# deweylab/RSEM

Hardware: AMD Instinct MI355X
Metric: EM read-alignments/s (nnz x EM iterations per second), rsem-run-em theta-only rounds (higher is better)
Workload: dtype f64; 1 GPU; BASELINE configs[2] (PairedEndQModel-shaped, the north-star target config): EM matrix of 50000000 reads x 200000 transcripts, 570042118 alignments (11.40/read) per GPU, frozen conprb (rounds >= 12); synthetic_config=C3, kernel=0, parallelism=1 GPU

## Files before the change

rsem_amd/csrc/em.hip:

```cpp
#include <climits>
#include <cstdlib>
#include <cmath>
#include <type_traits>

#include "comm_internal.hpp"
#include "em_internal.hpp"
#include "upload.hpp"
#include "sell_layout.hpp"

namespace {

using rsem::kEpsilon;

constexpr int kReduceBlocks = 64;
constexpr int kMaxTimedRounds = 4096;
constexpr int kWindow = 2048;
static_assert(kWindow == kLayoutWindow, "the layout sorts reads apart and sizes windows for the E step's LDS window (sell_layout.hpp)");

constexpr int kTotSlots = 64;

struct Ctrl {
    int done;
    int final_round;
    int totNum;
// ... 288 lines not shown
            const double change = fabs(th - old) / old;
            if (change >= 0.001) ++tot;
            bmax = fmax(bmax, change);
        }
    };
    if (pre) {
#pragma unroll
        for (int k = 0; k < kPre; k++) {
            const int i = lo + (int)threadIdx.x + kBlock * k;
            if (i < hi) one(i, pc[k], pp[k]);
        }
    } else {
        for (int i = lo + threadIdx.x; i < hi; i += kBlock) one(i, cur[i], A.prev[i]);
    }
    for (int d = 32; d >= 1; d >>= 1) {
        tot += __shfl_xor(tot, d);
        bmax = fmax(bmax, __shfl_xor(bmax, d));
    }
    csum = wave_sum(csum);
    __shared__ int s_tot[kBlock / 64];
    __shared__ double s_b[kBlock / 64], s_c[kBlock / 64];
    if (lane == 0) { s_tot[threadIdx.x >> 6] = tot; s_b[threadIdx.x >> 6] = bmax; s_c[threadIdx.x >> 6] = csum; }
    __syncthreads();
    if (threadIdx.x == 0) {
        for (int i = 1; i < kBlock / 64; i++) { tot += s_tot[i]; bmax = fmax(bmax, s_b[i]); csum += s_c[i]; }
        Ctrl* ctrl = A.ctrl;
        unsigned int zero = 0;
        if (bmax > 0.0) {
            const unsigned long long was = __hip_atomic_fetch_max(&ctrl->bbits, (unsigned long long)__double_as_longlong(bmax),
                                                                  __ATOMIC_RELAXED, __HIP_MEMORY_SCOPE_AGENT);
            asm volatile("v_and_b32 %0, 0, %1" : "=v"(zero) : "v"((unsigned int)was));
        }
        zero += sum_slot_put(ctrl, me, csum);
        const unsigned long long old = __hip_atomic_fetch_add(&ctrl->tick2, (((unsigned long long)(unsigned)tot << 32) | 1ull) + zero,
                                                              __ATOMIC_RELAXED, __HIP_MEMORY_SCOPE_AGENT);
        if ((int)(old & 0xffffffffull) == n_close - 1) {
            const int round = A.stat_round;
            const int totNum = (int)(old >> 32) + tot;
            const unsigned long long bb = __hip_atomic_load(&ctrl->bbits, __ATOMIC_RELAXED, __HIP_MEMORY_SCOPE_AGENT);
            const double fsum = sum_slots_take(ctrl, n_close);
            ctrl->last_sum = fsum;
            ctrl->last_bchange = __longlong_as_double((long long)bb);
            ctrl->last_totNum = totNum;
            ctrl->last_round = round;
            const bool stop = !(round < A.min_round || (totNum > 0 && round < A.max_round));
            if (stop) {
                ctrl->done = 1;
                ctrl->final_round = round;
            }
            if (A.mirror) {
                RoundStat* h = &A.mirror->hist[(round - 1) % kHistCap];
                h->sum = fsum;
                h->bchange = __longlong_as_double((long long)bb);
                h->totNum = totNum;
                h->round = round;
                if (stop) A.mirror->final_round = round;
                __hip_atomic_store(&A.mirror->last_round, round, __ATOMIC_RELEASE, __HIP_MEMORY_SCOPE_SYSTEM);
                if (stop) __hip_atomic_store(&A.mirror->done, 1, __ATOMIC_RELEASE, __HIP_MEMORY_SCOPE_SYSTEM);
            }
            __hip_atomic_store(&ctrl->bbits, 0ull, __ATOMIC_RELAXED, __HIP_MEMORY_SCOPE_AGENT);
            __hip_atomic_store(&ctrl->tick2, 0ull, __ATOMIC_RELAXED, __HIP_MEMORY_SCOPE_AGENT);
            for (int k = 0; k < 2 * kTotSlots; k++) A.prev[n + k] = 0.0;
        }
    }
}

__global__ __launch_bounds__(kBlock) void k_solo_finish(int32_t M, double N0, const double* __restrict__ buf, double* theta, double* counts_last) {
    const int n = M + 1;
    const int lane = threadIdx.x & 63;
    const double extra0 = wave_sum(buf[n + lane]) + N0, sum = wave_sum(buf[n + kTotSlots + lane]) + N0;
    const int i = blockIdx.x * blockDim.x + threadIdx.x;
    if (i < n) {
        const double c = buf[i] + (i == 0 ? extra0 : 0.0);
        counts_last[i] = c;
        theta[i] = c / sum;
    }
}

#ifndef RSEM_FQ_DEPTH
#define RSEM_FQ_DEPTH 3
#endif
constexpr int kFarQDepth = RSEM_FQ_DEPTH;
template <bool kFC, bool kSolo = false, bool kFQ = false>
__global__ __launch_bounds__(kBlock) void k_estep_lane(
    const Shape* __restrict__ shapes, const Unit* __restrict__ units, uint32_t T, int M,
    const double* __restrict__ theta, const double* __restrict__ tsrc, double N0, const unsigned char* __restrict__ sval,
    const int16_t* __restrict__ sexp, const int32_t* __restrict__ ssid, const double* __restrict__ sncp,
    const unsigned long long* __restrict__ masks, double* counts, double* noise_partial, double* totals, const Ctrl* ctrl,
    unsigned long long* trace, SoloArgs solo = SoloArgs(), XArgs xa = XArgs()) {
    if (ctrl->done) return;
    if (trace && threadIdx.x == 0) trace[2 * blockIdx.x] = wall_clock64();
    __shared__ double th_win[kWindow];
    __shared__ double cnt_win[kWindow];
    __shared__ int fq_sid[kFQ ? (kBlock / 64) * kFarQCap : 1];
    __shared__ double fq_val[kFQ ? (kBlock / 64) * kFarQCap : 1];
    __shared__ int fq_n[kBlock / 64];
    const Unit U = units[blockIdx.x];
    const int lane = threadIdx.x & 63;
    const int w = __builtin_amdgcn_readfirstlane((int)(threadIdx.x >> 6));
    FarQueue fq;
    if (kFQ) {
        fq.sid = fq_sid + w * kFarQCap;
        fq.val = fq_val + w * kFarQCap;
        fq.n = fq_n + w;
        if (lane == 0) fq_n[w] = 0;
    }
    if (kSolo && solo.stat_round > 0) solo_close_round(solo, M, N0, theta);
    double noise = 0.0, neff = 0.0;
    {
        const Shape& G = U.S;
        Shape S;
        S.plane_base = G.plane_base;
        S.slice_base = G.slice_base;
        S.n_slices = G.n_slices;
        S.row_base = 0;
        S.n_rows = 0;
        S.slot_base = G.slot_base;
        S.K = G.K;
        S.lg = G.lg;
        S.fmt = G.fmt;
        S.val_base = G.val_base;
        S.cut = G.cut;
        S.reserved = 0;
        const uint32_t u_end = S.slice_base + U.slice_begin + U.n_slices;
        const uint32_t s_begin = S.slice_base + U.slice_begin + (uint32_t)w * U.per_wave;
        const uint32_t s_end = min(u_end, s_begin + U.per_wave);
#define RSEM_ESTEP_BLOCK(KK, QQ, FF, XX) \
    estep_block<KK, kFC, QQ, (QQ ? kQ32Depth[KK - 1] : kF64Depth[KK - 1]), FF, XX>(S, s_begin, s_end, lane, U.base, U.span, theta, tsrc, N0, th_win, cnt_win, sval, sexp, ssid, sncp, masks, counts, noise, neff, M, xa)
#define RSEM_ESTEP_BLOCK_FQ(KK, QQ, XX) \
    estep_block<KK, kFC, QQ, kFarQDepth, true, XX, true>(S, s_begin, s_end, lane, U.base, U.span, theta, tsrc, N0, th_win, cnt_win, sval, sexp, ssid, sncp, masks, counts, noise, neff, M, xa, fq)
        const int code = (S.K - 1) | ((S.fmt == kFmtQ32 ? 1 : 0) << 2) | ((U.pad[0] != 0 ? 1 : 0) << 3) | (((!kFC && S.fmt == kFmtF64X) ? 1 : 0) << 4);
        if constexpr (kFQ) {
            if (s_begin < u_end) switch ((code & 7) | ((code >> 4) << 3)) {
                case 0: RSEM_ESTEP_BLOCK_FQ(1, false, false); break;
                case 1: RSEM_ESTEP_BLOCK_FQ(2, false, false); break;
                case 2: RSEM_ESTEP_BLOCK_FQ(3, false, false); break;
                case 3: RSEM_ESTEP_BLOCK_FQ(4, false, false); break;
                case 4: RSEM_ESTEP_BLOCK_FQ(1, true, false); break;
                case 5: RSEM_ESTEP_BLOCK_FQ(2, true, false); break;
                case 6: RSEM_ESTEP_BLOCK_FQ(3, true, false); break;
                case 7: RSEM_ESTEP_BLOCK_FQ(4, true, false); break;
                default:
                    if constexpr (!kFC) switch (code & 3) {
                        case 0: RSEM_ESTEP_BLOCK_FQ(1, false, true); break;
                        case 1: RSEM_ESTEP_BLOCK_FQ(2, false, true); break;
                        case 2: RSEM_ESTEP_BLOCK_FQ(3, false, true); break;
                        default: RSEM_ESTEP_BLOCK_FQ(4, false, true); break;
                    }
                    break;
            } else {
                const ThetaSrc th = theta_src<kFC>(theta, tsrc, N0, lane);
                stage_windows<kFC>(U.base, U.span, M, th, th_win, cnt_win);
            }
        } else
        if (s_begin < u_end) switch (code) {
            case 0: RSEM_ESTEP_BLOCK(1, false, false, false); break;
            case 1: RSEM_ESTEP_BLOCK(2, false, false, false); break;
            case 2: RSEM_ESTEP_BLOCK(3, false, false, false); break;
            case 3: RSEM_ESTEP_BLOCK(4, false, false, false); break;
            case 4: RSEM_ESTEP_BLOCK(1, true, false, false); break;
            case 5: RSEM_ESTEP_BLOCK(2, true, false, false); break;
            case 6: RSEM_ESTEP_BLOCK(3, true, false, false); break;
            case 7: RSEM_ESTEP_BLOCK(4, true, false, false); break;
            case 8: RSEM_ESTEP_BLOCK(1, false, true, false); break;
            case 9: RSEM_ESTEP_BLOCK(2, false, true, false); break;
            case 10: RSEM_ESTEP_BLOCK(3, false, true, false); break;
            case 11: RSEM_ESTEP_BLOCK(4, false, true, false); break;
            case 12: RSEM_ESTEP_BLOCK(1, true, true, false); break;
            case 13: RSEM_ESTEP_BLOCK(2, true, true, false); break;
            case 14: RSEM_ESTEP_BLOCK(3, true, true, false); break;
            case 15: RSEM_ESTEP_BLOCK(4, true, true, false); break;
            default:
                if constexpr (!kFC) switch (code & 11) {
                    case 0: RSEM_ESTEP_BLOCK(1, false, false, true); break;
                    case 1: RSEM_ESTEP_BLOCK(2, false, false, true); break;
                    case 2: RSEM_ESTEP_BLOCK(3, false, false, true); break;
                    case 3: RSEM_ESTEP_BLOCK(4, false, false, true); break;
                    case 8: RSEM_ESTEP_BLOCK(1, false, true, true); break;
                    case 9: RSEM_ESTEP_BLOCK(2, false, true, true); break;
                    case 10: RSEM_ESTEP_BLOCK(3, false, true, true); break;
                    default: RSEM_ESTEP_BLOCK(4, false, true, true); break;
                }
                break;
#undef RSEM_ESTEP_BLOCK
#undef RSEM_ESTEP_BLOCK_FQ
        } else {
            const ThetaSrc th = theta_src<kFC>(theta, tsrc, N0, lane);
            stage_windows<kFC>(U.base, U.span, M, th, th_win, cnt_win);
        }
    }
    __syncthreads();
    for (int i = threadIdx.x; i < U.span; i += blockDim.x) {
        const double v = cnt_win[i];
        if (v != 0.0) unsafeAtomicAdd(&counts[U.base + i], v);
    }
    block_add_totals(noise, neff, noise_partial, totals);
    if (trace && threadIdx.x == 0) trace[2 * blockIdx.x + 1] = wall_clock64();
}


__device__ inline double block_sum_det(double v) {
    __shared__ double red[kBlock / 64];
    __syncthreads();
    v = wave_sum(v);
    if ((threadIdx.x & 63) == 0) red[threadIdx.x >> 6] = v;
    __syncthreads();
    double t = 0.0;
    for (int i = 0; i < kBlock / 64; i++) t += red[i];
    return t;
}

__global__ __launch_bounds__(kBlock) void k_mstep_reduce(int32_t M, double N0, double* counts,
                                                          const double* __restrict__ noise_a, int n_a,
                                                          const double* __restrict__ noise_b, int n_b,
                                                          double* partials, const Ctrl* ctrl) {
    if (ctrl && ctrl->done) return;
    const int n = M + 1;
    const int per = (n + gridDim.x - 1) / gridDim.x;
    const int lo = blockIdx.x * per, hi = min(n, lo + per);
    if (blockIdx.x == 0) {
        double v = 0.0;
        for (int i = threadIdx.x; i < n_a; i += blockDim.x) v += noise_a[i];
        for (int i = threadIdx.x; i < n_b; i += blockDim.x) v += noise_b[i];
        double t = block_sum_det(v);
        if (threadIdx.x == 0) counts[0] = counts[0] + t + N0;
        __syncthreads();
    }
    double v = 0.0;
    for (int i = lo + threadIdx.x; i < hi; i += blockDim.x) v += counts[i];
    double t = block_sum_det(v);
    if (threadIdx.x == 0) partials[blockIdx.x] = t;
}

__global__ __launch_bounds__(kBlock) void k_mstep_apply(int32_t M, const double* __restrict__ partials,
                                                         int n_partials, double* counts,
                                                         const double* __restrict__ theta_old,
                                                         double* theta_new, double* counts_last, Ctrl* ctrl,
                                                         int round, int min_round, int max_round) {
// ... 192 lines not shown
#pragma unroll
        for (int k = 0; k < kPre; k++) {
            const int i = lo + (int)threadIdx.x + k * (int)blockDim.x;
            if (i < hi) one(i, pc[k], po[k]);
        }
    } else {
        for (int i = lo + threadIdx.x; i < hi; i += blockDim.x) one(i, counts[i], theta_old[i]);
    }
    __shared__ int s_tot[kBlock / 64];
    __shared__ double s_b[kBlock / 64], s_c[kBlock / 64];
    for (int d = 32; d >= 1; d >>= 1) {
        tot += __shfl_xor(tot, d);
        bmax = fmax(bmax, __shfl_xor(bmax, d));
    }
    csum = wave_sum(csum);
    __shared__ int s_last;
    if ((threadIdx.x & 63) == 0) { s_tot[threadIdx.x >> 6] = tot; s_b[threadIdx.x >> 6] = bmax; s_c[threadIdx.x >> 6] = csum; }
    if (threadIdx.x == 0) s_last = 0;
    __syncthreads();
    if (threadIdx.x == 0) {
        for (int i = 1; i < kBlock / 64; i++) { tot += s_tot[i]; bmax = fmax(bmax, s_b[i]); csum += s_c[i]; }
        unsigned int zero = 0;
        if (bmax > 0.0) {
            const unsigned long long was = __hip_atomic_fetch_max(&ctrl->bbits, (unsigned long long)__double_as_longlong(bmax),
                                                                  __ATOMIC_RELAXED, __HIP_MEMORY_SCOPE_AGENT);
            asm volatile("v_and_b32 %0, 0, %1" : "=v"(zero) : "v"((unsigned int)was));
        }
        zero += sum_slot_put(ctrl, (int)blockIdx.x, csum);
        const unsigned long long old = __hip_atomic_fetch_add(&ctrl->tick2, (((unsigned long long)(unsigned)tot << 32) | 1ull) + zero,
                                                              __ATOMIC_RELAXED, __HIP_MEMORY_SCOPE_AGENT);
        if ((unsigned)(old & 0xffffffffull) == gridDim.x - 1) {
            const int totNum = (int)(old >> 32) + tot;
            const unsigned long long bb = __hip_atomic_load(&ctrl->bbits, __ATOMIC_RELAXED, __HIP_MEMORY_SCOPE_AGENT);
            const double fsum = sum_slots_take(ctrl, (int)gridDim.x);
            ctrl->last_sum = fsum;
            ctrl->last_bchange = __longlong_as_double((long long)bb);
            ctrl->last_totNum = totNum;
            ctrl->last_round = round;
            const bool stop = !(round < min_round || (totNum > 0 && round < max_round));
            if (stop) {
                ctrl->done = 1;
                ctrl->final_round = round;
            }
            if (mirror) {
                RoundStat* h = &mirror->hist[(round - 1) % kHistCap];
                h->sum = fsum;
                h->bchange = __longlong_as_double((long long)bb);
                h->totNum = totNum;
                h->round = round;
                if (stop) mirror->final_round = round;
                __hip_atomic_store(&mirror->last_round, round, __ATOMIC_RELEASE, __HIP_MEMORY_SCOPE_SYSTEM);
                if (stop) __hip_atomic_store(&mirror->done, 1, __ATOMIC_RELEASE, __HIP_MEMORY_SCOPE_SYSTEM);
            }
            __hip_atomic_store(&ctrl->bbits, 0ull, __ATOMIC_RELAXED, __HIP_MEMORY_SCOPE_AGENT);
            __hip_atomic_store(&ctrl->tick2, 0ull, __ATOMIC_RELAXED, __HIP_MEMORY_SCOPE_AGENT);
            s_last = 1;
        }
    }
    __syncthreads();
    if (!kFused && s_last && threadIdx.x < 2 * kTotSlots) __hip_atomic_store(&totals[threadIdx.x], 0.0, __ATOMIC_RELAXED, __HIP_MEMORY_SCOPE_AGENT);
}

}


struct rsem_em_ctx {
    int device = 0;
    int32_t M = 0;
    uint64_t N1 = 0, nnz = 0;
    hipStream_t stream = nullptr;
    bool own_stream = true;
    uint64_t* d_row_ptr = nullptr;
    int32_t* d_sid = nullptr;
    double* d_cp = nullptr;
    double* d_ncp = nullptr;
    bool have_values = false;
    SellLayout L;
    unsigned char* d_sval = nullptr;
    double* d_sncp = nullptr;
    int16_t* d_sexp = nullptr;
    int* d_fill_err = nullptr;
    int value_bits = 64;
    int value_range_bits = 8;
    int short_last_plane = 1;
    int short_min_units = kShortClassMinUnits;
    bool layout_has_q32 = false;
    bool layout_ok = false;
    Unit* d_units = nullptr;
    unsigned long long* d_trace = nullptr;
    std::vector<Unit> h_units;
    uint64_t long_nnz = 0;
    uint32_t* d_rank = nullptr;
    double *d_xextra = nullptr, *d_xinv = nullptr;
    int split_rows = 1;
    int split_policy = 1;
    uint32_t n_far_units = 0;
    unsigned long long n_stray_reads = 0;
    int tune_passes_left = 1;
    uint32_t n_units = 0;
    uint32_t n_units_main = 0;
    uint32_t n_units_compact = 0;
    uint32_t n_units_queued = 0;
    int far_queue = 1;
    hipStream_t stream_x = nullptr;
    hipEvent_t ev_x_fork = nullptr, ev_x_join = nullptr;
    int x_overlap = 0;
    int noise_n = 0;
    size_t noise_cap = 0;
    double* d_theta[2] = {nullptr, nullptr};
    double* d_red3 = nullptr;
    double* d_red = nullptr;
    double* d_counts = nullptr;
    double* d_counts_last = nullptr;
    double* d_noise_a = nullptr;
    double* d_noise_b = nullptr;
    double* d_totals = nullptr;
    bool use_totals = false;
    double* d_partials = nullptr;
    double* d_w = nullptr;
    double* d_wn = nullptr;
    Ctrl* d_ctrl = nullptr;
    int grid_main = 0, grid_long = 0, grid_apply = 0;
    int kernel = RSEM_EM_KERNEL_AUTO;
    uint32_t forced_T = 0;
    int check_every = 64;
    int n_cus = 256;
    std::vector<hipEvent_t> events;
    HostMirror* mirror = nullptr;
    hipEvent_t lag_ev[2] = {nullptr, nullptr};
    hipStream_t stream2 = nullptr;
    hipEvent_t ev_e[4] = {nullptr, nullptr, nullptr, nullptr}, ev_s[4] = {nullptr, nullptr, nullptr, nullptr};
    rsem_comm* comm = nullptr;
    bool csr_released = false;
    int views_out = 0;
    rsem_em_progress_fn progress = nullptr;
    void* progress_user = nullptr;
};

namespace {

int resolved_kernel(const rsem_em_ctx* c) {
    return c->kernel == RSEM_EM_KERNEL_AUTO ? RSEM_EM_KERNEL_LANE : c->kernel;
}

bool same_unit(const Unit& a, const Unit& b) {
    return a.shape == b.shape && a.slice_begin == b.slice_begin && a.n_slices == b.n_slices && a.per_wave == b.per_wave && a.base == b.base &&
           a.span == b.span && a.pad[0] == b.pad[0] && a.pad[1] == b.pad[1] && !memcmp(&a.S, &b.S, sizeof(Shape));
}

int partition_units(rsem_em_ctx* c) {
    auto is_main = [](const Unit& u) { return u.S.fmt != kFmtF64X; };
    const auto mid = std::stable_partition(c->h_units.begin(), c->h_units.end(), is_main);
    c->n_units_main = (uint32_t)(mid - c->h_units.begin());
    auto queued = [](const Unit& u) { return u.pad[0] != 0 && (uint64_t)u.pad[1] <= 48ull * u.n_slices; };
    c->n_units_queued = (uint32_t)std::count_if(c->h_units.begin(), mid, queued);
    c->n_units_compact = c->n_units_main;
    if (c->far_queue && c->n_units_queued * 25ull >= c->n_units_main && c->n_units_queued)
        c->n_units_compact = (uint32_t)(std::stable_partition(c->h_units.begin(), mid, [&](const Unit& u) { return !queued(u); }) - c->h_units.begin());
    if (c->n_units)
        RSEM_HIP_TRY(hipMemcpyAsync(c->d_units, c->h_units.data(), sizeof(Unit) * c->n_units, hipMemcpyHostToDevice, c->stream));
    RSEM_HIP_TRY(hipStreamSynchronize(c->stream));
    return RSEM_OK;
}

int launch_estep(rsem_em_ctx* c, const double* d_theta, double* d_counts, hipStream_t st, bool use_ctrl) {
    const Ctrl* ctrl = c->d_ctrl;
// ... 23 lines not shown
                hipLaunchKernelGGL((k_estep_lane<false, false, true>), dim3(u1 - u0), dim3(kBlock), 0, s, c->L.d_shapes, c->d_units + u0, c->L.T, c->M,
                                   d_theta, (const double*)nullptr, 0.0, (const unsigned char*)c->d_sval, (const int16_t*)c->d_sexp, c->L.d_ssid,
                                   c->d_sncp, c->L.d_masks, d_counts, c->d_noise_a + u0, c->use_totals ? c->d_totals : nullptr, ctrl,
                                   c->d_trace ? c->d_trace + 2 * (size_t)u0 : nullptr, SoloArgs(), xa);
        };
        if (c->L.n_x_rows) {
            xa.extra = c->d_xextra; xa.inv = c->d_xinv; xa.slot_base = c->L.x_slot_base;
            static const bool batched = !(getenv("RSEM_HIP_ROWSUM_BATCHED") && atoi(getenv("RSEM_HIP_ROWSUM_BATCHED")) == 0);
            hipLaunchKernelGGL(batched ? k_far_rowsum<true> : k_far_rowsum<false>, dim3(rsem::ceil_div(c->L.n_x_slots, kBlock)), dim3(kBlock), 0, sx, c->L.n_x_slots,
                               (const uint64_t*)c->L.d_far_ptr, (const int32_t*)c->L.d_far_sid, (const double*)c->L.d_far_cp, d_theta, c->d_xextra, ctrl);
        }
        if (far_launch) lane_fq(nc, n_main, sf);
        if (!far_launch && sx == st) lane(0, n_all, st);
        else {
            lane(0, far_launch ? nc : n_main, st);
            lane(n_main, n_all, sx);
        }
        if (c->L.n_far) {
            const int grid = std::max(1, rsem::ceil_div(c->L.n_far, kBlock * 4));
            static const bool xcd = !(getenv("RSEM_HIP_COLSUM_XCD") && atoi(getenv("RSEM_HIP_COLSUM_XCD")) == 0);
            hipLaunchKernelGGL(xcd ? k_far_colsum<true> : k_far_colsum<false>, dim3(grid), dim3(kBlock), 0, sx, c->L.n_far, (const int32_t*)c->L.d_csc_sid,
                               (const double*)c->L.d_csc_cp, (const uint32_t*)c->L.d_csc_slot, c->L.x_slot_base, d_theta, (const double*)c->d_xinv, d_counts, ctrl);
        }
        if (second) {
            RSEM_HIP_TRY(hipGetLastError());
            RSEM_HIP_TRY(hipEventRecord(c->ev_x_join, s2));
            RSEM_HIP_TRY(hipStreamWaitEvent(st, c->ev_x_join, 0));
        }
    }
    RSEM_HIP_TRY(hipGetLastError());
    if (c->L.n_long_rows) {
        hipLaunchKernelGGL(k_estep_long, dim3(c->grid_long), dim3(kBlock), 0, st, (uint64_t)c->L.n_long_rows,
                           (const uint32_t*)(c->L.d_order + c->L.n_sell_rows), (const uint64_t*)c->d_row_ptr, (const int32_t*)c->d_sid, (const double*)c->d_cp,
                           (const double*)c->d_ncp, d_theta, d_counts, c->d_noise_b, ctrl, c->use_totals ? c->d_totals : nullptr);
        RSEM_HIP_TRY(hipGetLastError());
    }
    return RSEM_OK;
}

int n_noise_b(const rsem_em_ctx* c) {
    return c->L.n_long_rows ? c->grid_long : 0;
}

int launch_weights(rsem_em_ctx* c, const double* d_theta, hipStream_t st) {
    const int grid = std::max(1, std::min<int>(c->n_cus * 16, rsem::ceil_div(c->N1, kBlock)));
    hipLaunchKernelGGL(k_weights_csr, dim3(grid), dim3(kBlock), 0, st, c->N1, c->d_row_ptr, c->d_sid, c->d_cp, c->d_ncp, d_theta,
                       c->d_w, c->d_wn);
    RSEM_HIP_TRY(hipGetLastError());
    return RSEM_OK;
}

int launch_mstep(rsem_em_ctx* c, double N0, double* d_counts, const double* d_theta_old, double* d_theta_new,
                 int round, int min_round, int max_round, hipStream_t st, HostMirror* mirror = nullptr) {
    const int grid = std::max(1, std::min(kMstepBlocks, rsem::ceil_div((uint64_t)c->M + 1, kBlock * 4)));
    if (c->use_totals) {
        const int gridf = std::max(1, std::min(2 * kMstepBlocks, rsem::ceil_div((uint64_t)c->M + 1, kBlock * 2)));
        hipLaunchKernelGGL(k_mstep_fast<false>, dim3(gridf), dim3(kBlock), 0, st, c->M, N0, d_counts, c->d_totals, d_theta_old, d_theta_new,
                           c->d_counts_last, c->d_ctrl, round, min_round, max_round, mirror, (double*)nullptr);
        RSEM_HIP_TRY(hipGetLastError());
        return RSEM_OK;
    }
    hipLaunchKernelGGL(k_mstep_fused, dim3(grid), dim3(kBlock), 0, st, c->M, N0, d_counts, c->d_noise_a, c->noise_n,
                       c->d_noise_b, n_noise_b(c), c->d_partials, d_theta_old, d_theta_new, c->d_counts_last, c->d_ctrl,
                       round, min_round, max_round);
    RSEM_HIP_TRY(hipGetLastError());
    return RSEM_OK;
}

int build_layout(rsem_em_ctx* c);
void free_layout(rsem_em_ctx* c);

__global__ void k_sum_row_lengths(uint32_t n, const uint32_t* __restrict__ rows, const uint64_t* __restrict__ row_ptr, unsigned long long* out) {
    unsigned long long v = 0;
    for (uint32_t i = blockIdx.x * blockDim.x + threadIdx.x; i < n; i += gridDim.x * blockDim.x) v += row_ptr[rows[i] + 1] - row_ptr[rows[i]];
    for (int d = 32; d >= 1; d >>= 1) v += __shfl_xor(v, d);
    if ((threadIdx.x & 63) == 0 && v) atomicAdd(out, v);
}

int release_csr(rsem_em_ctx* c) {
    if (c->csr_released) return RSEM_OK;
    const char* why = nullptr;
    if (!c->layout_ok || !c->have_values) why = "there is no layout with values yet";
    else if (c->layout_has_q32 || c->value_bits == 32) why = "Q32 planes hold rounded values";
    else if (c->L.n_x_rows) why = "split rows keep part of their alignments outside the planes";
    else if (c->L.n_long_rows) why = "reads with more than 256 alignments live in the CSR alone";
    else if (c->views_out > 0) why = "a model context still holds the arrays";
    if (why) { rsem::set_last_error("release_csr: %s", why); return RSEM_ERR_STATE; }
    RSEM_HIP_TRY(hipSetDevice(c->device));
    RSEM_HIP_TRY(hipStreamSynchronize(c->stream));
    (void)hipFree(c->d_sid); c->d_sid = nullptr;
    (void)hipFree(c->d_cp); c->d_cp = nullptr;
    c->csr_released = true;
    return RSEM_OK;
}

int ensure_csr(rsem_em_ctx* c) {
    if (!c->csr_released) return RSEM_OK;
    RSEM_HIP_TRY(hipSetDevice(c->device));
    RSEM_HIP_TRY(dmalloc(&c->d_sid, c->nnz));
    if (hipError_t e = dmalloc(&c->d_cp, c->nnz); e != hipSuccess) {
        (void)hipFree(c->d_sid);
        c->d_sid = nullptr;
        RSEM_HIP_TRY(e);
    }
    if (c->L.n_sell_rows)
        hipLaunchKernelGGL(k_unfill_sell, dim3(rsem::ceil_div(c->L.n_sell_rows, kBlock)), dim3(kBlock), 0, c->stream, c->L.d_shapes, c->L.n_shapes, c->L.T,
                           c->L.n_sell_rows, (const uint32_t*)c->L.d_order, (const uint64_t*)c->d_row_ptr, (const int32_t*)c->L.d_ssid,
                           (const unsigned char*)c->d_sval, c->d_sid, c->d_cp);
    RSEM_HIP_TRY(hipGetLastError());
    RSEM_HIP_TRY(hipStreamSynchronize(c->stream));
    c->csr_released = false;
    return RSEM_OK;
}

int write_values(rsem_em_ctx* c) {
    if (c->d_fill_err) RSEM_HIP_TRY(hipMemsetAsync(c->d_fill_err, 0, sizeof(int), c->stream));
    int rc = sell_fill_values(c->L, c->stream, c->d_row_ptr, c->d_cp, c->d_ncp, c->d_sval, c->d_sncp, c->d_sexp, c->d_fill_err, c->d_sid);
    if (rc != RSEM_OK) return rc;
    if (c->layout_has_q32) {
        int h = 0;
        RSEM_HIP_TRY(hipMemcpyAsync(&h, c->d_fill_err, sizeof(int), hipMemcpyDeviceToHost, c->stream));
        RSEM_HIP_TRY(hipStreamSynchronize(c->stream));
        if (h) { rsem::set_last_error("Q32 planes: a read's values left the range its format was chosen for"); return RSEM_ERR_STATE; }
    }
    return RSEM_OK;
}

int fill_values(rsem_em_ctx* c) {
    if (c->value_bits == 32 || c->layout_has_q32) {
        free_layout(c);
        return build_layout(c);
    }
    return write_values(c);
}

void free_layout(rsem_em_ctx* c) {
    sell_free(c->L);
    hipFree(c->d_rank); hipFree(c->d_xextra); hipFree(c->d_xinv);
    c->d_rank = nullptr; c->d_xextra = nullptr; c->d_xinv = nullptr;
    hipFree(c->d_sval); hipFree(c->d_sncp); hipFree(c->d_sexp); hipFree(c->d_fill_err); hipFree(c->d_units); hipFree(c->d_noise_a);
    c->d_sval = nullptr; c->d_sncp = nullptr; c->d_sexp = nullptr; c->d_fill_err = nullptr; c->d_units = nullptr; c->d_noise_a = nullptr;
    c->h_units.clear();
    c->n_units = 0;
    c->layout_has_q32 = false;
    c->layout_ok = false;
}

int build_layout(rsem_em_ctx* c) {
    const uint32_t target_waves = (uint32_t)c->n_cus * 4 * 6 * 5 / 2;
    const bool q32 = c->value_bits == 32 && c->have_values;
    std::vector<Unit> units;
    int split = c->split_rows && resolved_kernel(c) == RSEM_EM_KERNEL_LANE && !q32;
    int short_on = c->short_last_plane, short_min_units = c->short_min_units;
    if (const char* e = getenv("RSEM_HIP_SHORT_LAST_PLANE")) short_on = atoi(e) != 0;
    if (const char* e = getenv("RSEM_HIP_SHORT_MIN_UNITS")) short_min_units = std::max(1, atoi(e));
    if (const char* e = getenv("RSEM_HIP_SPLIT")) split = split && atoi(e) != 0;
    if (split) split = c->split_policy;
    if (const char* e = getenv("RSEM_HIP_SPLIT_POLICY")) { if (split) split = !strcmp(e, "all") ? 2 : 1; }
    int rc = sell_build_refined(c->L, c->stream, c->N1, c->M, c->d_row_ptr, c->d_sid, target_waves, c->forced_T,
                                q32 ? c->d_cp : nullptr, c->value_range_bits, kWindow, units, &c->d_units, &c->n_stray_reads, split,
                                short_on ? short_min_units : 0);
    if (rc != RSEM_OK) return rc;
    if (c->L.n_x_rows) {
        const size_t nxs = (size_t)c->L.n_x_slots;
        RSEM_HIP_TRY(dmalloc(&c->d_xextra, nxs));
        RSEM_HIP_TRY(dmalloc(&c->d_xinv, nxs));
        RSEM_HIP_TRY(hipMemsetAsync(c->d_xextra, 0, sizeof(double) * std::max<size_t>(nxs, 1), c->stream));
        RSEM_HIP_TRY(hipMemsetAsync(c->d_xinv, 0, sizeof(double) * std::max<size_t>(nxs, 1), c->stream));
    }
    c->layout_has_q32 = q32;
    RSEM_HIP_TRY(hipMalloc((void**)&c->d_sval, std::max<uint64_t>(c->L.val_bytes, 1)));
    RSEM_HIP_TRY(dmalloc(&c->d_sncp, (size_t)c->L.n_slots));
    if (q32) {
        RSEM_HIP_TRY(dmalloc(&c->d_sexp, (size_t)c->L.n_slots));
        RSEM_HIP_TRY(dmalloc(&c->d_fill_err, 1));
    }
    RSEM_HIP_TRY(hipMemsetAsync(c->d_sval, 0, c->L.val_bytes, c->stream));
    RSEM_HIP_TRY(hipMemsetAsync(c->d_sncp, 0, sizeof(double) * c->L.n_slots, c->stream));
    if (c->have_values) {
        rc = write_values(c);
        if (rc != RSEM_OK) return rc;
    }
    RSEM_HIP_TRY(hipStreamSynchronize(c->stream));
    c->n_units = (uint32_t)units.size();
    c->h_units = units;
    if (const char* e = getenv("RSEM_HIP_X_OVERLAP")) c->x_overlap = atoi(e);
    if (const char* e = getenv("RSEM_HIP_FAR_QUEUE")) c->far_queue = atoi(e);
    rc = partition_units(c);
    if (rc != RSEM_OK) return rc;
    if ((c->L.n_x_rows || c->n_units_compact < c->n_units_main) && !c->stream_x) {
        RSEM_HIP_TRY(hipStreamCreateWithFlags(&c->stream_x, hipStreamNonBlocking));
        RSEM_HIP_TRY(hipEventCreateWithFlags(&c->ev_x_fork, hipEventDisableTiming));
        RSEM_HIP_TRY(hipEventCreateWithFlags(&c->ev_x_join, hipEventDisableTiming));
    }
    c->tune_passes_left = 1;
    if (const char* e = getenv("RSEM_HIP_TUNE")) c->tune_passes_left = atoi(e);
    c->n_far_units = 0;
    for (const Unit& u : c->h_units) c->n_far_units += u.pad[0] != 0;
    c->noise_cap = std::max<size_t>((size_t)c->n_cus * 8, c->n_units);
    RSEM_HIP_TRY(dmalloc(&c->d_noise_a, c->noise_cap));
    RSEM_HIP_TRY(hipMemsetAsync(c->d_noise_a, 0, sizeof(double) * c->noise_cap, c->stream));

    c->grid_long = std::max(1, std::min<int>(c->n_cus * 8, rsem::ceil_div(c->L.n_long_rows, kBlock / 64)));
    c->long_nnz = 0;
    if (c->L.n_long_rows) {
        unsigned long long* d_n = (unsigned long long*)c->d_noise_a;
        hipLaunchKernelGGL(k_sum_row_lengths, dim3(c->grid_long), dim3(kBlock), 0, c->stream, c->L.n_long_rows, c->L.d_order + c->L.n_sell_rows,
                           c->d_row_ptr, d_n);
        RSEM_HIP_TRY(hipGetLastError());
        unsigned long long h = 0;
        RSEM_HIP_TRY(hipMemcpyAsync(&h, d_n, sizeof(h), hipMemcpyDeviceToHost, c->stream));
        RSEM_HIP_TRY(hipMemsetAsync(c->d_noise_a, 0, sizeof(double), c->stream));
        RSEM_HIP_TRY(hipStreamSynchronize(c->stream));
        c->long_nnz = h;
    }
    c->layout_ok = true;
    return RSEM_OK;
}

void set_grid_for_kernel(rsem_em_ctx* c) {
    c->grid_main = std::max(1, std::min<int>(c->n_cus * 8, rsem::ceil_div(c->L.n_slices, kBlock / 64)));
}

}

extern "C" {

int rsem_em_create(rsem_em_ctx** out, int device, int32_t M, uint64_t N1, uint64_t nnz, const uint64_t* row_ptr,
                   const int32_t* sid, const double* conprb, const double* ncp) {
    RSEM_REQUIRE(out != nullptr, "out is NULL");
    *out = nullptr;
    RSEM_REQUIRE(M >= 1, "M must be >= 1");
    RSEM_REQUIRE(row_ptr != nullptr && (sid != nullptr || nnz == 0), "row_ptr / sid is NULL");
    RSEM_REQUIRE(N1 < 0xfffffff0ull, "N1 too large for one shard (max 2^32-16 reads)");
    RSEM_REQUIRE(row_ptr[0] == 0 && row_ptr[N1] == nnz, "row_ptr[0] != 0 or row_ptr[N1] != nnz");
    RSEM_REQUIRE((conprb == nullptr) == (ncp == nullptr), "conprb and ncp must be given together");
    int ndev = 0;
    if (hipGetDeviceCount(&ndev) != hipSuccess || device < 0 || device >= ndev) {
        (void)hipGetLastError();
        rsem::set_last_error("no HIP device %d (have %d)", device, ndev);
        return RSEM_ERR_NODEVICE;
    }
    RSEM_HIP_TRY(hipSetDevice(device));
    hipDeviceProp_t prop;
    RSEM_HIP_TRY(hipGetDeviceProperties(&prop, device));
    rsem_em_ctx* c = new (std::nothrow) rsem_em_ctx();
    if (!c) return RSEM_ERR_NOMEM;
    c->device = device;
    c->M = M;
    c->N1 = N1;
    c->nnz = nnz;
    c->n_cus = prop.multiProcessorCount > 0 ? prop.multiProcessorCount : 256;
    int rc = RSEM_OK;
    auto fail = [&](int code) { rsem_em_destroy(c); return code; };
#define TRY_OR_FAIL(expr)                                                                               \
    do {                                                                                                \
// ... 94 lines not shown
    }
    return RSEM_OK;
}

int rsem_em_set_comm(rsem_em_ctx* c, rsem_comm* comm) {
    RSEM_REQUIRE(c != nullptr, "NULL argument");
    c->comm = comm;
    return RSEM_OK;
}

int rsem_em_set_progress(rsem_em_ctx* c, rsem_em_progress_fn fn, void* user) {
    RSEM_REQUIRE(c != nullptr, "NULL argument");
    c->progress = fn;
    c->progress_user = user;
    return RSEM_OK;
}

int rsem_em_set_option(rsem_em_ctx* c, const char* key, int64_t value) {
    RSEM_REQUIRE(c && key, "NULL argument");
    if (!strcmp(key, "release_csr")) {
        RSEM_REQUIRE(value == 0 || value == 1, "release_csr must be 0 or 1");
        return value ? release_csr(c) : ensure_csr(c);
    }
    if (!strcmp(key, "kernel") || !strcmp(key, "split_rows") || !strcmp(key, "split_policy") || !strcmp(key, "value_bits") || !strcmp(key, "value_range_bits")) {
        int rc0 = ensure_csr(c);
        if (rc0 != RSEM_OK) return rc0;
    }
    if (!strcmp(key, "kernel")) {
        RSEM_REQUIRE(value >= RSEM_EM_KERNEL_AUTO && value <= RSEM_EM_KERNEL_LANE, "unknown kernel variant");
        RSEM_REQUIRE(value == RSEM_EM_KERNEL_AUTO || value == RSEM_EM_KERNEL_LANE, "kernel variants CSR (1) and SELL (2) were retired: AUTO (0) or LANE (3)");
        c->kernel = (int)value;
        if (c->layout_ok && c->L.n_x_rows && resolved_kernel(c) != RSEM_EM_KERNEL_LANE) {
            RSEM_HIP_TRY(hipSetDevice(c->device));
            free_layout(c);
            int rc = build_layout(c);
            if (rc != RSEM_OK) return rc;
        }
        set_grid_for_kernel(c);
        return RSEM_OK;
    }
    if (!strcmp(key, "split_overlap")) {
        RSEM_REQUIRE(value == 0 || value == 1, "split_overlap must be 0 or 1");
        c->x_overlap = (int)value;
        return RSEM_OK;
    }
    if (!strcmp(key, "split_policy")) {
        RSEM_REQUIRE(value == 1 || value == 2, "split_policy must be 1 (reads mostly outside their window) or 2 (every read with an id outside)");
        if (c->split_policy == (int)value) return RSEM_OK;
        c->split_policy = (int)value;
        c->x_overlap = value == 2 ? 1 : 0;
        RSEM_HIP_TRY(hipSetDevice(c->device));
        free_layout(c);
        int rc = build_layout(c);
        if (rc != RSEM_OK) return rc;
        set_grid_for_kernel(c);
        return RSEM_OK;
    }
    if (!strcmp(key, "split_rows")) {
        RSEM_REQUIRE(value == 0 || value == 1, "split_rows must be 0 or 1");
        if (c->split_rows == (int)value) return RSEM_OK;
        c->split_rows = (int)value;
        RSEM_HIP_TRY(hipSetDevice(c->device));
        free_layout(c);
        int rc = build_layout(c);
        if (rc != RSEM_OK) return rc;
        set_grid_for_kernel(c);
        return RSEM_OK;
    }
    if (!strcmp(key, "value_bits") || !strcmp(key, "value_range_bits")) {
        const bool bits = !strcmp(key, "value_bits");
        if (bits) RSEM_REQUIRE(value == 64 || value == 32, "value_bits must be 64 or 32");
        else RSEM_REQUIRE(value >= 0 && value <= 24, "value_range_bits must be in 0..24");
        int& field = bits ? c->value_bits : c->value_range_bits;
        if (field == (int)value) return RSEM_OK;
        field = (int)value;
        if (c->value_bits == 64 && !c->layout_has_q32) return RSEM_OK;
        RSEM_HIP_TRY(hipSetDevice(c->device));
        free_layout(c);
        int rc = build_layout(c);
        if (rc != RSEM_OK) return rc;
        set_grid_for_kernel(c);
        return RSEM_OK;
    }
    if (!strcmp(key, "short_last_plane") || !strcmp(key, "short_class_min_units")) {
        const bool sw = !strcmp(key, "short_last_plane");
        if (sw) RSEM_REQUIRE(value == 0 || value == 1, "short_last_plane must be 0 or 1");
        else RSEM_REQUIRE(value >= 1 && value <= 1000000, "short_class_min_units must be in 1..1000000");
        int& field = sw ? c->short_last_plane : c->short_min_units;
        if (field == (int)value) return RSEM_OK;
        field = (int)value;
        if (!sw && !c->short_last_plane) return RSEM_OK;
        RSEM_HIP_TRY(hipSetDevice(c->device));
        { int rc0 = ensure_csr(c); if (rc0 != RSEM_OK) return rc0; }
        free_layout(c);
        int rc = build_layout(c);
        if (rc != RSEM_OK) return rc;
        set_grid_for_kernel(c);
        return RSEM_OK;
    }
    if (!strcmp(key, "check_every")) {
        RSEM_REQUIRE(value >= 1 && value <= kHistCap / 4, "check_every out of range");
        c->check_every = (int)value;
        return RSEM_OK;
    }
    rsem::set_last_error("unknown option '%s'", key);
    return RSEM_ERR_INVALID;
}

int rsem_em_get_info(const rsem_em_ctx* c, const char* key, int64_t* value) {
    RSEM_REQUIRE(c && key && value, "NULL argument");
    if (!strcmp(key, "value_bits")) *value = c->value_bits;
    else if (!strcmp(key, "csr_released")) *value = c->csr_released ? 1 : 0;
    else if (!strcmp(key, "csr_bytes")) *value = (int64_t)(12 * c->nnz);
    else if (!strcmp(key, "value_range_bits")) *value = c->value_range_bits;
    else if (!strcmp(key, "far_units")) *value = c->n_far_units;
    else if (!strcmp(key, "units")) *value = c->n_units;
    else if (!strcmp(key, "units_compact")) *value = c->n_units_compact;
    else if (!strcmp(key, "units_main")) *value = c->n_units_main;
    else if (!strcmp(key, "units_queued")) *value = c->n_units_queued;
    else if (!strcmp(key, "unit_tables_agree")) {
        std::vector<Unit> d(c->n_units);
        if (c->n_units) {
            RSEM_HIP_TRY(hipSetDevice(c->device));
            RSEM_HIP_TRY(hipMemcpyAsync(d.data(), c->d_units, sizeof(Unit) * c->n_units, hipMemcpyDeviceToHost, c->stream));
            RSEM_HIP_TRY(hipStreamSynchronize(c->stream));
        }
        bool same = d.size() == c->h_units.size();
        for (size_t i = 0; same && i < d.size(); i++) same = same_unit(d[i], c->h_units[i]);
        *value = same ? 1 : 0;
    }
    else if (!strcmp(key, "stray_reads")) *value = (int64_t)c->n_stray_reads;
    else if (!strcmp(key, "reads_q32")) *value = c->L.n_q32_rows;
    else if (!strcmp(key, "reads_sliced")) *value = c->L.n_sell_rows;
    else if (!strcmp(key, "reads_long")) *value = c->L.n_long_rows;
    else if (!strcmp(key, "value_plane_bytes")) *value = (int64_t)c->L.val_bytes;
    else if (!strcmp(key, "value_plane_entries")) *value = (int64_t)c->L.n_val_entries;
    else if (!strcmp(key, "short_last_plane")) *value = c->short_last_plane;
    else if (!strcmp(key, "short_class_min_units")) *value = c->short_min_units;
    else if (!strcmp(key, "short_classes")) *value = (int64_t)__builtin_popcountll(c->L.short_classes);
    else if (!strcmp(key, "shapes")) *value = c->L.n_shapes;
    else if (!strcmp(key, "unit_bytes")) *value = (int64_t)sizeof(Unit);
    else if (!strcmp(key, "sid_plane_bytes")) *value = (int64_t)(c->L.n_planes * 256);
    else if (!strcmp(key, "slots")) *value = c->L.n_slots;
    else if (!strcmp(key, "sid_plane_bytes_loaded")) *value = (int64_t)(c->L.n_sid_planes_loaded * 256);
    else if (!strcmp(key, "slices")) *value = c->L.n_slices;
    else if (!strcmp(key, "split_rows")) *value = c->L.n_x_rows;
    else if (!strcmp(key, "far_entries")) *value = (int64_t)c->L.n_far;
    else if (!strcmp(key, "window_entries")) {
        int64_t w = 0;
        for (const Unit& u : c->h_units) w += u.span;
        *value = w;
    } else if (!strcmp(key, "physical_bytes_per_launch")) {
        int64_t w = 0;
        for (const Unit& u : c->h_units) w += u.span;
        const uint64_t long_nnz = c->long_nnz + (c->L.n_long_rows * 4ull) / 3;
        const uint64_t far_bytes = 28 * c->L.n_far + 40 * (uint64_t)c->L.n_x_slots;
        *value = (int64_t)(c->L.val_bytes + c->L.n_sid_planes_loaded * 256 + (uint64_t)c->L.n_slots * (8 + (c->layout_has_q32 ? 2 : 0)) +
                           (uint64_t)c->L.n_slices * 8 + (uint64_t)c->n_units * sizeof(Unit) + (uint64_t)w * 16 + 16 * ((uint64_t)c->M + 1)) +
                 (int64_t)(12 * long_nnz + far_bytes);
    }
    else if (!strcmp(key, "units")) *value = c->n_units;
    else { rsem::set_last_error("unknown info key '%s'", key); return RSEM_ERR_INVALID; }
    return RSEM_OK;
}

int rsem_em_debug_trace(rsem_em_ctx* c, const double* theta, unsigned long long* out, uint32_t* n_units_io) {
    RSEM_REQUIRE(c && theta && out && n_units_io, "NULL argument");
    RSEM_REQUIRE(resolved_kernel(c) == RSEM_EM_KERNEL_LANE && c->have_values && c->layout_ok, "needs the LANE kernel with values set");
    RSEM_REQUIRE(*n_units_io >= c->n_units, "trace buffer too small");
    RSEM_HIP_TRY(hipSetDevice(c->device));
    unsigned long long* d = nullptr;
    RSEM_HIP_TRY(hipMalloc((void**)&d, sizeof(unsigned long long) * 2 * std::max<uint32_t>(c->n_units, 1)));
    RSEM_HIP_TRY(hipMemcpyAsync(c->d_theta[0], theta, sizeof(double) * ((size_t)c->M + 1), hipMemcpyHostToDevice, c->stream));
    RSEM_HIP_TRY(hipMemsetAsync(c->d_ctrl, 0, sizeof(Ctrl), c->stream));
    int rc = RSEM_OK;
    for (int rep = 0; rep < 3 && rc == RSEM_OK; rep++) {
        c->d_trace = d;
        rc = launch_estep(c, c->d_theta[0], c->d_counts, c->stream, true);
        c->d_trace = nullptr;
    }
    hipError_t e = hipMemcpyAsync(out, d, sizeof(unsigned long long) * 2 * c->n_units, hipMemcpyDeviceToHost, c->stream);
    if (e == hipSuccess) e = hipStreamSynchronize(c->stream);
    (void)hipMemsetAsync(c->d_counts, 0, sizeof(double) * ((size_t)c->M + 1), c->stream);
    (void)hipStreamSynchronize(c->stream);
    (void)hipFree(d);
    if (e != hipSuccess) { rsem::set_last_error("trace download failed"); return RSEM_ERR_HIP; }
    *n_units_io = c->n_units;
    return rc;
}

int rsem_em_destroy(rsem_em_ctx* c) {
    if (!c) return RSEM_OK;
    (void)hipSetDevice(c->device);
    for (hipEvent_t e : c->events) (void)hipEventDestroy(e);
    hipFree(c->d_row_ptr); hipFree(c->d_sid); hipFree(c->d_cp); hipFree(c->d_ncp);
    sell_free(c->L); hipFree(c->d_sval); hipFree(c->d_sncp); hipFree(c->d_sexp); hipFree(c->d_fill_err);
    hipFree(c->d_theta[0]); hipFree(c->d_theta[1]); hipFree(c->d_red3);
    for (int i = 0; i < 4; i++) { if (c->ev_e[i]) (void)hipEventDestroy(c->ev_e[i]); if (c->ev_s[i]) (void)hipEventDestroy(c->ev_s[i]); }
    if (c->stream2) (void)hipStreamDestroy(c->stream2);
    if (c->stream_x) (void)hipStreamDestroy(c->stream_x);
    if (c->ev_x_fork) (void)hipEventDestroy(c->ev_x_fork);
    if (c->ev_x_join) (void)hipEventDestroy(c->ev_x_join);
    hipFree(c->d_counts_last); hipFree(c->d_noise_a); hipFree(c->d_noise_b); hipFree(c->d_partials);
    if (c->mirror) (void)hipHostFree(c->mirror);
    for (int i = 0; i < 2; i++) if (c->lag_ev[i]) (void)hipEventDestroy(c->lag_ev[i]);
    hipFree(c->d_w); hipFree(c->d_wn); hipFree(c->d_ctrl); hipFree(c->d_units);
    if (c->stream && c->own_stream) (void)hipStreamDestroy(c->stream);
    delete c;
    return RSEM_OK;
}

static int tune_unit_order(rsem_em_ctx* c, const double* d_theta) {
    while (c->tune_passes_left > 0) {
        --c->tune_passes_left;
        if (resolved_kernel(c) != RSEM_EM_KERNEL_LANE || c->n_units < 2048) return RSEM_OK;
        const uint32_t n = c->n_units;
        unsigned long long* d = nullptr;
        RSEM_HIP_TRY(hipMalloc((void**)&d, sizeof(unsigned long long) * 2 * n));
        std::vector<unsigned long long> t(2 * (size_t)n);
        int rc = RSEM_OK;
        for (int rep = 0; rep < 2 && rc == RSEM_OK; rep++) {
            c->d_trace = d;
            rc = launch_estep(c, d_theta, c->d_counts, c->stream, true);
            c->d_trace = nullptr;
        }
        hipError_t e = hipMemcpyAsync(t.data(), d, sizeof(unsigned long long) * 2 * n, hipMemcpyDeviceToHost, c->stream);
        if (e == hipSuccess) e = hipStreamSynchronize(c->stream);
        (void)hipFree(d);
        if (rc != RSEM_OK) return rc;
        if (e != hipSuccess) { rsem::set_last_error("unit tuning: trace download failed"); return RSEM_ERR_HIP; }
        std::vector<uint32_t> order(n);
        for (uint32_t i = 0; i < n; i++) order[i] = i;
        std::stable_sort(order.begin(), order.end(), [&](uint32_t a, uint32_t b) { return t[2 * a + 1] - t[2 * a] > t[2 * b + 1] - t[2 * b]; });
        std::vector<Unit> sorted(n);
        for (uint32_t i = 0; i < n; i++) sorted[i] = c->h_units[order[i]];
        c->h_units.swap(sorted);
        rc = partition_units(c);
        if (rc != RSEM_OK) return rc;
    }
    return RSEM_OK;
// ... 243 lines not shown
    RSEM_HIP_TRY(hipMemsetAsync(c->d_ctrl, 0, sizeof(Ctrl), st));
    RSEM_HIP_TRY(hipMemsetAsync(c->d_counts, 0, nb, st));
    int rc = launch_estep(c, c->d_theta[0], c->d_counts, st, true);
    if (rc != RSEM_OK) return rc;
    rc = launch_mstep(c, N0, c->d_counts, c->d_theta[0], c->d_theta[1], 1, 1, 1, st);
    if (rc != RSEM_OK) return rc;
    Ctrl h;
    RSEM_HIP_TRY(hipMemcpyAsync(&h, c->d_ctrl, sizeof(Ctrl), hipMemcpyDeviceToHost, st));
    if (counts) RSEM_HIP_TRY(hipMemcpyAsync(counts, c->d_counts_last, nb, hipMemcpyDeviceToHost, st));
    if (theta_new) RSEM_HIP_TRY(hipMemcpyAsync(theta_new, c->d_theta[1], nb, hipMemcpyDeviceToHost, st));
    RSEM_HIP_TRY(hipStreamSynchronize(st));
    if (sum) *sum = h.last_sum;
    if (bChange) *bChange = h.last_bchange;
    if (totNum) *totNum = h.last_totNum;
    return RSEM_OK;
}

int rsem_em_expected_weights(rsem_em_ctx* c, const double* theta, double N0, double* counts, double* w, double* w_noise) {
    RSEM_REQUIRE(c && theta, "NULL argument");
    if (!c->have_values) { rsem::set_last_error("CSR values were never set"); return RSEM_ERR_STATE; }
    if (!c->layout_ok) { rsem::set_last_error("the device layout could not be rebuilt after the last change of values / options"); return RSEM_ERR_STATE; }
    RSEM_HIP_TRY(hipSetDevice(c->device));
    hipStream_t st = c->stream;
    const size_t nb = sizeof(double) * ((size_t)c->M + 1);
    if (w || w_noise) { int rc0 = ensure_csr(c); if (rc0 != RSEM_OK) return rc0; }
    if ((w || w_noise) && !c->d_w) RSEM_HIP_TRY(dmalloc(&c->d_w, c->nnz));
    if ((w || w_noise) && !c->d_wn) RSEM_HIP_TRY(dmalloc(&c->d_wn, c->N1));
    RSEM_HIP_TRY(hipMemcpyAsync(c->d_theta[0], theta, nb, hipMemcpyHostToDevice, st));
    RSEM_HIP_TRY(hipMemsetAsync(c->d_ctrl, 0, sizeof(Ctrl), st));
    RSEM_HIP_TRY(hipMemsetAsync(c->d_counts, 0, nb, st));
    int rc = launch_estep(c, c->d_theta[0], c->d_counts, st, true);
    if (rc != RSEM_OK) return rc;
    hipLaunchKernelGGL(k_mstep_reduce, dim3(kReduceBlocks), dim3(kBlock), 0, st, c->M, N0, c->d_counts, c->d_noise_a, c->noise_n,
                       c->d_noise_b, n_noise_b(c), c->d_partials, (const Ctrl*)c->d_ctrl);
    RSEM_HIP_TRY(hipGetLastError());
    if ((w || w_noise) && c->N1) {
        rc = launch_weights(c, c->d_theta[0], st);
        if (rc != RSEM_OK) return rc;
    }
    if (counts) RSEM_HIP_TRY(hipMemcpyAsync(counts, c->d_counts, nb, hipMemcpyDeviceToHost, st));
    if (w && c->nnz) RSEM_HIP_TRY(hipMemcpyAsync(w, c->d_w, sizeof(double) * c->nnz, hipMemcpyDeviceToHost, st));
    if (w_noise && c->N1) RSEM_HIP_TRY(hipMemcpyAsync(w_noise, c->d_wn, sizeof(double) * c->N1, hipMemcpyDeviceToHost, st));
    RSEM_HIP_TRY(hipMemsetAsync(c->d_counts, 0, nb, st));
    RSEM_HIP_TRY(hipStreamSynchronize(st));
    return RSEM_OK;
}

}


namespace rsem {

int em_device_view(rsem_em_ctx* c, EmDeviceView* v) {
    RSEM_REQUIRE(c && v, "NULL argument");
    RSEM_HIP_TRY(hipSetDevice(c->device));
    { int rc0 = ensure_csr(c); if (rc0 != RSEM_OK) return rc0; }
    v->device = c->device;
    v->stream = c->stream;
    v->M = c->M;
    v->N1 = c->N1;
    v->nnz = c->nnz;
    v->d_row_ptr = c->d_row_ptr;
    v->d_sid = c->d_sid;
    v->d_cp = c->d_cp;
    v->d_ncp = c->d_ncp;
    v->d_w = c->d_w;
    v->d_wn = c->d_wn;
    return RSEM_OK;
}

__global__ void k_invert_order(uint64_t n, const uint32_t* __restrict__ order, uint32_t* rank) {
    const uint64_t p = (uint64_t)blockIdx.x * blockDim.x + threadIdx.x;
    if (p < n) rank[order[p]] = (uint32_t)p;
}

void em_view_hold(rsem_em_ctx* c) {
    if (c) c->views_out += 1;
}
void em_view_release(rsem_em_ctx* c) {
    if (c && c->views_out > 0) c->views_out -= 1;
}

bool em_planes_writable(const rsem_em_ctx* c) {
    return c && c->layout_ok && !c->layout_has_q32 && c->value_bits != 32 && !c->L.n_x_rows;
}

int em_planes_view(rsem_em_ctx* c, EmPlanesView* v) {
    RSEM_REQUIRE(c && v, "NULL argument");
    if (!em_planes_writable(c)) {
        set_last_error("the layout holds Q32 planes or split rows");
        return RSEM_ERR_STATE;
    }
    RSEM_HIP_TRY(hipSetDevice(c->device));
    if (!c->d_rank && c->N1) {
        RSEM_HIP_TRY(dmalloc(&c->d_rank, (size_t)c->N1));
        hipLaunchKernelGGL(k_invert_order, dim3(ceil_div(c->N1, kBlock)), dim3(kBlock), 0, c->stream, c->N1, (const uint32_t*)c->L.d_order, c->d_rank);
        RSEM_HIP_TRY(hipGetLastError());
    }
    v->d_rank = c->d_rank;
    v->d_shapes = c->L.d_shapes;
    v->n_shapes = c->L.n_shapes;
    v->T = c->L.T;
    v->n_sell_rows = c->L.n_sell_rows;
    v->d_sval = c->d_sval;
    v->d_sncp = c->d_sncp;
    return RSEM_OK;
}

int em_values_written_in_place(rsem_em_ctx* c) {
    RSEM_REQUIRE(c, "NULL argument");
    if (!c->layout_ok || c->layout_has_q32) { set_last_error("the layout cannot have been written in place"); return RSEM_ERR_STATE; }
    c->have_values = true;
    return RSEM_OK;
}

int em_values_changed(rsem_em_ctx* c) {
    RSEM_REQUIRE(c, "NULL argument");
    RSEM_HIP_TRY(hipSetDevice(c->device));
    c->have_values = true;
    return fill_values(c);
}


}

namespace { __global__ void k_preload_em() {} }
namespace rsem { void preload_em() { hipLaunchKernelGGL(k_preload_em, dim3(1), dim3(1), 0, nullptr); (void)hipGetLastError(); } }
```

rsem_amd/csrc/estep_block.hpp:

```cpp
#pragma once
#include <type_traits>

#include "simt_macros.hpp"

RSEM_DEVFN double wave_sum(double v) {
#pragma unroll
    for (int d = 32; d >= 1; d >>= 1) v += RSEM_SHFL_XOR(v, d);
    return v;
}


struct ThetaSrc {
    const double* v;
    double extra0, sum;
};
template <bool kFC>
RSEM_DEVFN double theta_at(const ThetaSrc& t, int i) {
    if (!kFC) return t.v[i];
    return (t.v[i] + (i == 0 ? t.extra0 : 0.0)) / t.sum;
}
template <bool kFC>
RSEM_DEVFN ThetaSrc theta_src(const double* __restrict__ v, const double* __restrict__ tsrc, double N0, int lane);

template <bool kFC>
RSEM_DEVFN void stage_windows(int base, int span, int M, const ThetaSrc& th, double* th_win, double* cnt_win) {
    for (int i = RSEM_TIDX; i < span; i += RSEM_BDIM) {
        const int sidv = base + i;
        th_win[i] = (sidv >= 0 && sidv <= M) ? theta_at<kFC>(th, sidv) : 0.0;
        cnt_win[i] = 0.0;
    }
    RSEM_SYNC();
}

struct XArgs {
    const double* extra = nullptr;
    double* inv = nullptr;
    uint32_t slot_base = 0;
};

#ifndef RSEM_FARQ_CAP
#define RSEM_FARQ_CAP 384
#endif
constexpr int kFarQCap = RSEM_FARQ_CAP;
static_assert(kFarQCap > 256, "a slice of K = 4 planes can append 256 entries");
struct FarQueue {
    int* sid = nullptr;
    double* val = nullptr;
    int* n = nullptr;
};

template <int K, bool kQ>
struct SliceRegs {
    int id[K];
    typename std::conditional<kQ, uint32_t, double>::type c[K];
    double nc;
    int e;
    double x;
    uint32_t slot0;
    double traw[K];
};

RSEM_DEVFN double pow2_of(int e) { return RSEM_LL_AS_DOUBLE((long long)(1023 + e) << 52); }

#ifndef RSEM_F64_DEPTHS
#define RSEM_F64_DEPTHS 2, 2, 2, 2
#endif
#ifndef RSEM_Q32_DEPTHS
#define RSEM_Q32_DEPTHS 2, 2, 2, 2
#endif
template <typename T>
RSEM_DEVFN T stream_load(const T* p) { return RSEM_NT_LOAD(p); }
template <int kCtrl>
RSEM_DEVFN double dpp_take(double v) {
    const long long b = RSEM_DOUBLE_AS_LL(v);
    const int lo = RSEM_DPP_MOV((int)(unsigned)b, kCtrl);
    const int hi = RSEM_DPP_MOV((int)(unsigned)(b >> 32), kCtrl);
    return RSEM_LL_AS_DOUBLE(((long long)hi << 32) | (unsigned)lo);
}
RSEM_DEVFN double read_sum_dpp(double part, int lg) {
    if (lg >= 1) part += dpp_take<0xB1>(part);
    if (lg >= 2) part += dpp_take<0x4E>(part);
    if (lg >= 3) part += dpp_take<0x141>(part);
    if (lg >= 4) part += dpp_take<0x140>(part);
    for (int d = 16; d < (1 << lg); d <<= 1) part += RSEM_SHFL_XOR(part, d);
    return part;
}
constexpr int kF64Depth[4] = {RSEM_F64_DEPTHS};
constexpr int kQ32Depth[4] = {RSEM_Q32_DEPTHS};

template <int K, bool kFC, bool kQ, int NBUF, bool kFar, bool kX = false, bool kFQ = false>
RSEM_DEVFN void estep_block(const Shape& S, uint32_t s_begin, uint32_t s_end, int lane, int base, int span,
                                   const double* __restrict__ theta, const double* __restrict__ tsrc, double N0, double* th_win, double* cnt_win,
                                   const unsigned char* __restrict__ sval, const int16_t* __restrict__ sexp, const int32_t* __restrict__ ssid,
                                   const double* __restrict__ sncp, const unsigned long long* __restrict__ masks,
                                   double* counts, double& noise, double& neff, int M, const XArgs& X = XArgs(), const FarQueue& FQ = FarQueue()) {
    static_assert(!kFQ || kFar, "the far queue belongs to the loop of the units with ids outside their window");
    static_assert(!kFQ || NBUF >= 3, "the far-queue loop requests theta a slice ahead: three register sets at least (the ring loop)");
    using ValT = typename std::conditional<kQ, uint32_t, double>::type;
    const ValT* __restrict__ scp = (const ValT*)(sval + S.val_base);
    const int lg = S.lg;
    const int g = lane & ((1 << lg) - 1);
    const bool g0 = (g == 0);
    const uint32_t R = 64u >> lg;
    uint32_t m_base = s_begin;
    unsigned long long mv = (s_begin + lane < s_end) ? masks[s_begin + lane] : ~0ull;
    auto mask_of = [&](uint32_t t) -> unsigned long long {
        if (t - m_base >= 64u) {
            m_base = t;
            mv = (t + lane < s_end) ? masks[t + lane] : ~0ull;
            RSEM_PIN(mv);
        }
        const int src = (int)(t - m_base);
        const uint32_t lo = RSEM_READLANE((int)(uint32_t)mv, src);
        const uint32_t hi = RSEM_READLANE((int)(uint32_t)(mv >> 32), src);
        return ((unsigned long long)hi << 32) | lo;
    };
    const unsigned ulane = (unsigned)lane, uslot = ulane >> lg;
    const unsigned Gk = (unsigned)shape_Gk(S);
    const unsigned last_lane = uslot * Gk + ((unsigned)g < Gk ? (unsigned)g : Gk - 1u);
    const bool last_ok = (unsigned)g < Gk;
    const uint32_t vstride = (uint32_t)RSEM_READFIRSTLANE((int)shape_val_stride(S));
    auto issue = [&](uint32_t t, unsigned long long m, SliceRegs<K, kQ>& b) {
        const uint32_t sl = t - S.slice_base;
        const uint64_t v0 = (uint64_t)sl * (K * 64);
        const ValT* __restrict__ vp = scp + (uint64_t)sl * vstride;
        if (kFQ || m != 0ull) {
            const int32_t* __restrict__ ip = ssid + (S.plane_base * 64 + v0);
#pragma unroll
            for (int k = 0; k < K; k++) b.id[k] = ip[k * 64 + ulane];
        }
#pragma unroll
        for (int k = 0; k < K - 1; k++) b.c[k] = stream_load(&vp[k * 64 + ulane]);
        b.c[K - 1] = stream_load(&vp[(K - 1) * 64 + last_lane]);
        const uint32_t slot0 = S.slot_base + sl * R;
        b.nc = (sncp + slot0)[uslot];
        b.e = kQ ? (int)(sexp + slot0)[uslot] : 0;
        b.x = kX ? (X.extra + (slot0 - X.slot_base))[uslot] : 0.0;
        b.slot0 = slot0;
    };
    auto spill = [&](const int* rsid, double* acc) {
#pragma unroll
        for (int k = 0; k < K; k++) {
            if (acc[k] != 0.0) {
                const unsigned off = (unsigned)(rsid[k] - base);
                if (!kFar) RSEM_LDS_ADD(&cnt_win[off < (unsigned)span ? off : 0u], acc[k]);
                else if (off < (unsigned)span) RSEM_LDS_ADD(&cnt_win[off], acc[k]);
                else if (kFQ) {
                    const int at = RSEM_LDS_FETCH_ADD_I32(FQ.n, 1);
                    FQ.sid[at] = rsid[k];
                    FQ.val[at] = acc[k];
                } else RSEM_ATOMIC_ADD(&counts[rsid[k]], acc[k]);
            }
            acc[k] = 0.0;
        }
    };
    auto far_queue_room = [&](bool all) {
        if (!kFQ) return;
        RSEM_WAVE_SYNC();
        const int n = RSEM_READFIRSTLANE(*FQ.n);
        if (n > (all ? 0 : kFarQCap - 64 * K)) {
            for (int i = lane; i < n; i += 64) RSEM_ATOMIC_ADD(&counts[FQ.sid[i]], FQ.val[i]);
            RSEM_WAIT_VM0();
            RSEM_WAVE_SYNC();
            if (lane == 0) *FQ.n = 0;
            RSEM_WAVE_SYNC();
        }
    };

    int rsid[K];
    double rth[K], acc[K];
#pragma unroll
    for (int k = 0; k < K; k++) { rsid[k] = 0; rth[k] = 0.0; acc[k] = 0.0; }
    ThetaSrc th{theta, 0.0, 1.0};
    double th0 = 0.0;
    auto pregather = [&](SliceRegs<K, kQ>& b, unsigned long long m) {
        if (!kFQ) return;
        const bool starts = ((m >> lane) & 1ull) != 0ull;
#pragma unroll
        for (int k = 0; k < K; k++) {
            const int sidv = b.id[k];
            const bool want = starts && !((unsigned)(sidv - base) < (unsigned)span);
            b.traw[k] = th.v[want ? sidv : 0];
        }
    };
    auto reduce = [&](const SliceRegs<K, kQ>& cur, unsigned long long cur_m) {
        if (cur_m != 0ull) {
            far_queue_room(false);
            if ((cur_m >> lane) & 1ull) {
                spill(rsid, acc);
                bool far = false;
#pragma unroll
                for (int k = 0; k < K; k++) {
                    const int sidv = cur.id[k];
                    rsid[k] = sidv;
                    const unsigned off = (unsigned)(sidv - base);
                    const bool in = off < (unsigned)span;
                    rth[k] = th_win[in ? off : 0u];
                    far = far || !in;
                }
                if (kFQ) {
#pragma unroll
                    for (int k = 0; k < K; k++)
                        if (!((unsigned)(rsid[k] - base) < (unsigned)span))
                            rth[k] = kFC ? (cur.traw[k] + (rsid[k] == 0 ? th.extra0 : 0.0)) / th.sum : cur.traw[k];
                } else if (kFar && far) {
                    double t[K];
#pragma unroll
                    for (int k = 0; k < K; k++) {
                        const bool in = (unsigned)(rsid[k] - base) < (unsigned)span;
                        t[k] = theta_at<kFC>(th, in ? 0 : rsid[k]);
                    }
#pragma unroll
                    for (int k = 0; k < K; k++) {
                        RSEM_PIN(t[k]);
                        if (!((unsigned)(rsid[k] - base) < (unsigned)span)) rth[k] = t[k];
                    }
                }
            }
        }
        double f0 = g0 ? th0 * cur.nc : 0.0;
        if (f0 < kEpsilon) f0 = 0.0;
        double f[K];
        double part = f0 + ((kX && g0) ? cur.x : 0.0);
        const double scale = kQ ? pow2_of(cur.e) : 1.0;
#pragma unroll
        for (int k = 0; k < K; k++) {
            const ValT cr = (k == K - 1 && !last_ok) ? ValT(0) : cur.c[k];
            const double cv = kQ ? (double)cr * scale : (double)cr;
            double v = rth[k] * cv;
            if (v < kEpsilon) v = 0.0;
            f[k] = v;
            part += v;
        }
        part = read_sum_dpp(part, lg);
        const double inv = (part >= kEpsilon) ? 1.0 / part : 0.0;
        if (kX) RSEM_STORE_SAME(&(X.inv + (cur.slot0 - X.slot_base))[uslot], inv);
        noise += f0 * inv;
        neff += (g0 && part >= kEpsilon) ? 1.0 : 0.0;
#pragma unroll
        for (int k = 0; k < K; k++) acc[k] = acc[k] + f[k] * inv;
    };
    if constexpr (NBUF == 2) {
        SliceRegs<K, kQ> A, B;
        unsigned long long mA = ~0ull, mB = 0;
        issue(s_begin, mA, A);
        th = theta_src<kFC>(theta, tsrc, N0, lane);
        th0 = theta_at<kFC>(th, 0);
        stage_windows<kFC>(base, span, M, th, th_win, cnt_win);
        uint32_t s = s_begin;
        for (; s + 2 < s_end; s += 2) {
            mB = mask_of(s + 1);
            issue(s + 1, mB, B);
            reduce(A, mA);
            mA = mask_of(s + 2);
            issue(s + 2, mA, A);
            reduce(B, mB);
        }
        if (s + 1 < s_end) {
            mB = mask_of(s + 1);
            issue(s + 1, mB, B);
            reduce(A, mA);
            reduce(B, mB);
        } else {
            reduce(A, mA);
        }
    } else {
        SliceRegs<K, kQ> buf[NBUF];
        unsigned long long mk[NBUF];
        mk[0] = ~0ull;
        issue(s_begin, mk[0], buf[0]);
        th = theta_src<kFC>(theta, tsrc, N0, lane);
        th0 = theta_at<kFC>(th, 0);
        stage_windows<kFC>(base, span, M, th, th_win, cnt_win);
        auto within = [&](uint32_t t) -> uint32_t { return t < s_end ? t : s_end - 1u; };
#pragma unroll
        for (int j = 1; j < NBUF - 1; j++) {
            const uint32_t tt = within(s_begin + j);
            mk[j] = mask_of(tt);
            issue(tt, mk[j], buf[j]);
        }
        pregather(buf[0], mk[0]);
        uint32_t s = s_begin;
        for (; s + NBUF <= s_end; s += NBUF) {
#pragma unroll
            for (int j = 0; j < NBUF; j++) {
                constexpr int ahead = NBUF - 1;
                const int nj = (j + ahead) % NBUF;
                const uint32_t tt = within(s + j + ahead);
                mk[nj] = mask_of(tt);
                issue(tt, mk[nj], buf[nj]);
                pregather(buf[(j + 1) % NBUF], mk[(j + 1) % NBUF]);
                reduce(buf[j], mk[j]);
            }
        }
#pragma unroll
        for (int j = 0; j < NBUF - 1; j++)
            if (s + j < s_end) {
                if (j > 0) pregather(buf[j], mk[j]);
                reduce(buf[j], mk[j]);
            }
    }
    far_queue_room(false);
    spill(rsid, acc);
    far_queue_room(true);
}

template <bool kFC>
RSEM_DEVFN ThetaSrc theta_src(const double* __restrict__ v, const double* __restrict__ tsrc, double N0, int lane) {
    ThetaSrc t{v, 0.0, 1.0};
    if (kFC) {
        const double a = wave_sum(tsrc[lane]);
        const double b = wave_sum(tsrc[kTotSlots + lane]);
        t.extra0 = a + N0;
        t.sum = b + N0;
    }
    return t;
}
```

rsem_amd/csrc/host/run_em.cpp:

```cpp
#include <charconv>
#include <chrono>
#include <cstdint>
#include <cstdio>
#include <cstdlib>
#include <cstring>
#include <ctime>
#include <fcntl.h>
#include <functional>
#include <memory>
#include <string>
#include <unistd.h>
#include <thread>
#include <vector>

#include "../../../include/rsem_hip.h"
#include "bam_io.hpp"
#include "files.hpp"
#include "model_host.hpp"
#include "reads.hpp"
#include "results.hpp"
#include "ofb.hpp"
#include "rsb.hpp"

using namespace rsemh;
// ... 538 lines not shown
    do {
        ++ROUND;
        const bool updateModel = ROUND <= 10;
        const bool calc = model.needCalcConPrb;
        rsem_model_tables t = tables_of(model);
        each_shard([&](Shard& X, int k) {
            X.rc = RSEM_OK;
            if (calc) X.rc = rsem_model_set_tables(X.mc, &t);
            if (X.rc != RSEM_OK) { X.err = rsem_hip_last_error(); return; }
            double* cts = S == 1 ? counts.data() : s_counts[k].data();
            double s1 = 0.0, b1 = 0.0;
            int32_t t1 = 0;
            rsem_model_accum a;
            if (updateModel) {
                Model::Accum& A = S == 1 ? acc : s_acc[k];
                a.prof = A.prof.data(); a.noise = A.noise.data(); a.rspd = A.rspd.data(); a.gld = A.gld.data();
                a.gld0_lb = P.minL - 1; a.gld0_ub = P.maxL;
            }
            const double n0 = S == 1 ? (double)N0 : 0.0;
            double* thn = S == 1 ? theta_new.data() : nullptr;
            if (calc)
                X.rc = rsem_model_round(X.mc, theta.data(), n0, cts, thn, &s1, &b1, &t1, updateModel ? &a : nullptr);
            else if (updateModel) X.rc = rsem_model_estep_update(X.mc, theta.data(), n0, cts, thn, &s1, &b1, &t1, &a);
            else X.rc = rsem_em_step(X.em, theta.data(), n0, cts, thn, &s1, &b1, &t1);
            if (X.rc != RSEM_OK) { X.err = rsem_hip_last_error(); return; }
            if (S == 1) { sum = s1; bChange = b1; totNum = t1; }
        });
        check_shards(calc ? "rsem_model_round" : (updateModel ? "rsem_model_estep_update" : "rsem_em_step"));
        model.needCalcConPrb = false;
        if (S > 1) {
            for (int j = 0; j <= M; j++) {
                double c = s_counts[0][j];
                for (int k = 1; k < S; k++) c += s_counts[k][j];
                counts[j] = c;
            }
            counts[0] += N0;
            sum = 0.0;
            for (int j = 0; j <= M; j++) sum += counts[j];
            if (!(sum >= kEpsilon)) die("rsem-run-em: the fractional counts sum to %g", sum);
            bChange = 0.0; totNum = 0;
            for (int j = 0; j <= M; j++) {
                theta_new[j] = counts[j] / sum;
                if (theta[j] >= 1e-7) {
                    const double change = fabs(theta_new[j] - theta[j]) / theta[j];
                    if (change >= 0.001) ++totNum;
                    if (bChange < change) bChange = change;
                }
            }
            if (updateModel) {
                for (size_t i = 0; i < acc.prof.size(); i++) { double v = s_acc[0].prof[i]; for (int k = 1; k < S; k++) v += s_acc[k].prof[i]; acc.prof[i] = v; }
                for (size_t i = 0; i < acc.noise.size(); i++) { double v = s_acc[0].noise[i]; for (int k = 1; k < S; k++) v += s_acc[k].noise[i]; acc.noise[i] = v; }
                for (size_t i = 0; i < acc.rspd.size(); i++) { double v = s_acc[0].rspd[i]; for (int k = 1; k < S; k++) v += s_acc[k].rspd[i]; acc.rspd[i] = v; }
                for (size_t i = 0; i < acc.gld.size(); i++) { double v = s_acc[0].gld[i]; for (int k = 1; k < S; k++) v += s_acc[k].gld[i]; acc.gld[i] = v; }
            }
        }
        if (updateModel) model.finish_round(acc, refs);
        theta.swap(theta_new);
        if (verbose) printf("ROUND = %d, SUM = %.15g, bChange = %g, totNum = %d\n", ROUND, sum, bChange, totNum);
        if (round_times) {
            const auto now = std::chrono::steady_clock::now();
            printf("[timing]   model round %-2d            %8.3f s\n", ROUND, std::chrono::duration<double>(now - t_round).count());
            t_round = now;
        }
        if (ROUND >= 11 && !model.needCalcConPrb) break;
    } while (ROUND < MIN_ROUND || (totNum > 0 && ROUND < MAX_ROUND));
    lap("rounds 1-11 (model rounds)");
    std::thread releaser([&]() {
        if (getenv("RSEM_HIP_NO_RELEASE")) return;
        {
            std::vector<std::pair<char*, size_t>> big;
            for (int tag = 0; tag < 3; tag++)
                for (int m = 0; m < 2; m++) { big.push_back(rs.mate[tag][m].off.owned_bytes()); big.push_back(rs.mate[tag][m].seq.owned_bytes()); big.push_back(rs.mate[tag][m].qual.owned_bytes()); }
            big.push_back(dat.pos.owned_bytes()); big.push_back(dat.insertL.owned_bytes()); big.push_back(dat.sid_signed.owned_bytes());
            give_back_pages(big, getenv("RSEM_HIP_RELEASE_THREADS") ? atoi(getenv("RSEM_HIP_RELEASE_THREADS")) : 8);
        }
        for (int tag = 0; tag < 3; tag++)
            for (int m = 0; m < 2; m++) rs.mate[tag][m] = ReadFile();
        dat.pos.release(); dat.insertL.release(); dat.sid_signed.release();
        std::vector<uint8_t>().swap(ref_seq);
        std::vector<uint32_t>().swap(mask_words);
        std::vector<uint8_t>().swap(lq);
    });
    Joiner release_joiner{releaser};
    if (leanDevice) {
        each_shard([&](Shard& X, int) {
            rsem_model_destroy(X.mc);
            X.mc = nullptr;
            if (rsem_em_set_option(X.em, "release_csr", 1) != RSEM_OK && verbose)
                printf("--lean-device: the caller-order arrays stay on the device (%s)\n", rsem_hip_last_error());
        });
        lap("lean device");
    }
    if (ROUND < MIN_ROUND || (totNum > 0 && ROUND < MAX_ROUND)) {
        const int round0 = ROUND;
        std::vector<std::vector<double>> s_theta(S, theta);
        std::vector<int> s_rounds(S, ROUND);
        std::vector<int32_t> s_tn(S, 0);
        std::vector<double> s_bc(S, 0.0);
        if (verbose)
            hip_check(rsem_em_set_progress(sh[0].em, [](int r, double sm, double bc, int tn, void*) {
                printf("ROUND = %d, SUM = %.15g, bChange = %g, totNum = %d\n", r, sm, bc, tn);
            }, nullptr), "rsem_em_set_progress");
        if (value_bits == 32) {
            each_shard([&](Shard& X, int) {
                X.rc = value_range_bits >= 0 ? rsem_em_set_option(X.em, "value_range_bits", value_range_bits) : RSEM_OK;
                if (X.rc == RSEM_OK) X.rc = rsem_em_set_option(X.em, "value_bits", 32);
                if (X.rc != RSEM_OK) X.err = rsem_hip_last_error();
            });
            check_shards("rsem_em_set_option(value_bits)");
            lap("Q32 value planes");
        }
        each_shard([&](Shard& X, int k) {
            X.rc = rsem_em_run(X.em, s_theta[k].data(), (double)N0, round0, MIN_ROUND, MAX_ROUND, &s_rounds[k], k == 0 ? counts.data() : nullptr,
                               &s_bc[k], &s_tn[k], nullptr);
            if (X.rc != RSEM_OK) X.err = rsem_hip_last_error();
        });
        check_shards("rsem_em_run");
        for (int k = 1; k < S; k++)
            if (s_rounds[k] != s_rounds[0]) die("rsem-run-em: shard %d stopped at round %d, shard 0 at round %d", k, s_rounds[k], s_rounds[0]);
        theta = s_theta[0];
        ROUND = s_rounds[0];
        totNum = s_tn[0];
        bChange = s_bc[0];
    }
    lap("rounds >= 12 (device loop)");
    if (totNum > 0) fprintf(stderr, "Warning: RSEM reaches %d iterations before meeting the convergence criteria.\n", MAX_ROUND);

    if (genGibbsOut) {
        std::unique_ptr<double[]> cp(new double[nnz ? nnz : 1]), ncp(new double[N1 ? N1 : 1]);
        OfbHeader ofb_hdr;
        each_shard([&](Shard& X, int) {
            X.rc = X.mc ? rsem_model_get_values(X.mc, cp.get() + X.a, ncp.get() + X.lo) : rsem_em_get_values(X.em, cp.get() + X.a, ncp.get() + X.lo);
            if (X.rc != RSEM_OK) X.err = rsem_hip_last_error();
        });
        check_shards("rsem_model_get_values");
        if (ofbMode >= 1) {
            const int ntb = N1 > 100000 ? hardware_threads() : 1;
            std::vector<OfbPart> parts(ntb);
            parallel_for(ntb, [&](int t) {
                const uint64_t lo = N1 * t / ntb, hi = N1 * (t + 1) / ntb;
                OfbPart& P = parts[t];
                P.lens.reserve((size_t)(hi - lo));
                P.sid.reserve((size_t)(dat.row_ptr[hi] - dat.row_ptr[lo] + (hi - lo)));
                P.val.reserve((size_t)(dat.row_ptr[hi] - dat.row_ptr[lo] + (hi - lo)));
                for (uint64_t i = lo; i < hi; i++) {
                    uint32_t n = 0;
                    if (ncp[i] >= kEpsilon) { ++n; P.sid.push_back(0); P.val.push_back(through_15_digits(ncp[i])); }
                    for (uint64_t k = dat.row_ptr[i]; k < dat.row_ptr[i + 1]; k++)
                        if (cp[k] >= kEpsilon) { ++n; P.sid.push_back(sid_abs[k]); P.val.push_back(through_15_digits(cp[k])); }
                    if (n > 0) P.lens.push_back(n);
                }
            });
            ofb_hdr = write_ofb_arrays(imdName, M, N0, parts);
            if (ofbMode == 1) write_ofb_header(imdName, ofb_hdr);
        } else {
            remove_ofb(imdName);
        }
        const std::string ofg_path = imdName + ".ofg";
        if (ofbMode == 1) ::unlink(ofg_path.c_str());
        char head[64];
        const int head_n = snprintf(head, sizeof(head), "%d %llu\n", M, (unsigned long long)N0);
        const int nt = ofbMode == 1 ? 0 : (N1 > 100000 ? hardware_threads() : 1);
        std::vector<std::string> bufs(nt);
        parallel_for(nt, [&](int t) {
            const uint64_t lo = N1 * t / nt, hi = N1 * (t + 1) / nt;
            std::string& b = bufs[t];
// ... 131 lines not shown
```

rsem_amd/csrc/sell_layout.hpp:

```cpp
#pragma once
#include <hipcub/hipcub.hpp>

#include <algorithm>
#include <vector>

#include "common.hpp"

namespace {

#include "sell_shape.hpp"

constexpr int kShapesPerFmt = 28;
constexpr int kShapeBits = 8;
constexpr int kFullShapes = 3 * kShapesPerFmt;
constexpr int kShortPerFmt = 32;
constexpr int kMaxShapes = kFullShapes + 2 * kShortPerFmt;
static_assert(kMaxShapes <= kShapeTableMax, "the kernels that keep the shape table in LDS size it by kShapeTableMax (sell_shape.hpp)");
constexpr int kShapeIds = 1 << kShapeBits;
constexpr int kLongShape = kShapeIds - 1;
constexpr uint32_t kKeyMinSidCap = (1u << (31 - kShapeBits)) - 1;
constexpr int kKeyApartBit = 63 - kShapeBits;
constexpr int kMaxK = 4;
constexpr int kBlock = 256;

struct Q32Scale { int e; };
__host__ __device__ inline bool q32_scale_of(double mx, double mn_nonzero, int range_bits, Q32Scale& q) {
    if (!(mx > 0.0) || !(mx < 1e300)) return false;
    int ex;
    (void)frexp(mx, &ex);
    q.e = ex - 32;
    if (q.e < -1000 || q.e > 900) return false;
    return mn_nonzero >= ldexp(mx, -range_bits);
}
struct Q32Range {
    double vmx = 0.0, vmn = 1.79e308;
    __host__ __device__ void add(double v) {
        if (!(v >= 0.0)) vmx = 1e308;
        vmx = fmax(vmx, v);
        if (v > 0.0) vmn = fmin(vmn, v);
    }
    __host__ __device__ bool takes_q32(int range_bits, Q32Scale& q) const { return q32_scale_of(vmx, vmn, range_bits, q); }
};
__host__ __device__ inline bool row_takes_q32(const double* __restrict__ cp, uint64_t fr, uint64_t to, int range_bits) {
    Q32Range r;
    for (uint64_t j = fr; j < to; j++) r.add(cp[j]);
    Q32Scale q;
    return r.takes_q32(range_bits, q);
}
__host__ __device__ inline uint32_t q32_mantissa(double v, int e) {
    const double m = rint(ldexp(v, -e));
    return m >= 4294967295.0 ? 0xffffffffu : (uint32_t)m;
}

__host__ __device__ inline int short_class_index(int lg, int K, int q) {
    if (lg < 1 || lg > 6 || K < 3 || K > 4 || q < 1 || q > 3) return -1;
    if (lg == 1) return q == 2 ? (K - 3) : -1;
    return 2 + (lg - 2) * 6 + (K - 3) * 3 + (q - 1);
}
__host__ __device__ inline bool shape_of_id(int id, int& fmt, int& lg, int& K, int& cut) {
    if (id < 0 || id >= kMaxShapes) return false;
    if (id < kFullShapes) {
        fmt = id / kShapesPerFmt;
        lg = (id % kShapesPerFmt) / 4;
        K = id % 4 + 1;
        cut = 0;
        return true;
    }
    const int j = id - kFullShapes, i = j % kShortPerFmt;
    fmt = j / kShortPerFmt;
    if (i < 2) { lg = 1; K = 3 + i; cut = 2; return true; }
    lg = 2 + (i - 2) / 6;
    K = 3 + ((i - 2) % 6) / 3;
    cut = 3 - (i - 2) % 3;
    return true;
}
__host__ __device__ inline int shape_fmt_of_id(int id) { return id < kFullShapes ? id / kShapesPerFmt : (id - kFullShapes) / kShortPerFmt; }
__host__ __device__ inline int full_shape_of_id(int id) {
    int fmt, lg, K, cut;
    if (id < kFullShapes || !shape_of_id(id, fmt, lg, K, cut)) return id;
    return fmt * kShapesPerFmt + lg * 4 + K - 1;
}

__host__ __device__ inline int shape_id_of(uint64_t L, uint32_t short_classes = 0, bool even_quarters = false) {
    if (L <= 4) return (int)(L == 0 ? 0 : L - 1);
    int lg = 1;
    uint64_t cap = 8;
    while (L > cap) { cap <<= 1; ++lg; }
    if (lg > 6) return kLongShape;
    int K = (int)((L + (1u << lg) - 1) >> lg);
    if (short_classes) {
        const int G = 1 << lg, n_last = (int)L - (K - 1) * G;
        int q = (n_last * 4 + G - 1) >> lg;
        if (even_quarters) q = (q + 1) & ~1;
        const int i = short_class_index(lg, K, q);
        if (i >= 0 && ((short_classes >> i) & 1u)) return kFullShapes + i;
    }
    return lg * 4 + (K - 1);
}
__host__ __device__ inline int shape_id_in_fmt(int id, int fmt) {
    return id < kFullShapes ? id + fmt * kShapesPerFmt : id + fmt * kShortPerFmt;
}

__host__ __device__ inline bool slot_to_row(const Shape& S, uint32_t T, uint32_t slice_local, uint32_t r, uint32_t& q) {
    const uint32_t R = shape_R(S), rpb = R * T;
    const uint32_t b = slice_local / T, t = slice_local % T;
    if ((uint64_t)b * rpb >= S.n_rows) return false;
    const uint32_t left = S.n_rows - b * rpb;
    const uint32_t nb = left < rpb ? left : rpb;
    const uint32_t Tb = (nb + R - 1) / R;
    if (t >= Tb || r * Tb + t >= nb) return false;
    q = b * rpb + r * Tb + t;
    return true;
}

__host__ __device__ inline uint32_t mix32(uint32_t h, uint32_t v) {
    h ^= v + 0x9e3779b9u + (h << 6) + (h >> 2);
    return h;
}


constexpr int kLayoutWindow = 2048;
constexpr int kAnchorReach = kLayoutWindow / 2;
constexpr int kMedianExactMax = 64;
__host__ __device__ inline uint64_t row_key_of(uint64_t i, int32_t M, const uint64_t* __restrict__ row_ptr,
                                               const int32_t* __restrict__ sid, const double* __restrict__ cp, int range_bits,
                                               int apart, int* err, int split = 0, uint32_t* split_far = nullptr,
                                               uint64_t short_classes = 0 ) {
    uint64_t fr = row_ptr[i], to = row_ptr[i + 1];
    if (to < fr) { *err = 1; return 0; }
    uint32_t h = 0x811c9dc5u, mn = 0xffffffffu;
    Q32Range vr;
    for (uint64_t j = fr; j < to; j++) {
        int32_t s = sid[j];
        if (s < 1 || s > M) { *err = 2; s = 1; }
        h = mix32(h, (uint32_t)s);
        mn = (uint32_t)s < mn ? (uint32_t)s : mn;
        if (cp) vr.add(cp[j]);
    }
    const uint64_t L = to - fr;
    if (L > 1 && !*err) {
        uint32_t med = (uint32_t)sid[fr + L / 2];
        if (L <= (uint64_t)kMedianExactMax) {
            for (uint64_t j = fr; j < to; j++) {
                const uint32_t v = (uint32_t)sid[j];
                uint32_t less = 0, leq = 0;
                for (uint64_t k = fr; k < to; k++) {
                    const uint32_t u = (uint32_t)sid[k];
                    less += u < v ? 1u : 0u;
                    leq += u <= v ? 1u : 0u;
                }
                if (less <= L / 2 && L / 2 < leq) { med = v; break; }
            }
        }
        const uint32_t floor_sid = med > (uint32_t)kAnchorReach ? med - (uint32_t)kAnchorReach : 0u;
        uint32_t lo = med;
        for (uint64_t j = fr; j < to; j++) {
            const uint32_t v = (uint32_t)sid[j];
            if (v >= floor_sid && v < lo) lo = v;
        }
        mn = lo;
    }
    uint64_t far = 0, L_in = 0;
    uint32_t h_in = 0x811c9dc5u;
    if (apart && L > 1 && !*err)
        for (uint64_t j = fr; j < to; j++) {
            const uint32_t v = (uint32_t)sid[j];
            if (v < mn || v >= mn + (uint32_t)apart) far = 1;
            else { ++L_in; h_in = mix32(h_in, v); }
        }
    int shape = shape_id_of(to - fr);
    if (far && split && (split == 2 || 2 * L_in <= L) && shape != kLongShape && (uint64_t)mn <= kKeyMinSidCap) {
        shape = shape_id_in_fmt(shape_id_of(L_in), kFmtF64X);
        if (split_far) *split_far = (uint32_t)(L - L_in);
        return ((uint64_t)shape << (64 - kShapeBits)) | ((uint64_t)mn << 32) | h_in;
    }
    if (mn > kKeyMinSidCap) mn = kKeyMinSidCap;
    Q32Scale q;
    if (shape != kLongShape) {
        const bool q32 = cp && vr.takes_q32(range_bits, q);
        if (short_classes) shape = shape_id_of(to - fr, (uint32_t)(short_classes >> (q32 ? 32 : 0)), q32);
        if (q32) shape = shape_id_in_fmt(shape, kFmtQ32);
    }
    return ((uint64_t)shape << (64 - kShapeBits)) | (far << kKeyApartBit) | ((uint64_t)mn << 32) | h;
}

__global__ void k_row_keys(uint64_t N1, int32_t M, const uint64_t* __restrict__ row_ptr,
                           const int32_t* __restrict__ sid, const double* __restrict__ cp, int range_bits, int apart, int split,
                           const unsigned char* __restrict__ also_apart, uint64_t* keys, uint32_t* vals, int* err,
                           unsigned long long* n_split = nullptr , uint64_t short_classes = 0) {
    uint64_t i = (uint64_t)blockIdx.x * blockDim.x + threadIdx.x;
    if (i >= N1) return;
    int e = 0;
    uint32_t nf = 0;
    uint64_t key = row_key_of(i, M, row_ptr, sid, cp, range_bits, apart, &e, split, &nf, short_classes);
    if (n_split && nf) { atomicAdd(&n_split[0], 1ull); atomicAdd(&n_split[1], (unsigned long long)nf); }
    if (also_apart && also_apart[i] && shape_fmt_of_id((int)(key >> (64 - kShapeBits))) != kFmtF64X) key |= 1ull << kKeyApartBit;
    if (e) *err = e;
    if (e == 1) return;
    keys[i] = key;
    vals[i] = (uint32_t)i;
}

constexpr int kLenHist = 257;
__global__ void k_row_length_hist(uint64_t N1, const uint64_t* __restrict__ row_ptr, const double* __restrict__ cp, int range_bits,
                                  unsigned long long* hist ) {
    __shared__ unsigned int h[2 * kLenHist];
    for (int i = threadIdx.x; i < 2 * kLenHist; i += blockDim.x) h[i] = 0;
    __syncthreads();
    for (uint64_t i = (uint64_t)blockIdx.x * blockDim.x + threadIdx.x; i < N1; i += (uint64_t)gridDim.x * blockDim.x) {
        const uint64_t fr = row_ptr[i], to = row_ptr[i + 1];
        if (to < fr || to - fr > 256) continue;
        const int fmt = (cp && row_takes_q32(cp, fr, to, range_bits)) ? kFmtQ32 : kFmtF64;
        atomicAdd(&h[fmt * kLenHist + (int)(to - fr)], 1u);
    }
    __syncthreads();
    for (int i = threadIdx.x; i < 2 * kLenHist; i += blockDim.x)
        if (h[i]) atomicAdd(&hist[i], (unsigned long long)h[i]);
}
#ifndef RSEM_SHORT_CLASS_MIN_UNITS
#define RSEM_SHORT_CLASS_MIN_UNITS 8
#endif
constexpr int kShortClassMinUnits = RSEM_SHORT_CLASS_MIN_UNITS;
inline uint64_t short_classes_worth_it(const unsigned long long* hist, uint32_t target_waves, uint32_t forced_T, int min_units) {
    uint64_t rows[2][kShortPerFmt] = {}, n_slices = 0;
    for (int f = 0; f < 2; f++)
        for (int L = 1; L < kLenHist; L++) {
            const unsigned long long n = hist[f * kLenHist + L];
            if (!n) continue;
            int fmt, lg, K, cut;
            const int id = shape_id_of((uint64_t)L, 0xffffffffu, f == kFmtQ32);
            shape_of_id(id, fmt, lg, K, cut);
            n_slices += (n + (64u >> lg) - 1) >> (6 - lg);
            if (id >= kFullShapes) rows[f][id - kFullShapes] += n;
        }
    const uint32_t T = forced_T ? forced_T : std::min<uint64_t>(256, std::max<uint64_t>(8, n_slices / std::max(1u, target_waves)));
    uint64_t mask = 0;
    for (int f = 0; f < 2; f++)
        for (int i = 0; i < kShortPerFmt; i++) {
            int fmt, lg, K, cut;
            shape_of_id(kFullShapes + i, fmt, lg, K, cut);
            const uint64_t slices = rows[f][i] >> (6 - lg);
            if (slices >= (uint64_t)min_units * 4 * T && slices > 0) mask |= 1ull << (f * 32 + i);
        }
    return mask;
}

__global__ void k_shape_bounds(uint64_t N1, const uint64_t* __restrict__ keys, uint32_t* first) {
    uint64_t p = (uint64_t)blockIdx.x * blockDim.x + threadIdx.x;
    if (p >= N1) return;
    int sh = (int)(keys[p] >> (64 - kShapeBits));
    if (p == 0 || sh != (int)(keys[p - 1] >> (64 - kShapeBits))) first[sh] = (uint32_t)p;
}

__device__ inline int find_shape_by_row(const Shape* shapes, int n, uint32_t p) {
    int sh = 0;
    while (sh + 1 < n && p >= shapes[sh + 1].row_base) ++sh;
    return sh;
}

__host__ __device__ inline bool in_split_window(int32_t id, uint32_t anchor, int reach) { return (uint32_t)id - anchor < (uint32_t)reach; }

template <bool kIds>
__host__ __device__ inline void sell_fill_row(const Shape& S, uint32_t T, uint32_t p, const uint32_t* __restrict__ order,
                                              const uint64_t* __restrict__ row_ptr, const int32_t* __restrict__ sid,
                                              const double* __restrict__ cp, const double* __restrict__ ncp, int32_t* ssid,
                                              unsigned char* sval, double* sncp, int16_t* sexp, int* err, uint32_t anchor = 0,
                                              int reach = kLayoutWindow) {
    const int G = shape_G(S);
    uint32_t slice_local, r;
    row_to_slot(S, T, p - S.row_base, slice_local, r);
    uint32_t orig = order[p];
    uint64_t fr = row_ptr[orig];
    int L = (int)(row_ptr[orig + 1] - fr);
    const uint64_t pl_local = (uint64_t)slice_local * S.K * 64;
    const uint64_t vl_local = (uint64_t)slice_local * shape_val_stride(S);
    const uint64_t pl0 = S.plane_base * 64 + pl_local;
    const uint32_t slot = S.slot_base + slice_local * shape_R(S) + r;
    Q32Scale q{0};
    if (cp && S.fmt == kFmtQ32) {
        double vmx = 0.0;
        for (int c = 0; c < L; c++) vmx = fmax(vmx, cp[fr + c]);
        if (!q32_scale_of(vmx, vmx, 0, q)) { if (err) *err = 3; q.e = 0; }
        if (sexp) sexp[slot] = (int16_t)q.e;
    }
    int ci = 0;
    for (int c = 0; c < L; c++) {
        if (S.fmt == kFmtF64X && !in_split_window(sid[fr + c], anchor, reach)) continue;
        const uint64_t off = (uint64_t)(ci >> S.lg) * 64 + r * G + (ci & (G - 1));
        bool ok;
        const uint64_t voff = vl_local + shape_val_off(S, r, ci, &ok);
        ++ci;
        if (!ok) { if (err) *err = 4; continue; }
        if (kIds) ssid[pl0 + off] = sid[fr + c];
        if (cp) {
            if (S.fmt == kFmtQ32) ((uint32_t*)(sval + S.val_base))[voff] = q32_mantissa(cp[fr + c], q.e);
            else ((double*)(sval + S.val_base))[voff] = cp[fr + c];
        }
    }
    if (ncp) sncp[slot] = ncp[orig];
}

__host__ __device__ inline void sell_unfill_row(const Shape& S, uint32_t T, uint32_t p, const uint32_t* __restrict__ order,
                                                const uint64_t* __restrict__ row_ptr, const int32_t* __restrict__ ssid,
                                                const unsigned char* __restrict__ sval, int32_t* sid, double* cp) {
    const int G = shape_G(S);
    uint32_t slice_local, r;
    row_to_slot(S, T, p - S.row_base, slice_local, r);
    const uint32_t orig = order[p];
    const uint64_t fr = row_ptr[orig];
    const int L = (int)(row_ptr[orig + 1] - fr);
    const uint64_t pl_local = (uint64_t)slice_local * S.K * 64;
    const uint64_t vl_local = (uint64_t)slice_local * shape_val_stride(S);
    const uint64_t pl0 = S.plane_base * 64 + pl_local;
    for (int c = 0; c < L; c++) {
        const uint64_t off = (uint64_t)(c >> S.lg) * 64 + r * G + (c & (G - 1));
        sid[fr + c] = ssid[pl0 + off];
        cp[fr + c] = ((const double*)(sval + S.val_base))[vl_local + shape_val_off(S, r, c)];
    }
}
__global__ void k_unfill_sell(const Shape* __restrict__ shapes, int n_shapes, uint32_t T, uint32_t n_sell_rows,
                              const uint32_t* __restrict__ order, const uint64_t* __restrict__ row_ptr, const int32_t* __restrict__ ssid,
                              const unsigned char* __restrict__ sval, int32_t* sid, double* cp) {
    const uint32_t p = blockIdx.x * blockDim.x + threadIdx.x;
    if (p >= n_sell_rows) return;
    sell_unfill_row(shapes[find_shape_by_row(shapes, n_shapes, p)], T, p, order, row_ptr, ssid, sval, sid, cp);
}

template <bool kIds>
__global__ void k_fill_sell(const Shape* __restrict__ shapes, int n_shapes, uint32_t T, uint32_t n_sell_rows,
                            const uint32_t* __restrict__ order, const uint64_t* __restrict__ row_ptr,
                            const int32_t* __restrict__ sid, const double* __restrict__ cp,
                            const double* __restrict__ ncp, int32_t* ssid, unsigned char* sval, double* sncp,
                            int16_t* sexp, int* err, const uint32_t* __restrict__ xanchor, uint32_t x_row_base, int reach,
                            const uint32_t* __restrict__ xreach = nullptr ) {
    uint32_t p = blockIdx.x * blockDim.x + threadIdx.x;
    if (p >= n_sell_rows) return;
    const Shape S = shapes[find_shape_by_row(shapes, n_shapes, p)];
    const bool x = S.fmt == kFmtF64X;
    sell_fill_row<kIds>(S, T, p, order, row_ptr, sid, cp, ncp, ssid, sval, sncp, sexp, err, x ? xanchor[p - x_row_base] : 0u,
                        (x && xreach) ? (int)xreach[p - x_row_base] : reach);
}

__host__ __device__ inline bool slice_lane_changed(const Shape& S, uint32_t T, uint32_t sl, int lane, const int32_t* __restrict__ ssid) {
    if (sl % T == 0) return true;
    const uint64_t pl0 = (S.plane_base + (uint64_t)sl * S.K) * 64;
    bool changed = false;
    for (int k = 0; k < S.K; k++) {
        int v = ssid[pl0 + (uint64_t)k * 64 + lane];
        int pv = ssid[pl0 - (uint64_t)S.K * 64 + (uint64_t)k * 64 + lane];
        changed = changed || (pv != v);
    }
    return changed;
}
__host__ __device__ inline unsigned long long read_lanes_of(const Shape& S, int lane) {
    const int G = shape_G(S);
    const int gb = lane & ~(G - 1);
    return (G == 64) ? ~0ull : (((1ull << G) - 1) << gb);
}

__global__ void k_slice_masks(const Shape* __restrict__ shapes, int n_shapes, uint32_t T, uint32_t n_slices,
                              const int32_t* __restrict__ ssid, unsigned long long* masks) {
    __shared__ Shape sh_shapes[kMaxShapes];
    for (int i = threadIdx.x; i < n_shapes; i += blockDim.x) sh_shapes[i] = shapes[i];
    __syncthreads();
    int lane = threadIdx.x & 63;
    uint32_t s = blockIdx.x * (blockDim.x / 64) + (threadIdx.x >> 6);
    if (s >= n_slices) return;
    int sh = 0;
    while (sh + 1 < n_shapes && s >= sh_shapes[sh + 1].slice_base) ++sh;
    const Shape S = sh_shapes[sh];
    const bool changed = slice_lane_changed(S, T, s - S.slice_base, lane, ssid);
    unsigned long long m = __ballot(changed);
    m = __ballot((m & read_lanes_of(S, lane)) != 0);
    if (lane == 0) masks[s] = m;
}

__global__ void k_count_sid_planes(const Shape* __restrict__ shapes, int n_shapes, uint32_t n_slices,
                                   const unsigned long long* __restrict__ masks, unsigned long long* out) {
    const uint32_t s = blockIdx.x * blockDim.x + threadIdx.x;
    unsigned long long k = 0;
    if (s < n_slices && masks[s] != 0ull) {
        int sh = 0;
        while (sh + 1 < n_shapes && s >= shapes[sh + 1].slice_base) ++sh;
        k = (unsigned long long)shapes[sh].K;
    }
    for (int d = 32; d >= 1; d >>= 1) k += __shfl_xor(k, d);
    if ((threadIdx.x & 63) == 0 && k) atomicAdd(out, k);
}

__global__ void k_slice_minsid(const Shape* __restrict__ shapes, int n_shapes, uint32_t T, uint32_t n_slices,
                               const uint64_t* __restrict__ keys_sorted, uint32_t* slice_minsid) {
    uint32_t s = blockIdx.x * blockDim.x + threadIdx.x;
    if (s >= n_slices) return;
    int sh = 0;
    while (sh + 1 < n_shapes && s >= shapes[sh + 1].slice_base) ++sh;
    const Shape S = shapes[sh];
    const uint32_t sl = s - S.slice_base, R = shape_R(S);
    uint32_t q = (sl / T) * R * T + sl % T;
    slice_minsid[s] = (uint32_t)((keys_sorted[S.row_base + q] >> 32) & kKeyMinSidCap);
}

__global__ void k_slice_maxanchor(const Shape* __restrict__ shapes, int n_shapes, uint32_t T, uint32_t n_slices,
                                  const uint64_t* __restrict__ keys_sorted, uint32_t* slice_maxanchor) {
    uint32_t s = blockIdx.x * blockDim.x + threadIdx.x;
    if (s >= n_slices) return;
    int sh = 0;
    while (sh + 1 < n_shapes && s >= shapes[sh + 1].slice_base) ++sh;
    const Shape S = shapes[sh];
// ... 18 lines not shown
    while (sh + 1 < n_shapes && s >= sh_shapes[sh + 1].slice_base) ++sh;
    const Shape S = sh_shapes[sh];
    uint64_t pl0 = (S.plane_base + (uint64_t)(s - S.slice_base) * S.K) * 64;
    int mx = 0;
    const long long lim = (long long)slice_minsid[s] + window_cap;
    for (int k = 0; k < S.K; k++) {
        const int v = ssid[pl0 + (uint64_t)k * 64 + lane];
        if ((long long)v < lim) mx = max(mx, v);
    }
    for (int d = 32; d >= 1; d >>= 1) mx = max(mx, __shfl_xor(mx, d));
    if (lane == 0) slice_maxsid[s] = (uint32_t)mx;
}

template <typename T>
hipError_t dmalloc(T** p, size_t n) { return hipMalloc((void**)p, std::max<size_t>(n, 1) * sizeof(T)); }

__global__ void k_x_anchors(uint32_t n_x, uint32_t x_row_base, const uint64_t* __restrict__ keys_sorted, uint32_t* xanchor) {
    const uint32_t x = blockIdx.x * blockDim.x + threadIdx.x;
    if (x < n_x) xanchor[x] = (uint32_t)((keys_sorted[x_row_base + x] >> 32) & kKeyMinSidCap);
}
__global__ void k_x_far(const Shape* __restrict__ shapes, int n_shapes, uint32_t T, uint32_t n_x, uint32_t x_row_base, uint32_t x_slot_base,
                        const uint32_t* __restrict__ order, const uint64_t* __restrict__ row_ptr, const int32_t* __restrict__ sid,
                        const uint32_t* __restrict__ xanchor, uint64_t* nfar, const uint64_t* __restrict__ far_ptr, int32_t* far_sid, uint64_t* far_src,
                        uint32_t* far_eslot, int reach, const uint32_t* __restrict__ xreach = nullptr) {
    const uint32_t x = blockIdx.x * blockDim.x + threadIdx.x;
    if (x >= n_x) return;
    if (xreach) reach = (int)xreach[x];
    const uint32_t p = x_row_base + x, orig = order[p], anchor = xanchor[x];
    const uint64_t fr = row_ptr[orig], to = row_ptr[orig + 1];
    const Shape S = shapes[find_shape_by_row(shapes, n_shapes, p)];
    uint32_t slice_local, r;
    row_to_slot(S, T, p - S.row_base, slice_local, r);
    const uint32_t slot = S.slot_base + slice_local * shape_R(S) + r, xs = slot - x_slot_base;
    if (!far_ptr) {
        uint64_t n = 0;
        for (uint64_t j = fr; j < to; j++) n += in_split_window(sid[j], anchor, reach) ? 0 : 1;
        nfar[xs] = n;
        return;
    }
    uint64_t e = far_ptr[xs];
    for (uint64_t j = fr; j < to; j++)
        if (!in_split_window(sid[j], anchor, reach)) { far_sid[e] = sid[j]; far_src[e] = j; far_eslot[e] = slot; ++e; }
}
constexpr int kCscSlotBlockLg = 16;
__global__ void k_x_csc_keys(uint64_t n_far, uint32_t x_slot_base, const int32_t* __restrict__ far_sid, const uint32_t* __restrict__ far_eslot,
                             uint64_t* keys, uint64_t* vals, int block_lg) {
    const uint64_t e = (uint64_t)blockIdx.x * blockDim.x + threadIdx.x;
    if (e >= n_far) return;
    keys[e] = ((uint64_t)((far_eslot[e] - x_slot_base) >> block_lg) << 32) | (uint32_t)far_sid[e];
    vals[e] = e;
}
__global__ void k_x_csc(uint64_t n_far, const uint64_t* __restrict__ perm, const int32_t* __restrict__ far_sid, const uint64_t* __restrict__ far_src,
                        const uint32_t* __restrict__ far_eslot, int32_t* csc_sid, uint64_t* csc_src, uint32_t* csc_slot) {
    const uint64_t i = (uint64_t)blockIdx.x * blockDim.x + threadIdx.x;
    if (i >= n_far) return;
    const uint64_t e = perm[i];
    csc_sid[i] = far_sid[e];
    csc_src[i] = far_src[e];
    csc_slot[i] = far_eslot[e];
}
__global__ void k_x_values(uint64_t n_far, const double* __restrict__ cp, const uint64_t* __restrict__ far_src, const uint64_t* __restrict__ csc_src,
                           double* far_cp, double* csc_cp) {
    const uint64_t i = (uint64_t)blockIdx.x * blockDim.x + threadIdx.x;
    if (i >= n_far) return;
    far_cp[i] = cp[far_src[i]];
    csc_cp[i] = cp[csc_src[i]];
}

struct SellLayout {
    uint64_t N1 = 0;
    uint32_t T = 16;
    uint32_t* d_order = nullptr;
    uint32_t n_sell_rows = 0;
    uint32_t n_long_rows = 0;
    Shape h_shapes[kMaxShapes];
    int n_shapes = 0;
    Shape* d_shapes = nullptr;
    uint32_t n_slices = 0;
    uint32_t n_slots = 0;
    uint64_t n_planes = 0;
    uint64_t val_bytes = 0;
    uint64_t n_val_entries = 0;
    uint64_t short_classes = 0;
    uint32_t n_q32_rows = 0;
    uint64_t n_q32_planes = 0;
    uint64_t n_sid_planes_loaded = 0;
    uint32_t x_row_base = 0, n_x_rows = 0;
    uint32_t x_slot_base = 0;
    uint64_t n_far = 0;
    uint32_t* d_xanchor = nullptr;
    uint32_t* d_xreach = nullptr;
    uint32_t n_x_slots = 0;
    uint64_t* d_far_ptr = nullptr;
    int32_t* d_far_sid = nullptr;
    uint64_t* d_far_src = nullptr;
    double* d_far_cp = nullptr;
    int32_t* d_csc_sid = nullptr;
    uint64_t* d_csc_src = nullptr;
    uint32_t* d_csc_slot = nullptr;
    double* d_csc_cp = nullptr;
    int32_t* d_ssid = nullptr;
    unsigned long long* d_masks = nullptr;
    uint32_t* d_slice_minsid = nullptr;
    uint32_t* d_slice_maxsid = nullptr;
    uint32_t* d_slice_maxanchor = nullptr;
};

inline void sell_free(SellLayout& L) {
    hipFree(L.d_order); hipFree(L.d_shapes); hipFree(L.d_ssid); hipFree(L.d_masks); hipFree(L.d_slice_minsid); hipFree(L.d_slice_maxsid); hipFree(L.d_slice_maxanchor);
    hipFree(L.d_xanchor); hipFree(L.d_xreach); hipFree(L.d_far_ptr); hipFree(L.d_far_sid); hipFree(L.d_far_src); hipFree(L.d_far_cp);
    hipFree(L.d_csc_sid); hipFree(L.d_csc_src); hipFree(L.d_csc_slot); hipFree(L.d_csc_cp);
    L = SellLayout();
}

inline int sell_fill_values(const SellLayout& L, hipStream_t st, const uint64_t* d_row_ptr, const double* d_cp,
                            const double* d_ncp, void* d_sval, double* d_sncp, int16_t* d_sexp = nullptr,
                            int* d_err = nullptr, const int32_t* d_sid = nullptr) {
    RSEM_HIP_TRY(hipMemsetAsync(d_sval, 0, L.val_bytes, st));
    RSEM_HIP_TRY(hipMemsetAsync(d_sncp, 0, sizeof(double) * L.n_slots, st));
    if (d_sexp) RSEM_HIP_TRY(hipMemsetAsync(d_sexp, 0, sizeof(int16_t) * L.n_slots, st));
    if (L.n_x_rows && !d_sid) { rsem::set_last_error("a layout with split rows needs the transcript ids to place their values"); return RSEM_ERR_STATE; }
    if (L.n_sell_rows) {
        hipLaunchKernelGGL(k_fill_sell<false>, dim3(rsem::ceil_div(L.n_sell_rows, kBlock)), dim3(kBlock), 0, st,
                           L.d_shapes, L.n_shapes, L.T, L.n_sell_rows, L.d_order, d_row_ptr, d_sid,
                           d_cp, d_ncp, (int32_t*)nullptr, (unsigned char*)d_sval, d_sncp, d_sexp, d_err, (const uint32_t*)L.d_xanchor, L.x_row_base, kLayoutWindow,
                           (const uint32_t*)L.d_xreach);
        RSEM_HIP_TRY(hipGetLastError());
    }
    if (L.n_far) {
        hipLaunchKernelGGL(k_x_values, dim3(rsem::ceil_div(L.n_far, kBlock)), dim3(kBlock), 0, st, L.n_far, d_cp, (const uint64_t*)L.d_far_src,
                           (const uint64_t*)L.d_csc_src, L.d_far_cp, L.d_csc_cp);
        RSEM_HIP_TRY(hipGetLastError());
    }
    return RSEM_OK;
}

inline int sell_build_far(SellLayout& L, hipStream_t st, const uint64_t* d_row_ptr, const int32_t* d_sid, const uint64_t* d_keys_sorted) {
    const uint32_t nx = L.n_x_rows;
    if (!nx) return RSEM_OK;
    const uint32_t nxs = L.n_x_slots;
    if (d_keys_sorted) {
        RSEM_HIP_TRY(dmalloc(&L.d_xanchor, nx));
        hipLaunchKernelGGL(k_x_anchors, dim3(rsem::ceil_div(nx, kBlock)), dim3(kBlock), 0, st, nx, L.x_row_base, d_keys_sorted, L.d_xanchor);
    } else {
        hipFree(L.d_far_ptr); hipFree(L.d_far_sid); hipFree(L.d_far_src); hipFree(L.d_far_cp);
        hipFree(L.d_csc_sid); hipFree(L.d_csc_src); hipFree(L.d_csc_slot); hipFree(L.d_csc_cp);
        L.d_far_ptr = nullptr; L.d_far_sid = nullptr; L.d_far_src = nullptr; L.d_far_cp = nullptr;
        L.d_csc_sid = nullptr; L.d_csc_src = nullptr; L.d_csc_slot = nullptr; L.d_csc_cp = nullptr;
        L.n_far = 0;
    }
    RSEM_HIP_TRY(dmalloc(&L.d_far_ptr, (size_t)nxs + 1));
    uint64_t* d_n = nullptr;
    void* d_tmp = nullptr;
    uint64_t *d_perm_in = nullptr, *d_perm = nullptr, *d_k_in = nullptr, *d_k_out = nullptr;
    uint32_t* d_eslot = nullptr;
    auto cleanup = [&]() { hipFree(d_n); hipFree(d_tmp); hipFree(d_perm_in); hipFree(d_perm); hipFree(d_k_in); hipFree(d_k_out); hipFree(d_eslot); };
    hipError_t e = dmalloc(&d_n, (size_t)nxs + 1);
    if (e == hipSuccess) e = hipMemsetAsync(d_n, 0, sizeof(uint64_t) * ((size_t)nxs + 1), st);
    if (e != hipSuccess) { cleanup(); RSEM_HIP_TRY(e); }
    hipLaunchKernelGGL(k_x_far, dim3(rsem::ceil_div(nx, kBlock)), dim3(kBlock), 0, st, (const Shape*)L.d_shapes, L.n_shapes, L.T, nx, L.x_row_base, L.x_slot_base,
                       (const uint32_t*)L.d_order, d_row_ptr, d_sid, (const uint32_t*)L.d_xanchor, d_n, (const uint64_t*)nullptr, (int32_t*)nullptr,
                       (uint64_t*)nullptr, (uint32_t*)nullptr, kLayoutWindow, (const uint32_t*)L.d_xreach);
    size_t tb = 0;
    e = hipcub::DeviceScan::ExclusiveSum(nullptr, tb, d_n, L.d_far_ptr, (size_t)nxs + 1, st);
    if (e == hipSuccess) e = hipMalloc(&d_tmp, tb ? tb : 1);
    if (e == hipSuccess) e = hipcub::DeviceScan::ExclusiveSum(d_tmp, tb, d_n, L.d_far_ptr, (size_t)nxs + 1, st);
    uint64_t nf = 0;
    if (e == hipSuccess) e = hipMemcpyAsync(&nf, L.d_far_ptr + nxs, sizeof(uint64_t), hipMemcpyDeviceToHost, st);
    if (e == hipSuccess) e = hipStreamSynchronize(st);
    if (e != hipSuccess) { cleanup(); RSEM_HIP_TRY(e); }
    L.n_far = nf;
    e = dmalloc(&L.d_far_sid, nf);
    if (e == hipSuccess) e = dmalloc(&L.d_far_src, nf);
    if (e == hipSuccess) e = dmalloc(&L.d_far_cp, nf);
    if (e == hipSuccess) e = dmalloc(&L.d_csc_sid, nf);
    if (e == hipSuccess) e = dmalloc(&L.d_csc_src, nf);
    if (e == hipSuccess) e = dmalloc(&L.d_csc_slot, nf);
    if (e == hipSuccess) e = dmalloc(&L.d_csc_cp, nf);
    if (e == hipSuccess) e = dmalloc(&d_eslot, nf);
    if (e == hipSuccess) e = hipMemsetAsync(L.d_far_cp, 0, sizeof(double) * std::max<uint64_t>(nf, 1), st);
    if (e == hipSuccess) e = hipMemsetAsync(L.d_csc_cp, 0, sizeof(double) * std::max<uint64_t>(nf, 1), st);
    if (e != hipSuccess) { cleanup(); RSEM_HIP_TRY(e); }
    hipLaunchKernelGGL(k_x_far, dim3(rsem::ceil_div(nx, kBlock)), dim3(kBlock), 0, st, (const Shape*)L.d_shapes, L.n_shapes, L.T, nx, L.x_row_base, L.x_slot_base,
                       (const uint32_t*)L.d_order, d_row_ptr, d_sid, (const uint32_t*)L.d_xanchor, (uint64_t*)nullptr, (const uint64_t*)L.d_far_ptr,
                       L.d_far_sid, L.d_far_src, d_eslot, kLayoutWindow, (const uint32_t*)L.d_xreach);
    if (nf) {
        hipFree(d_tmp); d_tmp = nullptr;
        e = dmalloc(&d_perm_in, nf);
        if (e == hipSuccess) e = dmalloc(&d_perm, nf);
        if (e == hipSuccess) e = dmalloc(&d_k_in, nf);
        if (e == hipSuccess) e = dmalloc(&d_k_out, nf);
        if (e != hipSuccess) { cleanup(); RSEM_HIP_TRY(e); }
        int block_lg = kCscSlotBlockLg;
        if (const char* eb = getenv("RSEM_HIP_CSC_BLOCK_LG")) block_lg = std::min(31, std::max(8, atoi(eb)));
        hipLaunchKernelGGL(k_x_csc_keys, dim3(rsem::ceil_div(nf, kBlock)), dim3(kBlock), 0, st, nf, L.x_slot_base, (const int32_t*)L.d_far_sid,
                           (const uint32_t*)d_eslot, d_k_in, d_perm_in, block_lg);
        tb = 0;
        e = hipcub::DeviceRadixSort::SortPairs(nullptr, tb, (const uint64_t*)d_k_in, d_k_out, (const uint64_t*)d_perm_in, d_perm, nf, 0, 64, st);
        if (e == hipSuccess) e = hipMalloc(&d_tmp, tb ? tb : 1);
        if (e == hipSuccess) e = hipcub::DeviceRadixSort::SortPairs(d_tmp, tb, (const uint64_t*)d_k_in, d_k_out, (const uint64_t*)d_perm_in, d_perm, nf, 0, 64, st);
        if (e != hipSuccess) { cleanup(); RSEM_HIP_TRY(e); }
        hipLaunchKernelGGL(k_x_csc, dim3(rsem::ceil_div(nf, kBlock)), dim3(kBlock), 0, st, nf, (const uint64_t*)d_perm, (const int32_t*)L.d_far_sid,
                           (const uint64_t*)L.d_far_src, (const uint32_t*)d_eslot, L.d_csc_sid, L.d_csc_src, L.d_csc_slot);
    }
    e = hipGetLastError();
    if (e == hipSuccess) e = hipStreamSynchronize(st);
    cleanup();
    RSEM_HIP_TRY(e);
    return RSEM_OK;
}

inline int sell_build(SellLayout& L, hipStream_t st, uint64_t N1, int32_t M, const uint64_t* d_row_ptr,
                      const int32_t* d_sid, uint32_t target_waves, uint32_t forced_T = 0,
                      const double* d_cp_for_q32 = nullptr, int range_bits = 0, const unsigned char* d_also_apart = nullptr, int split = 0,
                      int short_min_units = 0 ) {
    L.N1 = N1;
    int apart = kLayoutWindow;
    if (const char* e = getenv("RSEM_HIP_APART")) apart = atoi(e) ? kLayoutWindow : 0;
    uint64_t *d_keys = nullptr, *d_keys2 = nullptr;
    uint32_t *d_vals = nullptr, *d_first = nullptr;
    int* d_err = nullptr;
    void* d_tmp = nullptr;
    unsigned long long* d_ns = nullptr;
    auto cleanup = [&]() {
        hipFree(d_keys); hipFree(d_keys2); hipFree(d_vals); hipFree(d_first); hipFree(d_err); hipFree(d_tmp); hipFree(d_ns);
    };
    RSEM_HIP_TRY(dmalloc(&d_keys, N1));
    RSEM_HIP_TRY(dmalloc(&d_keys2, N1));
    RSEM_HIP_TRY(dmalloc(&d_vals, N1));
    RSEM_HIP_TRY(dmalloc(&L.d_order, N1));
    RSEM_HIP_TRY(dmalloc(&d_first, kShapeIds));
    RSEM_HIP_TRY(dmalloc(&d_err, 1));
    RSEM_HIP_TRY(hipMemsetAsync(d_err, 0, sizeof(int), st));
    RSEM_HIP_TRY(hipMemsetAsync(d_first, 0xff, kShapeIds * sizeof(uint32_t), st));
    uint64_t short_classes = 0;
    if (N1 && short_min_units > 0) {
        unsigned long long* d_hist = nullptr;
        unsigned long long h_hist[2 * kLenHist];
        RSEM_HIP_TRY(dmalloc(&d_hist, 2 * kLenHist));
        hipError_t e = hipMemsetAsync(d_hist, 0, sizeof(h_hist), st);
        if (e == hipSuccess) {
            hipLaunchKernelGGL(k_row_length_hist, dim3((unsigned)std::min<uint64_t>(4096, rsem::ceil_div(N1, kBlock))), dim3(kBlock), 0, st, N1, d_row_ptr,
                               d_cp_for_q32, range_bits, d_hist);
            e = hipGetLastError();
        }
        if (e == hipSuccess) e = hipMemcpyAsync(h_hist, d_hist, sizeof(h_hist), hipMemcpyDeviceToHost, st);
        if (e == hipSuccess) e = hipStreamSynchronize(st);
        (void)hipFree(d_hist);
        if (e != hipSuccess) { cleanup(); RSEM_HIP_TRY(e); }
        short_classes = short_classes_worth_it(h_hist, target_waves, forced_T, short_min_units);
    }
    L.short_classes = short_classes;
    if (N1) {
        int do_split = apart ? split : 0;
        if (do_split) {
            unsigned long long h_ns[2] = {0, 0};
            RSEM_HIP_TRY(dmalloc(&d_ns, 2));
            RSEM_HIP_TRY(hipMemsetAsync(d_ns, 0, 2 * sizeof(unsigned long long), st));
            hipLaunchKernelGGL(k_row_keys, dim3(rsem::ceil_div(N1, kBlock)), dim3(kBlock), 0, st, N1, M, d_row_ptr, d_sid,
                               d_cp_for_q32, range_bits, apart, do_split, d_also_apart, d_keys, d_vals, d_err, d_ns, short_classes);
            RSEM_HIP_TRY(hipGetLastError());
            RSEM_HIP_TRY(hipMemcpyAsync(h_ns, d_ns, sizeof(h_ns), hipMemcpyDeviceToHost, st));
            RSEM_HIP_TRY(hipStreamSynchronize(st));
            if (h_ns[0] * 20ull < N1 && !getenv("RSEM_HIP_SPLIT_ALWAYS")) do_split = 0;
        }
        if (!do_split) {
            hipLaunchKernelGGL(k_row_keys, dim3(rsem::ceil_div(N1, kBlock)), dim3(kBlock), 0, st, N1, M, d_row_ptr, d_sid,
                               d_cp_for_q32, range_bits, apart, 0, d_also_apart, d_keys, d_vals, d_err, (unsigned long long*)nullptr, short_classes);
            RSEM_HIP_TRY(hipGetLastError());
        }
        size_t tb = 0;
        RSEM_HIP_TRY(hipcub::DeviceRadixSort::SortPairs(nullptr, tb, d_keys, d_keys2, d_vals, L.d_order, N1, 0, 64, st));
        RSEM_HIP_TRY(hipMalloc(&d_tmp, tb ? tb : 1));
        RSEM_HIP_TRY(hipcub::DeviceRadixSort::SortPairs(d_tmp, tb, d_keys, d_keys2, d_vals, L.d_order, N1, 0, 64, st));
        hipLaunchKernelGGL(k_shape_bounds, dim3(rsem::ceil_div(N1, kBlock)), dim3(kBlock), 0, st, N1, d_keys2, d_first);
        RSEM_HIP_TRY(hipGetLastError());
    }
    uint32_t h_first[kShapeIds];
    int h_err = 0;
    RSEM_HIP_TRY(hipMemcpyAsync(h_first, d_first, sizeof(h_first), hipMemcpyDeviceToHost, st));
    RSEM_HIP_TRY(hipMemcpyAsync(&h_err, d_err, sizeof(int), hipMemcpyDeviceToHost, st));
    RSEM_HIP_TRY(hipStreamSynchronize(st));
    if (h_err) {
        cleanup();
        rsem::set_last_error(h_err == 1 ? "row_ptr is not monotone" : "sid outside 1..M");
        return RSEM_ERR_INVALID;
    }
    L.n_shapes = 0;
    L.n_slices = 0;
    L.n_planes = 0;
    L.n_slots = 0;
    L.val_bytes = 0;
    L.n_q32_rows = 0;
    L.n_q32_planes = 0;
    L.n_x_rows = 0;
    L.x_row_base = 0;
    L.x_slot_base = 0;
    L.n_far = 0;
    L.n_x_slots = 0;
    L.n_val_entries = 0;
    uint32_t long_first = (h_first[kLongShape] == 0xffffffffu) ? (uint32_t)N1 : h_first[kLongShape];
    L.n_sell_rows = long_first;
    L.n_long_rows = (uint32_t)N1 - long_first;
    for (int id = 0; id < kMaxShapes; id++) {
        if (h_first[id] == 0xffffffffu) continue;
        uint32_t next = long_first;
        for (int j = id + 1; j < kMaxShapes; j++)
            if (h_first[j] != 0xffffffffu) { next = h_first[j]; break; }
        Shape& S = L.h_shapes[L.n_shapes++];
        {
            int fmt = 0, lg = 0, K = 1, cut = 0;
            shape_of_id(id, fmt, lg, K, cut);
            S.fmt = fmt; S.lg = lg; S.K = K; S.cut = cut; S.reserved = 0;
        }
        S.row_base = h_first[id];
        S.n_rows = next - h_first[id];
        uint32_t rps = shape_R(S);
        S.n_slices = (S.n_rows + rps - 1) / rps;
        S.slice_base = L.n_slices;
        S.plane_base = L.n_planes;
        S.slot_base = L.n_slots;
        S.val_base = L.val_bytes;
        L.n_slices += S.n_slices;
        L.n_planes += (uint64_t)S.n_slices * S.K;
        L.n_slots += S.n_slices * rps;
        L.val_bytes += shape_val_bytes(S);
        L.n_val_entries += (uint64_t)S.n_slices * shape_val_stride(S);
        if (S.fmt == kFmtQ32) { L.n_q32_rows += S.n_rows; L.n_q32_planes += (uint64_t)S.n_slices * S.K; }
        if (S.fmt == kFmtF64X) {
            if (!L.n_x_rows) { L.x_row_base = S.row_base; L.x_slot_base = S.slot_base; }
            L.n_x_rows += S.n_rows;
            L.n_x_slots += S.n_slices * rps;
        }
    }
    uint32_t T = forced_T ? forced_T : L.n_slices / std::max(1u, target_waves);
    L.T = std::min<uint32_t>(256, std::max<uint32_t>(forced_T ? 1 : 8, T));
    RSEM_HIP_TRY(dmalloc(&L.d_shapes, kMaxShapes));
    RSEM_HIP_TRY(hipMemcpyAsync(L.d_shapes, L.h_shapes, sizeof(Shape) * kMaxShapes, hipMemcpyHostToDevice, st));
    RSEM_HIP_TRY(dmalloc(&L.d_ssid, L.n_planes * 64));
    RSEM_HIP_TRY(dmalloc(&L.d_masks, (size_t)L.n_slices));
    RSEM_HIP_TRY(dmalloc(&L.d_slice_minsid, (size_t)L.n_slices));
    RSEM_HIP_TRY(dmalloc(&L.d_slice_maxsid, (size_t)L.n_slices));
    RSEM_HIP_TRY(dmalloc(&L.d_slice_maxanchor, (size_t)L.n_slices));
    RSEM_HIP_TRY(hipMemsetAsync(L.d_ssid, 0, sizeof(int32_t) * L.n_planes * 64, st));
    if (L.n_x_rows) {
        const int frc = sell_build_far(L, st, d_row_ptr, d_sid, d_keys2);
        if (frc != RSEM_OK) { cleanup(); return frc; }
    }
    if (L.n_sell_rows) {
        hipLaunchKernelGGL(k_fill_sell<true>, dim3(rsem::ceil_div(L.n_sell_rows, kBlock)), dim3(kBlock), 0, st,
                           L.d_shapes, L.n_shapes, L.T, L.n_sell_rows, L.d_order, d_row_ptr, d_sid, (const double*)nullptr,
                           (const double*)nullptr, L.d_ssid, (unsigned char*)nullptr, (double*)nullptr, (int16_t*)nullptr,
                           (int*)nullptr, (const uint32_t*)L.d_xanchor, L.x_row_base, kLayoutWindow);
        RSEM_HIP_TRY(hipGetLastError());
        hipLaunchKernelGGL(k_slice_minsid, dim3(rsem::ceil_div(L.n_slices, kBlock)), dim3(kBlock), 0, st, L.d_shapes,
                           L.n_shapes, L.T, L.n_slices, d_keys2, L.d_slice_minsid);
        RSEM_HIP_TRY(hipGetLastError());
        hipLaunchKernelGGL(k_slice_maxanchor, dim3(rsem::ceil_div(L.n_slices, kBlock)), dim3(kBlock), 0, st, L.d_shapes,
                           L.n_shapes, L.T, L.n_slices, d_keys2, L.d_slice_maxanchor);
        RSEM_HIP_TRY(hipGetLastError());
        hipLaunchKernelGGL(k_slice_maxsid, dim3(rsem::ceil_div(L.n_slices, kBlock / 64)), dim3(kBlock), 0, st, L.d_shapes,
                           L.n_shapes, L.n_slices, L.d_ssid, L.d_slice_minsid, kLayoutWindow, L.d_slice_maxsid);
        RSEM_HIP_TRY(hipGetLastError());
        hipLaunchKernelGGL(k_slice_masks, dim3(rsem::ceil_div(L.n_slices, kBlock / 64)), dim3(kBlock), 0, st,
                           L.d_shapes, L.n_shapes, L.T, L.n_slices, L.d_ssid, L.d_masks);
        RSEM_HIP_TRY(hipGetLastError());
        unsigned long long* d_cnt = (unsigned long long*)d_keys;
        RSEM_HIP_TRY(hipMemsetAsync(d_cnt, 0, sizeof(unsigned long long), st));
        hipLaunchKernelGGL(k_count_sid_planes, dim3(rsem::ceil_div(L.n_slices, kBlock)), dim3(kBlock), 0, st, L.d_shapes, L.n_shapes,
                           L.n_slices, (const unsigned long long*)L.d_masks, d_cnt);
        RSEM_HIP_TRY(hipGetLastError());
        unsigned long long h_cnt = 0;
        RSEM_HIP_TRY(hipMemcpyAsync(&h_cnt, d_cnt, sizeof(h_cnt), hipMemcpyDeviceToHost, st));
        RSEM_HIP_TRY(hipStreamSynchronize(st));
        L.n_sid_planes_loaded = h_cnt;
    }
    RSEM_HIP_TRY(hipStreamSynchronize(st));
    cleanup();
    return RSEM_OK;
}

struct Unit {
    int32_t shape;
    uint32_t slice_begin;
    uint32_t n_slices;
    uint32_t per_wave;
    int32_t base;
    int32_t span;
    int32_t pad[2];
    Shape S;
};

inline int sell_build_units(const SellLayout& L, std::vector<Unit>& units, int window_cap) {
    std::vector<uint32_t> ms(L.n_slices), mx(L.n_slices), ma(L.n_slices);
    if (L.n_slices) {
        RSEM_HIP_TRY(hipMemcpy(ms.data(), L.d_slice_minsid, sizeof(uint32_t) * L.n_slices, hipMemcpyDeviceToHost));
        RSEM_HIP_TRY(hipMemcpy(mx.data(), L.d_slice_maxsid, sizeof(uint32_t) * L.n_slices, hipMemcpyDeviceToHost));
        RSEM_HIP_TRY(hipMemcpy(ma.data(), L.d_slice_maxanchor, sizeof(uint32_t) * L.n_slices, hipMemcpyDeviceToHost));
    }
    double f_full = 1.0, f_half = 0.0;
    if (const char* e = getenv("RSEM_HIP_TAPER")) {
        double a = 0, b = 0;
        if (sscanf(e, "%lf,%lf", &a, &b) == 2 && a >= 0 && b >= 0 && a + b <= 1.0) { f_full = a; f_half = b; }
    }
    constexpr uint32_t W = 4;
    units.clear();
    auto add = [&](int sh, const Shape& S, uint32_t sl0, uint32_t n, uint32_t per_wave) {
        Unit U;
        U.shape = sh;
        U.slice_begin = sl0;
// ... 75 lines not shown
__global__ __launch_bounds__(256) void k_x_reach(const Unit* __restrict__ units, uint32_t T, const uint32_t* __restrict__ xanchor, uint32_t x_row_base, uint32_t* xreach) {
    const Unit U = units[blockIdx.x];
    const Shape& S = U.S;
    if (S.fmt != kFmtF64X) return;
    const uint32_t R = shape_R(S);
    for (uint32_t i = threadIdx.x; i < U.n_slices * R; i += blockDim.x) {
        uint32_t q;
        if (!slot_to_row(S, T, U.slice_begin + i / R, i % R, q)) continue;
        const uint32_t x = S.row_base + q - x_row_base;
        const long long top = (long long)U.base + U.span;
        const long long r = top - (long long)xanchor[x];
        xreach[x] = (uint32_t)(r < 1 ? kLayoutWindow : (r > kLayoutWindow ? kLayoutWindow : r));
    }
}

inline int sell_masks(SellLayout& L, hipStream_t st) {
    if (!L.n_slices) return RSEM_OK;
    hipLaunchKernelGGL(k_slice_masks, dim3(rsem::ceil_div(L.n_slices, kBlock / 64)), dim3(kBlock), 0, st, L.d_shapes, L.n_shapes, L.T, L.n_slices, L.d_ssid, L.d_masks);
    RSEM_HIP_TRY(hipGetLastError());
    unsigned long long* d_cnt = nullptr;
    RSEM_HIP_TRY(dmalloc(&d_cnt, 1));
    hipError_t e = hipMemsetAsync(d_cnt, 0, sizeof(unsigned long long), st);
    if (e == hipSuccess) {
        hipLaunchKernelGGL(k_count_sid_planes, dim3(rsem::ceil_div(L.n_slices, kBlock)), dim3(kBlock), 0, st, L.d_shapes, L.n_shapes, L.n_slices,
                           (const unsigned long long*)L.d_masks, d_cnt);
        e = hipGetLastError();
    }
    unsigned long long h_cnt = 0;
    if (e == hipSuccess) e = hipMemcpyAsync(&h_cnt, d_cnt, sizeof(h_cnt), hipMemcpyDeviceToHost, st);
    if (e == hipSuccess) e = hipStreamSynchronize(st);
    (void)hipFree(d_cnt);
    RSEM_HIP_TRY(e);
    L.n_sid_planes_loaded = h_cnt;
    return RSEM_OK;
}

inline int sell_refine_split_windows(SellLayout& L, hipStream_t st, const uint64_t* d_row_ptr, const int32_t* d_sid, std::vector<Unit>& units, Unit* d_units) {
    if (!L.n_x_rows || units.empty()) return RSEM_OK;
    size_t n_far_x = 0;
    for (const Unit& u : units) n_far_x += (u.S.fmt == kFmtF64X && u.pad[0] != 0) ? 1 : 0;
    if (!n_far_x) return RSEM_OK;
    RSEM_HIP_TRY(dmalloc(&L.d_xreach, L.n_x_rows));
    hipLaunchKernelGGL(k_x_reach, dim3((unsigned)units.size()), dim3(256), 0, st, (const Unit*)d_units, L.T, (const uint32_t*)L.d_xanchor, L.x_row_base, L.d_xreach);
    RSEM_HIP_TRY(hipGetLastError());
    RSEM_HIP_TRY(hipMemsetAsync(L.d_ssid, 0, sizeof(int32_t) * L.n_planes * 64, st));
    hipLaunchKernelGGL(k_fill_sell<true>, dim3(rsem::ceil_div(L.n_sell_rows, kBlock)), dim3(kBlock), 0, st, L.d_shapes, L.n_shapes, L.T, L.n_sell_rows, L.d_order,
                       d_row_ptr, d_sid, (const double*)nullptr, (const double*)nullptr, L.d_ssid, (unsigned char*)nullptr, (double*)nullptr, (int16_t*)nullptr,
                       (int*)nullptr, (const uint32_t*)L.d_xanchor, L.x_row_base, kLayoutWindow, (const uint32_t*)L.d_xreach);
    RSEM_HIP_TRY(hipGetLastError());
    int rc = sell_masks(L, st);
    if (rc == RSEM_OK) rc = sell_build_far(L, st, d_row_ptr, d_sid, nullptr);
    if (rc == RSEM_OK) rc = sell_flag_far_units(L, units, d_units, st);
    return rc;
}

__global__ __launch_bounds__(256) void k_mark_stray_reads(const Unit* __restrict__ units, const int32_t* __restrict__ ssid, const uint32_t* __restrict__ order,
                                                          uint32_t T, int32_t M, const uint64_t* __restrict__ row_ptr, const int32_t* __restrict__ sid,
                                                          unsigned char* also_apart, unsigned long long* n_marked) {
    const Unit U = units[blockIdx.x];
    if (U.pad[0] == 0) return;
    const Shape& S = U.S;
    const uint64_t p0 = (S.plane_base + (uint64_t)U.slice_begin * S.K) * 64, n = (uint64_t)U.n_slices * S.K * 64;
    unsigned long long mine = 0;
    for (uint64_t i = threadIdx.x; i < n; i += blockDim.x) {
        if (!unit_entry_is_far(U, ssid[p0 + i])) continue;
        const uint32_t sl = U.slice_begin + (uint32_t)(i / ((uint64_t)S.K * 64));
        const uint32_t r = (uint32_t)(i % 64) >> S.lg;
        uint32_t q;
        if (!slot_to_row(S, T, sl, r, q)) continue;
        const uint32_t orig = order[S.row_base + q];
        int e = 0;
        const uint64_t key = row_key_of(orig, M, row_ptr, sid, nullptr, 0, kLayoutWindow, &e);
        if (((key >> kKeyApartBit) & 1ull) == 0ull && also_apart[orig] == 0) {
            also_apart[orig] = 1;
            ++mine;
        }
    }
    if (mine) atomicAdd(n_marked, mine);
}

inline int sell_build_refined(SellLayout& L, hipStream_t st, uint64_t N1, int32_t M, const uint64_t* d_row_ptr, const int32_t* d_sid,
                              uint32_t target_waves, uint32_t forced_T, const double* d_cp_for_q32, int range_bits, int window_cap,
                              std::vector<Unit>& units, Unit** d_units, unsigned long long* n_strays = nullptr, int split = 0,
                              int short_min_units = 0) {
    unsigned char* d_also = nullptr;
    unsigned long long* d_n = nullptr;
    if (n_strays) *n_strays = 0;
    const char* knob = getenv("RSEM_HIP_APART");
    const bool refine = !(knob && atoi(knob) == 0);
    for (int pass = 0; pass < 2; pass++) {
        int rc = sell_build(L, st, N1, M, d_row_ptr, d_sid, target_waves, forced_T, d_cp_for_q32, range_bits, d_also, split, short_min_units);
        if (rc == RSEM_OK) rc = sell_build_units(L, units, window_cap);
        if (rc != RSEM_OK) { (void)hipFree(d_also); return rc; }
        (void)hipFree(*d_units);
        *d_units = nullptr;
        hipError_t e = dmalloc(d_units, units.size());
        if (e == hipSuccess && !units.empty()) e = hipMemcpyAsync(*d_units, units.data(), sizeof(Unit) * units.size(), hipMemcpyHostToDevice, st);
        if (e != hipSuccess) { (void)hipFree(d_also); RSEM_HIP_TRY(e); }
        rc = sell_flag_far_units(L, units, *d_units, st);
        if (rc != RSEM_OK) { (void)hipFree(d_also); return rc; }
        size_t n_far_units = 0;
        for (const Unit& u : units) n_far_units += u.pad[0] != 0;
        if (pass == 1 || !n_far_units || N1 == 0 || !refine) break;
        unsigned long long n = 0;
        e = hipMalloc((void**)&d_also, N1);
        if (e == hipSuccess) e = hipMalloc((void**)&d_n, sizeof(unsigned long long));
        if (e == hipSuccess) e = hipMemsetAsync(d_also, 0, N1, st);
        if (e == hipSuccess) e = hipMemsetAsync(d_n, 0, sizeof(unsigned long long), st);
        if (e == hipSuccess) {
            hipLaunchKernelGGL(k_mark_stray_reads, dim3((unsigned)units.size()), dim3(256), 0, st, (const Unit*)*d_units, (const int32_t*)L.d_ssid,
                               (const uint32_t*)L.d_order, L.T, M, d_row_ptr, d_sid, d_also, d_n);
            e = hipGetLastError();
        }
        if (e == hipSuccess) e = hipMemcpyAsync(&n, d_n, sizeof(n), hipMemcpyDeviceToHost, st);
        if (e == hipSuccess) e = hipStreamSynchronize(st);
        (void)hipFree(d_n);
        if (e != hipSuccess) { (void)hipFree(d_also); RSEM_HIP_TRY(e); }
        if (n == 0) break;
        if (n * 1000ull < N1 && n_far_units * 100 < units.size()) break;
        if (n_strays) *n_strays = n;
        sell_free(L);
    }
    (void)hipFree(d_also);
    if (L.n_x_rows && !(getenv("RSEM_HIP_X_REFINE") && atoi(getenv("RSEM_HIP_X_REFINE")) == 0))
        return sell_refine_split_windows(L, st, d_row_ptr, d_sid, units, *d_units);
    return RSEM_OK;
}

}
```

rsem_amd/csrc/sell_shape.hpp:

```cpp
#pragma once

constexpr int kFmtF64 = 0, kFmtQ32 = 1, kFmtF64X = 2;
constexpr int kShapeTableMax = 148;

struct Shape {
    uint64_t plane_base;
    uint32_t slice_base;
    uint32_t n_slices;
    uint32_t row_base;
    uint32_t n_rows;
    uint32_t slot_base;
    int32_t K;
    int32_t lg;
    int32_t fmt;
    uint64_t val_base;
    int32_t cut;
    int32_t reserved;
};

__host__ __device__ inline uint32_t plane_bytes(int fmt) { return fmt == kFmtQ32 ? 256u : 512u; }

__host__ __device__ inline int shape_G(const Shape& S) {
    return 1 << S.lg;
}
__host__ __device__ inline uint32_t shape_R(const Shape& S) {
    return 64u >> S.lg;
}

__host__ __device__ inline uint32_t shape_val_stride(int K, int cut) {
    return (uint32_t)(K * 64 - 16 * cut);
}
__host__ __device__ inline uint32_t shape_val_stride(const Shape& S) { return shape_val_stride(S.K, S.cut); }
__host__ __device__ inline int shape_Gk(int lg, int cut) {
    return ((1 << lg) * (4 - cut)) >> 2;
}
__host__ __device__ inline int shape_Gk(const Shape& S) { return shape_Gk(S.lg, S.cut); }
__host__ __device__ inline uint32_t shape_val_off(int lg, int K, int cut, uint32_t r, int c, bool* ok = nullptr) {
    const int k = c >> lg, g = c & ((1 << lg) - 1);
    if (k < K - 1 || cut == 0) {
        if (ok) *ok = k < K;
        return (uint32_t)k * 64u + (r << lg) + (uint32_t)g;
    }
    const int Gk = shape_Gk(lg, cut);
    if (ok) *ok = k == K - 1 && g < Gk;
    return (uint32_t)(K - 1) * 64u + r * (uint32_t)Gk + (uint32_t)g;
}
__host__ __device__ inline uint32_t shape_val_off(const Shape& S, uint32_t r, int c, bool* ok = nullptr) {
    return shape_val_off(S.lg, S.K, S.cut, r, c, ok);
}
__host__ __device__ inline uint64_t shape_val_bytes(const Shape& S) {
    return (uint64_t)S.n_slices * shape_val_stride(S) * (plane_bytes(S.fmt) / 64u);
}

__host__ __device__ inline void row_to_slot(const Shape& S, uint32_t T, uint32_t q, uint32_t& slice_local, uint32_t& r) {
    const uint32_t R = shape_R(S), rpb = R * T;
    const uint32_t b = q / rpb, qb = q % rpb;
    const uint32_t left = S.n_rows - b * rpb;
    const uint32_t nb = left < rpb ? left : rpb;
    const uint32_t Tb = (nb + R - 1) / R;
    r = qb / Tb;
    slice_local = b * T + qb % Tb;
}
```

Before: 633.9 billion read-alignments/s.

## Add 56-bit packed value planes with shared per-read exponent for E-step

After: 635.3 billion read-alignments/s, median of 4. No clear change (+0.2%).

```diff
diff --git a/rsem_amd/csrc/em.hip b/rsem_amd/csrc/em.hip
--- a/rsem_amd/csrc/em.hip
+++ b/rsem_amd/csrc/em.hip
@@ -394,7 +394,7 @@
 #endif
 constexpr int kFarQDepth = RSEM_FQ_DEPTH;
 template <bool kFC, bool kSolo = false, bool kFQ = false>
-__global__ __launch_bounds__(kBlock) void k_estep_lane(
+__global__ __launch_bounds__(kBlock, kFQ ? 1 : 4) void k_estep_lane(
     const Shape* __restrict__ shapes, const Unit* __restrict__ units, uint32_t T, int M,
     const double* __restrict__ theta, const double* __restrict__ tsrc, double N0, const unsigned char* __restrict__ sval,
     const int16_t* __restrict__ sexp, const int32_t* __restrict__ ssid, const double* __restrict__ sncp,
@@ -438,12 +438,17 @@
         const uint32_t s_begin = S.slice_base + U.slice_begin + (uint32_t)w * U.per_wave;
         const uint32_t s_end = min(u_end, s_begin + U.per_wave);
 #define RSEM_ESTEP_BLOCK(KK, QQ, FF, XX) \
-    estep_block<KK, kFC, QQ, (QQ ? kQ32Depth[KK - 1] : kF64Depth[KK - 1]), FF, XX>(S, s_begin, s_end, lane, U.base, U.span, theta, tsrc, N0, th_win, cnt_win, sval, sexp, ssid, sncp, masks, counts, noise, neff, M, xa)
+    estep_block<KK, kFC, QQ, (QQ == kFmtQ32 ? kQ32Depth[KK - 1] : kF64Depth[KK - 1]), FF, XX>(S, s_begin, s_end, lane, U.base, U.span, theta, tsrc, N0, th_win, cnt_win, sval, sexp, ssid, sncp, masks, counts, noise, neff, M, xa)
 #define RSEM_ESTEP_BLOCK_FQ(KK, QQ, XX) \
     estep_block<KK, kFC, QQ, kFarQDepth, true, XX, true>(S, s_begin, s_end, lane, U.base, U.span, theta, tsrc, N0, th_win, cnt_win, sval, sexp, ssid, sncp, masks, counts, noise, neff, M, xa, fq)
-        const int code = (S.K - 1) | ((S.fmt == kFmtQ32 ? 1 : 0) << 2) | ((U.pad[0] != 0 ? 1 : 0) << 3) | (((!kFC && S.fmt == kFmtF64X) ? 1 : 0) << 4);
+        const int code = (S.K - 1) | ((S.fmt == kFmtQ32 ? 1 : 0) << 2) | ((U.pad[0] != 0 ? 1 : 0) << 3) | (((!kFC && S.fmt == kFmtF64X) ? 1 : 0) << 4) |
+                         ((S.fmt == kFmtF56 ? 1 : 0) << 5);
         if constexpr (kFQ) {
             if (s_begin < u_end) switch ((code & 7) | ((code >> 4) << 3)) {
+                case 16: RSEM_ESTEP_BLOCK_FQ(1, kFmtF56, false); break;
+                case 17: RSEM_ESTEP_BLOCK_FQ(2, kFmtF56, false); break;
+                case 18: RSEM_ESTEP_BLOCK_FQ(3, kFmtF56, false); break;
+                case 19: RSEM_ESTEP_BLOCK_FQ(4, kFmtF56, false); break;
                 case 0: RSEM_ESTEP_BLOCK_FQ(1, false, false); break;
                 case 1: RSEM_ESTEP_BLOCK_FQ(2, false, false); break;
                 case 2: RSEM_ESTEP_BLOCK_FQ(3, false, false); break;
@@ -466,6 +471,14 @@
             }
         } else
         if (s_begin < u_end) switch (code) {
+            case 32: RSEM_ESTEP_BLOCK(1, kFmtF56, false, false); break;
+            case 33: RSEM_ESTEP_BLOCK(2, kFmtF56, false, false); break;
+            case 34: RSEM_ESTEP_BLOCK(3, kFmtF56, false, false); break;
+            case 35: RSEM_ESTEP_BLOCK(4, kFmtF56, false, false); break;
+            case 40: RSEM_ESTEP_BLOCK(1, kFmtF56, true, false); break;
+            case 41: RSEM_ESTEP_BLOCK(2, kFmtF56, true, false); break;
+            case 42: RSEM_ESTEP_BLOCK(3, kFmtF56, true, false); break;
+            case 43: RSEM_ESTEP_BLOCK(4, kFmtF56, true, false); break;
             case 0: RSEM_ESTEP_BLOCK(1, false, false, false); break;
             case 1: RSEM_ESTEP_BLOCK(2, false, false, false); break;
             case 2: RSEM_ESTEP_BLOCK(3, false, false, false); break;
@@ -824,6 +837,8 @@
     int* d_fill_err = nullptr;
     int value_bits = 64;
     int value_range_bits = 8;
+    int value_pack = 0;
+    bool layout_packed = false;
     int short_last_plane = 1;
     int short_min_units = kShortClassMinUnits;
     bool layout_has_q32 = false;
@@ -1013,6 +1028,7 @@
     const char* why = nullptr;
     if (!c->layout_ok || !c->have_values) why = "there is no layout with values yet";
     else if (c->layout_has_q32 || c->value_bits == 32) why = "Q32 planes hold rounded values";
+    else if (c->L.n_f56_rows && !c->d_sexp) why = "the packed reads' exponents are missing";
     else if (c->L.n_x_rows) why = "split rows keep part of their alignments outside the planes";
     else if (c->L.n_long_rows) why = "reads with more than 256 alignments live in the CSR alone";
     else if (c->views_out > 0) why = "a model context still holds the arrays";
@@ -1037,7 +1053,7 @@
     if (c->L.n_sell_rows)
         hipLaunchKernelGGL(k_unfill_sell, dim3(rsem::ceil_div(c->L.n_sell_rows, kBlock)), dim3(kBlock), 0, c->stream, c->L.d_shapes, c->L.n_shapes, c->L.T,
                            c->L.n_sell_rows, (const uint32_t*)c->L.d_order, (const uint64_t*)c->d_row_ptr, (const int32_t*)c->L.d_ssid,
-                           (const unsigned char*)c->d_sval, c->d_sid, c->d_cp);
+                           (const unsigned char*)c->d_sval, c->d_sid, c->d_cp, (const int16_t*)c->d_sexp);
     RSEM_HIP_TRY(hipGetLastError());
     RSEM_HIP_TRY(hipStreamSynchronize(c->stream));
     c->csr_released = false;
@@ -1048,17 +1064,18 @@
     if (c->d_fill_err) RSEM_HIP_TRY(hipMemsetAsync(c->d_fill_err, 0, sizeof(int), c->stream));
     int rc = sell_fill_values(c->L, c->stream, c->d_row_ptr, c->d_cp, c->d_ncp, c->d_sval, c->d_sncp, c->d_sexp, c->d_fill_err, c->d_sid);
     if (rc != RSEM_OK) return rc;
-    if (c->layout_has_q32) {
+    if (c->layout_has_q32 || c->L.n_f56_rows) {
         int h = 0;
         RSEM_HIP_TRY(hipMemcpyAsync(&h, c->d_fill_err, sizeof(int), hipMemcpyDeviceToHost, c->stream));
         RSEM_HIP_TRY(hipStreamSynchronize(c->stream));
-        if (h) { rsem::set_last_error("Q32 planes: a read's values left the range its format was chosen for"); return RSEM_ERR_STATE; }
-    }
-    return RSEM_OK;
-}
-
+        if (h) { rsem::set_last_error("Q32 / packed planes: a read's values left the range its format was chosen for"); return RSEM_ERR_STATE; }
+    }
+    return RSEM_OK;
+}
+
+bool pack_wanted(const rsem_em_ctx* c);
 int fill_values(rsem_em_ctx* c) {
-    if (c->value_bits == 32 || c->layout_has_q32) {
+    if (c->value_bits == 32 || c->layout_has_q32 || c->layout_packed || pack_wanted(c)) {
         free_layout(c);
         return build_layout(c);
     }
@@ -1074,12 +1091,20 @@
     c->h_units.clear();
     c->n_units = 0;
     c->layout_has_q32 = false;
+    c->layout_packed = false;
     c->layout_ok = false;
+}
+
+bool pack_wanted(const rsem_em_ctx* c) {
+    int on = c->value_pack;
+    if (const char* e = getenv("RSEM_HIP_VALUE_PACK")) on = atoi(e) != 0;
+    return on && c->have_values && c->value_bits != 32 && resolved_kernel(c) == RSEM_EM_KERNEL_LANE;
 }
 
 int build_layout(rsem_em_ctx* c) {
     const uint32_t target_waves = (uint32_t)c->n_cus * 4 * 6 * 5 / 2;
     const bool q32 = c->value_bits == 32 && c->have_values;
+    const bool pack = !q32 && pack_wanted(c);
     std::vector<Unit> units;
     int split = c->split_rows && resolved_kernel(c) == RSEM_EM_KERNEL_LANE && !q32;
     int short_on = c->short_last_plane, short_min_units = c->short_min_units;
@@ -1089,8 +1114,8 @@
     if (split) split = c->split_policy;
     if (const char* e = getenv("RSEM_HIP_SPLIT_POLICY")) { if (split) split = !strcmp(e, "all") ? 2 : 1; }
     int rc = sell_build_refined(c->L, c->stream, c->N1, c->M, c->d_row_ptr, c->d_sid, target_waves, c->forced_T,
-                                q32 ? c->d_cp : nullptr, c->value_range_bits, kWindow, units, &c->d_units, &c->n_stray_reads, split,
-                                short_on ? short_min_units : 0);
+                                (q32 || pack) ? c->d_cp : nullptr, c->value_range_bits, kWindow, units, &c->d_units, &c->n_stray_reads, split,
+                                short_on ? short_min_units : 0, pack ? 1 : 0);
     if (rc != RSEM_OK) return rc;
     if (c->L.n_x_rows) {
         const size_t nxs = (size_t)c->L.n_x_slots;
@@ -1100,9 +1125,10 @@
         RSEM_HIP_TRY(hipMemsetAsync(c->d_xinv, 0, sizeof(double) * std::max<size_t>(nxs, 1), c->stream));
     }
     c->layout_has_q32 = q32;
+    c->layout_packed = pack;
     RSEM_HIP_TRY(hipMalloc((void**)&c->d_sval, std::max<uint64_t>(c->L.val_bytes, 1)));
     RSEM_HIP_TRY(dmalloc(&c->d_sncp, (size_t)c->L.n_slots));
-    if (q32) {
+    if (q32 || c->L.n_f56_rows) {
         RSEM_HIP_TRY(dmalloc(&c->d_sexp, (size_t)c->L.n_slots));
         RSEM_HIP_TRY(dmalloc(&c->d_fill_err, 1));
     }
@@ -1363,6 +1389,18 @@
         set_grid_for_kernel(c);
         return RSEM_OK;
     }
+    if (!strcmp(key, "value_pack")) {
+        RSEM_REQUIRE(value == 0 || value == 1, "value_pack must be 0 or 1");
+        c->value_pack = (int)value;
+        if (!c->layout_ok || c->layout_has_q32 || pack_wanted(c) == c->layout_packed) return RSEM_OK;
+        RSEM_HIP_TRY(hipSetDevice(c->device));
+        { int rc0 = ensure_csr(c); if (rc0 != RSEM_OK) return rc0; }
+        free_layout(c);
+        int rc = build_layout(c);
+        if (rc != RSEM_OK) return rc;
+        set_grid_for_kernel(c);
+        return RSEM_OK;
+    }
     if (!strcmp(key, "short_last_plane") || !strcmp(key, "short_class_min_units")) {
         const bool sw = !strcmp(key, "short_last_plane");
         if (sw) RSEM_REQUIRE(value == 0 || value == 1, "short_last_plane must be 0 or 1");
@@ -1416,9 +1454,15 @@
     else if (!strcmp(key, "reads_long")) *value = c->L.n_long_rows;
     else if (!strcmp(key, "value_plane_bytes")) *value = (int64_t)c->L.val_bytes;
     else if (!strcmp(key, "value_plane_entries")) *value = (int64_t)c->L.n_val_entries;
+    else if (!strcmp(key, "value_pack")) *value = c->value_pack;
+    else if (!strcmp(key, "reads_f56")) *value = c->L.n_f56_rows;
+    else if (!strcmp(key, "reads_f56_fraction")) {
+        *value = c->L.n_sell_rows ? (int64_t)(((unsigned __int128)c->L.n_f56_rows * 1000000000ull) / c->L.n_sell_rows) : 0;
+    }
+    else if (!strcmp(key, "value_exponent_bytes")) *value = (c->layout_has_q32 || c->L.n_f56_rows) ? (int64_t)c->L.n_slots * 2 : 0;
     else if (!strcmp(key, "short_last_plane")) *value = c->short_last_plane;
     else if (!strcmp(key, "short_class_min_units")) *value = c->short_min_units;
-    else if (!strcmp(key, "short_classes")) *value = (int64_t)__builtin_popcountll(c->L.short_classes);
+    else if (!strcmp(key, "short_classes")) *value = (int64_t)(__builtin_popcountll(c->L.short_classes) + __builtin_popcount(c->L.short_classes_f56));
     else if (!strcmp(key, "shapes")) *value = c->L.n_shapes;
     else if (!strcmp(key, "unit_bytes")) *value = (int64_t)sizeof(Unit);
     else if (!strcmp(key, "sid_plane_bytes")) *value = (int64_t)(c->L.n_planes * 256);
@@ -1436,7 +1480,7 @@
         for (const Unit& u : c->h_units) w += u.span;
         const uint64_t long_nnz = c->long_nnz + (c->L.n_long_rows * 4ull) / 3;
         const uint64_t far_bytes = 28 * c->L.n_far + 40 * (uint64_t)c->L.n_x_slots;
-        *value = (int64_t)(c->L.val_bytes + c->L.n_sid_planes_loaded * 256 + (uint64_t)c->L.n_slots * (8 + (c->layout_has_q32 ? 2 : 0)) +
+        *value = (int64_t)(c->L.val_bytes + c->L.n_sid_planes_loaded * 256 + (uint64_t)c->L.n_slots * (8 + ((c->layout_has_q32 || c->L.n_f56_rows) ? 2 : 0)) +
                            (uint64_t)c->L.n_slices * 8 + (uint64_t)c->n_units * sizeof(Unit) + (uint64_t)w * 16 + 16 * ((uint64_t)c->M + 1)) +
                  (int64_t)(12 * long_nnz + far_bytes);
     }
@@ -1846,13 +1890,13 @@
 }
 
 bool em_planes_writable(const rsem_em_ctx* c) {
-    return c && c->layout_ok && !c->layout_has_q32 && c->value_bits != 32 && !c->L.n_x_rows;
+    return c && c->layout_ok && !c->layout_has_q32 && c->value_bits != 32 && !c->L.n_x_rows && !c->L.n_f56_rows;
 }
 
 int em_planes_view(rsem_em_ctx* c, EmPlanesView* v) {
     RSEM_REQUIRE(c && v, "NULL argument");
     if (!em_planes_writable(c)) {
-        set_last_error("the layout holds Q32 planes or split rows");
+        set_last_error("the layout holds Q32 planes, split rows or 56-bit entries (value_pack)");
         return RSEM_ERR_STATE;
     }
     RSEM_HIP_TRY(hipSetDevice(c->device));
@@ -1873,7 +1917,7 @@
 
 int em_values_written_in_place(rsem_em_ctx* c) {
     RSEM_REQUIRE(c, "NULL argument");
-    if (!c->layout_ok || c->layout_has_q32) { set_last_error("the layout cannot have been written in place"); return RSEM_ERR_STATE; }
+    if (!c->layout_ok || c->layout_has_q32 || c->L.n_f56_rows) { set_last_error("the layout cannot have been written in place"); return RSEM_ERR_STATE; }
     c->have_values = true;
     return RSEM_OK;
 }
diff --git a/rsem_amd/csrc/estep_block.hpp b/rsem_amd/csrc/estep_block.hpp
--- a/rsem_amd/csrc/estep_block.hpp
+++ b/rsem_amd/csrc/estep_block.hpp
@@ -49,10 +49,12 @@
     int* n = nullptr;
 };
 
-template <int K, bool kQ>
+template <int kFmt>
+struct SliceVal { using type = typename std::conditional<kFmt == kFmtQ32, uint32_t, typename std::conditional<kFmt == kFmtF56, uint64_t, double>::type>::type; };
+template <int K, int kFmt>
 struct SliceRegs {
     int id[K];
-    typename std::conditional<kQ, uint32_t, double>::type c[K];
+    typename SliceVal<kFmt>::type c[K];
     double nc;
     int e;
     double x;
@@ -88,7 +90,17 @@
 constexpr int kF64Depth[4] = {RSEM_F64_DEPTHS};
 constexpr int kQ32Depth[4] = {RSEM_Q32_DEPTHS};
 
-template <int K, bool kFC, bool kQ, int NBUF, bool kFar, bool kX = false, bool kFQ = false>
+RSEM_DEVFN void f56_or_group(uint32_t& lo, uint32_t& hi) {
+    lo |= (uint32_t)RSEM_DPP_MOV((int)lo, 0xB1);  hi |= (uint32_t)RSEM_DPP_MOV((int)hi, 0xB1);
+    lo |= (uint32_t)RSEM_DPP_MOV((int)lo, 0x4E);  hi |= (uint32_t)RSEM_DPP_MOV((int)hi, 0x4E);
+    lo |= (uint32_t)RSEM_DPP_MOV((int)lo, 0x141); hi |= (uint32_t)RSEM_DPP_MOV((int)hi, 0x141);
+}
+RSEM_DEVFN void f56_top_byte(uint64_t w, unsigned j, uint32_t& lo, uint32_t& hi) {
+    const uint32_t tb = j < 7u ? (uint32_t)(w >> 56) : 0u;
+    lo = j < 4u ? tb << (8u * j) : 0u;
+    hi = j >= 4u ? tb << (8u * (j & 3u)) : 0u;
+}
+template <int K, bool kFC, int kFmt, int NBUF, bool kFar, bool kX = false, bool kFQ = false>
 RSEM_DEVFN void estep_block(const Shape& S, uint32_t s_begin, uint32_t s_end, int lane, int base, int span,
                                    const double* __restrict__ theta, const double* __restrict__ tsrc, double N0, double* th_win, double* cnt_win,
                                    const unsigned char* __restrict__ sval, const int16_t* __restrict__ sexp, const int32_t* __restrict__ ssid,
@@ -96,7 +108,10 @@
                                    double* counts, double& noise, double& neff, int M, const XArgs& X = XArgs(), const FarQueue& FQ = FarQueue()) {
     static_assert(!kFQ || kFar, "the far queue belongs to the loop of the units with ids outside their window");
     static_assert(!kFQ || NBUF >= 3, "the far-queue loop requests theta a slice ahead: three register sets at least (the ring loop)");
-    using ValT = typename std::conditional<kQ, uint32_t, double>::type;
+    constexpr bool kQ = kFmt == kFmtQ32, kP = kFmt == kFmtF56;
+    static_assert(kFmt == kFmtF64 || kQ || kP, "split rows (F64X shapes) run the F64 loop with kX");
+    static_assert(!(kP && kX), "split rows hold doubles");
+    using ValT = typename SliceVal<kFmt>::type;
     const ValT* __restrict__ scp = (const ValT*)(sval + S.val_base);
     const int lg = S.lg;
     const int g = lane & ((1 << lg) - 1);
@@ -119,8 +134,13 @@
     const unsigned Gk = (unsigned)shape_Gk(S);
     const unsigned last_lane = uslot * Gk + ((unsigned)g < Gk ? (unsigned)g : Gk - 1u);
     const bool last_ok = (unsigned)g < Gk;
-    const uint32_t vstride = (uint32_t)RSEM_READFIRSTLANE((int)shape_val_stride(S));
-    auto issue = [&](uint32_t t, unsigned long long m, SliceRegs<K, kQ>& b) {
+    const uint32_t vstride = (uint32_t)RSEM_READFIRSTLANE((int)(kP ? shape_val_stride(S) / 8u * 7u : shape_val_stride(S)));
+    constexpr unsigned kPlane = kP ? 56u : 64u;
+    const unsigned vlane = kP ? (unsigned)f56_word_of(ulane) : ulane;
+    const unsigned vlast = kP ? (unsigned)f56_word_of(last_lane) : last_lane;
+    const bool p_regroup = kP && (Gk & 7u) != 0u && Gk != (1u << lg);
+    const unsigned entry_src = p_regroup ? ((ulane / Gk) << lg) + ulane % Gk : ulane;
+    auto issue = [&](uint32_t t, unsigned long long m, SliceRegs<K, kFmt>& b) {
         const uint32_t sl = t - S.slice_base;
         const uint64_t v0 = (uint64_t)sl * (K * 64);
         const ValT* __restrict__ vp = scp + (uint64_t)sl * vstride;
@@ -130,11 +150,11 @@
             for (int k = 0; k < K; k++) b.id[k] = ip[k * 64 + ulane];
         }
 #pragma unroll
-        for (int k = 0; k < K - 1; k++) b.c[k] = stream_load(&vp[k * 64 + ulane]);
-        b.c[K - 1] = stream_load(&vp[(K - 1) * 64 + last_lane]);
+        for (int k = 0; k < K - 1; k++) b.c[k] = stream_load(&vp[k * kPlane + vlane]);
+        b.c[K - 1] = stream_load(&vp[(K - 1) * kPlane + vlast]);
         const uint32_t slot0 = S.slot_base + sl * R;
         b.nc = (sncp + slot0)[uslot];
-        b.e = kQ ? (int)(sexp + slot0)[uslot] : 0;
+        b.e = (kQ || kP) ? (int)(sexp + slot0)[uslot] : 0;
         b.x = kX ? (X.extra + (slot0 - X.slot_base))[uslot] : 0.0;
         b.slot0 = slot0;
     };
@@ -173,7 +193,7 @@
     for (int k = 0; k < K; k++) { rsid[k] = 0; rth[k] = 0.0; acc[k] = 0.0; }
     ThetaSrc th{theta, 0.0, 1.0};
     double th0 = 0.0;
-    auto pregather = [&](SliceRegs<K, kQ>& b, unsigned long long m) {
+    auto pregather = [&](SliceRegs<K, kFmt>& b, unsigned long long m) {
         if (!kFQ) return;
         const bool starts = ((m >> lane) & 1ull) != 0ull;
 #pragma unroll
@@ -183,7 +203,22 @@
             b.traw[k] = th.v[want ? sidv : 0];
         }
     };
-    auto reduce = [&](const SliceRegs<K, kQ>& cur, unsigned long long cur_m) {
+    auto f56_value = [&](uint64_t w, bool last) -> double {
+        const bool regroup = last && p_regroup;
+        uint32_t lo, hi;
+        uint32_t wtop = (uint32_t)(w >> 32);
+        if (regroup) wtop = (uint32_t)RSEM_SHFL((int)wtop, (int)entry_src);
+        f56_top_byte((uint64_t)wtop << 32, ulane & 7u, lo, hi);
+        f56_or_group(lo, hi);
+        if (regroup) {
+            lo = (uint32_t)RSEM_SHFL((int)lo, (int)last_lane);
+            hi = (uint32_t)RSEM_SHFL((int)hi, (int)last_lane);
+        }
+        const unsigned j = (last ? last_lane : ulane) & 7u;
+        const uint64_t entry = j == 7u ? (((uint64_t)hi << 32) | lo) : (w & 0x00ffffffffffffffull);
+        return RSEM_LL_AS_DOUBLE((long long)entry);
+    };
+    auto reduce = [&](const SliceRegs<K, kFmt>& cur, unsigned long long cur_m) {
         if (cur_m != 0ull) {
             far_queue_room(false);
             if ((cur_m >> lane) & 1ull) {
@@ -223,10 +258,18 @@
         double f[K];
         double part = f0 + ((kX && g0) ? cur.x : 0.0);
         const double scale = kQ ? pow2_of(cur.e) : 1.0;
+        const uint64_t rebase = kP ? (uint64_t)(long long)(cur.e - 1) << 52 : 0ull;
 #pragma unroll
         for (int k = 0; k < K; k++) {
-            const ValT cr = (k == K - 1 && !last_ok) ? ValT(0) : cur.c[k];
-            const double cv = kQ ? (double)cr * scale : (double)cr;
+            double cv;
+            if constexpr (kP) {
+                const uint64_t entry = (uint64_t)RSEM_DOUBLE_AS_LL(f56_value(cur.c[k], k == K - 1));
+                const bool none = (k == K - 1 && !last_ok) || (entry >> 52) == 0ull;
+                cv = none ? 0.0 : RSEM_LL_AS_DOUBLE((long long)(entry + rebase));
+            } else {
+                const ValT cr = (k == K - 1 && !last_ok) ? ValT(0) : cur.c[k];
+                cv = kQ ? (double)cr * scale : (double)cr;
+            }
             double v = rth[k] * cv;
             if (v < kEpsilon) v = 0.0;
             f[k] = v;
@@ -241,7 +284,7 @@
         for (int k = 0; k < K; k++) acc[k] = acc[k] + f[k] * inv;
     };
     if constexpr (NBUF == 2) {
-        SliceRegs<K, kQ> A, B;
+        SliceRegs<K, kFmt> A, B;
         unsigned long long mA = ~0ull, mB = 0;
         issue(s_begin, mA, A);
         th = theta_src<kFC>(theta, tsrc, N0, lane);
@@ -265,7 +308,7 @@
             reduce(A, mA);
         }
     } else {
-        SliceRegs<K, kQ> buf[NBUF];
+        SliceRegs<K, kFmt> buf[NBUF];
         unsigned long long mk[NBUF];
         mk[0] = ~0ull;
         issue(s_begin, mk[0], buf[0]);
diff --git a/rsem_amd/csrc/host/run_em.cpp b/rsem_amd/csrc/host/run_em.cpp
--- a/rsem_amd/csrc/host/run_em.cpp
+++ b/rsem_amd/csrc/host/run_em.cpp
@@ -644,6 +644,16 @@
         std::vector<uint8_t>().swap(lq);
     });
     Joiner release_joiner{releaser};
+    if (value_bits != 32 && (ROUND < MIN_ROUND || (totNum > 0 && ROUND < MAX_ROUND))) {
+        each_shard([&](Shard& X, int) {
+            int64_t cur = 0;
+            X.rc = rsem_em_get_info(X.em, "value_pack", &cur);
+            if (X.rc == RSEM_OK) X.rc = rsem_em_set_option(X.em, "value_pack", cur);
+            if (X.rc != RSEM_OK) X.err = rsem_hip_last_error();
+        });
+        check_shards("rsem_em_set_option(value_pack)");
+        lap("packed value planes");
+    }
     if (leanDevice) {
         each_shard([&](Shard& X, int) {
             rsem_model_destroy(X.mc);
diff --git a/rsem_amd/csrc/sell_layout.hpp b/rsem_amd/csrc/sell_layout.hpp
--- a/rsem_amd/csrc/sell_layout.hpp
+++ b/rsem_amd/csrc/sell_layout.hpp
@@ -16,6 +16,9 @@
 constexpr int kShortPerFmt = 32;
 constexpr int kMaxShapes = kFullShapes + 2 * kShortPerFmt;
 static_assert(kMaxShapes <= kShapeTableMax, "the kernels that keep the shape table in LDS size it by kShapeTableMax (sell_shape.hpp)");
+constexpr int kF56FullBase = kMaxShapes;
+constexpr int kF56ShortBase = kF56FullBase + kShapesPerFmt;
+constexpr int kShapeIdEnd = kF56ShortBase + kShortPerFmt;
 constexpr int kShapeIds = 1 << kShapeBits;
 constexpr int kLongShape = kShapeIds - 1;
 constexpr uint32_t kKeyMinSidCap = (1u << (31 - kShapeBits)) - 1;
@@ -58,7 +61,12 @@
     return 2 + (lg - 2) * 6 + (K - 3) * 3 + (q - 1);
 }
 __host__ __device__ inline bool shape_of_id(int id, int& fmt, int& lg, int& K, int& cut) {
-    if (id < 0 || id >= kMaxShapes) return false;
+    if (id < 0 || id >= kShapeIdEnd) return false;
+    if (id >= kF56FullBase) {
+        const bool ok = id < kF56ShortBase ? shape_of_id(id - kF56FullBase, fmt, lg, K, cut) : shape_of_id(kFullShapes + (id - kF56ShortBase), fmt, lg, K, cut);
+        fmt = kFmtF56;
+        return ok;
+    }
     if (id < kFullShapes) {
         fmt = id / kShapesPerFmt;
         lg = (id % kShapesPerFmt) / 4;
@@ -74,11 +82,14 @@
     cut = 3 - (i - 2) % 3;
     return true;
 }
-__host__ __device__ inline int shape_fmt_of_id(int id) { return id < kFullShapes ? id / kShapesPerFmt : (id - kFullShapes) / kShortPerFmt; }
+__host__ __device__ inline int shape_fmt_of_id(int id) {
+    if (id >= kF56FullBase) return kFmtF56;
+    return id < kFullShapes ? id / kShapesPerFmt : (id - kFullShapes) / kShortPerFmt;
+}
 __host__ __device__ inline int full_shape_of_id(int id) {
     int fmt, lg, K, cut;
-    if (id < kFullShapes || !shape_of_id(id, fmt, lg, K, cut)) return id;
-    return fmt * kShapesPerFmt + lg * 4 + K - 1;
+    if (id < kFullShapes || (id >= kF56FullBase && id < kF56ShortBase) || !shape_of_id(id, fmt, lg, K, cut)) return id;
+    return (fmt == kFmtF56 ? kF56FullBase : fmt * kShapesPerFmt) + lg * 4 + K - 1;
 }
 
 __host__ __device__ inline int shape_id_of(uint64_t L, uint32_t short_classes = 0, bool even_quarters = false) {
@@ -98,6 +109,7 @@
     return lg * 4 + (K - 1);
 }
 __host__ __device__ inline int shape_id_in_fmt(int id, int fmt) {
+    if (fmt == kFmtF56) return id < kFullShapes ? kF56FullBase + id : kF56ShortBase + (id - kFullShapes);
     return id < kFullShapes ? id + fmt * kShapesPerFmt : id + fmt * kShortPerFmt;
 }
 
@@ -125,17 +137,19 @@
 __host__ __device__ inline uint64_t row_key_of(uint64_t i, int32_t M, const uint64_t* __restrict__ row_ptr,
                                                const int32_t* __restrict__ sid, const double* __restrict__ cp, int range_bits,
                                                int apart, int* err, int split = 0, uint32_t* split_far = nullptr,
-                                               uint64_t short_classes = 0 ) {
+                                               uint64_t short_classes = 0 ,
+                                               int pack = 0 , uint32_t short_f56 = 0 ) {
     uint64_t fr = row_ptr[i], to = row_ptr[i + 1];
     if (to < fr) { *err = 1; return 0; }
     uint32_t h = 0x811c9dc5u, mn = 0xffffffffu;
     Q32Range vr;
+    F56Range pr;
     for (uint64_t j = fr; j < to; j++) {
         int32_t s = sid[j];
         if (s < 1 || s > M) { *err = 2; s = 1; }
         h = mix32(h, (uint32_t)s);
         mn = (uint32_t)s < mn ? (uint32_t)s : mn;
-        if (cp) vr.add(cp[j]);
+        if (cp) { if (pack) pr.add(cp[j]); else vr.add(cp[j]); }
     }
     const uint64_t L = to - fr;
     if (L > 1 && !*err) {
@@ -177,8 +191,11 @@
     if (mn > kKeyMinSidCap) mn = kKeyMinSidCap;
     Q32Scale q;
     if (shape != kLongShape) {
-        const bool q32 = cp && vr.takes_q32(range_bits, q);
-        if (short_classes) shape = shape_id_of(to - fr, (uint32_t)(short_classes >> (q32 ? 32 : 0)), q32);
+        const bool q32 = cp && !pack && vr.takes_q32(range_bits, q);
+        int E56;
+        const bool f56 = cp && pack && pr.takes_f56(E56);
+        if (f56) shape = shape_id_in_fmt(shape_id_of(to - fr, short_f56), kFmtF56);
+        else if (short_classes) shape = shape_id_of(to - fr, (uint32_t)(short_classes >> (q32 ? 32 : 0)), q32);
         if (q32) shape = shape_id_in_fmt(shape, kFmtQ32);
     }
     return ((uint64_t)shape << (64 - kShapeBits)) | (far << kKeyApartBit) | ((uint64_t)mn << 32) | h;
@@ -187,12 +204,13 @@
 __global__ void k_row_keys(uint64_t N1, int32_t M, const uint64_t* __restrict__ row_ptr,
                            const int32_t* __restrict__ sid, const double* __restrict__ cp, int range_bits, int apart, int split,
                            const unsigned char* __restrict__ also_apart, uint64_t* keys, uint32_t* vals, int* err,
-                           unsigned long long* n_split = nullptr , uint64_t short_classes = 0) {
+                           unsigned long long* n_split = nullptr , uint64_t short_classes = 0,
+                           int pack = 0, uint32_t short_f56 = 0) {
     uint64_t i = (uint64_t)blockIdx.x * blockDim.x + threadIdx.x;
     if (i >= N1) return;
     int e = 0;
     uint32_t nf = 0;
-    uint64_t key = row_key_of(i, M, row_ptr, sid, cp, range_bits, apart, &e, split, &nf, short_classes);
+    uint64_t key = row_key_of(i, M, row_ptr, sid, cp, range_bits, apart, &e, split, &nf, short_classes, pack, short_f56);
     if (n_split && nf) { atomicAdd(&n_split[0], 1ull); atomicAdd(&n_split[1], (unsigned long long)nf); }
     if (also_apart && also_apart[i] && shape_fmt_of_id((int)(key >> (64 - kShapeBits))) != kFmtF64X) key |= 1ull << kKeyApartBit;
     if (e) *err = e;
@@ -203,27 +221,30 @@
 
 constexpr int kLenHist = 257;
 __global__ void k_row_length_hist(uint64_t N1, const uint64_t* __restrict__ row_ptr, const double* __restrict__ cp, int range_bits,
-                                  unsigned long long* hist ) {
-    __shared__ unsigned int h[2 * kLenHist];
-    for (int i = threadIdx.x; i < 2 * kLenHist; i += blockDim.x) h[i] = 0;
+                                  unsigned long long* hist , int pack = 0) {
+    __shared__ unsigned int h[3 * kLenHist];
+    for (int i = threadIdx.x; i < 3 * kLenHist; i += blockDim.x) h[i] = 0;
     __syncthreads();
     for (uint64_t i = (uint64_t)blockIdx.x * blockDim.x + threadIdx.x; i < N1; i += (uint64_t)gridDim.x * blockDim.x) {
         const uint64_t fr = row_ptr[i], to = row_ptr[i + 1];
         if (to < fr || to - fr > 256) continue;
-        const int fmt = (cp && row_takes_q32(cp, fr, to, range_bits)) ? kFmtQ32 : kFmtF64;
+        int E56;
+        const int fmt = (cp && pack) ? (row_takes_f56(cp, fr, to, E56) ? 2 : 0) : ((cp && row_takes_q32(cp, fr, to, range_bits)) ? kFmtQ32 : kFmtF64);
         atomicAdd(&h[fmt * kLenHist + (int)(to - fr)], 1u);
     }
     __syncthreads();
-    for (int i = threadIdx.x; i < 2 * kLenHist; i += blockDim.x)
+    for (int i = threadIdx.x; i < 3 * kLenHist; i += blockDim.x)
         if (h[i]) atomicAdd(&hist[i], (unsigned long long)h[i]);
 }
 #ifndef RSEM_SHORT_CLASS_MIN_UNITS
 #define RSEM_SHORT_CLASS_MIN_UNITS 8
 #endif
 constexpr int kShortClassMinUnits = RSEM_SHORT_CLASS_MIN_UNITS;
-inline uint64_t short_classes_worth_it(const unsigned long long* hist, uint32_t target_waves, uint32_t forced_T, int min_units) {
-    uint64_t rows[2][kShortPerFmt] = {}, n_slices = 0;
-    for (int f = 0; f < 2; f++)
+inline uint64_t short_classes_worth_it(const unsigned long long* hist, uint32_t target_waves, uint32_t forced_T, int min_units, uint32_t* mask_f56 = nullptr) {
+    uint64_t rows[3][kShortPerFmt] = {}, n_slices = 0;
+    const int nf = mask_f56 ? 3 : 2;
+    if (mask_f56) *mask_f56 = 0;
+    for (int f = 0; f < nf; f++)
         for (int L = 1; L < kLenHist; L++) {
             const unsigned long long n = hist[f * kLenHist + L];
             if (!n) continue;
@@ -235,12 +256,14 @@
         }
     const uint32_t T = forced_T ? forced_T : std::min<uint64_t>(256, std::max<uint64_t>(8, n_slices / std::max(1u, target_waves)));
     uint64_t mask = 0;
-    for (int f = 0; f < 2; f++)
+    for (int f = 0; f < nf; f++)
         for (int i = 0; i < kShortPerFmt; i++) {
             int fmt, lg, K, cut;
             shape_of_id(kFullShapes + i, fmt, lg, K, cut);
             const uint64_t slices = rows[f][i] >> (6 - lg);
-            if (slices >= (uint64_t)min_units * 4 * T && slices > 0) mask |= 1ull << (f * 32 + i);
+            if (!(slices >= (uint64_t)min_units * 4 * T && slices > 0)) continue;
+            if (f < 2) mask |= 1ull << (f * 32 + i);
+            else *mask_f56 |= 1u << i;
         }
     return mask;
 }
@@ -277,6 +300,11 @@
     const uint64_t pl0 = S.plane_base * 64 + pl_local;
     const uint32_t slot = S.slot_base + slice_local * shape_R(S) + r;
     Q32Scale q{0};
+    int E56 = 1;
+    if (cp && S.fmt == kFmtF56) {
+        if (!row_takes_f56(cp, fr, fr + (uint64_t)L, E56)) { if (err) *err = 3; E56 = 1; }
+        if (sexp) sexp[slot] = (int16_t)E56;
+    }
     if (cp && S.fmt == kFmtQ32) {
         double vmx = 0.0;
         for (int c = 0; c < L; c++) vmx = fmax(vmx, cp[fr + c]);
@@ -294,6 +322,7 @@
         if (kIds) ssid[pl0 + off] = sid[fr + c];
         if (cp) {
             if (S.fmt == kFmtQ32) ((uint32_t*)(sval + S.val_base))[voff] = q32_mantissa(cp[fr + c], q.e);
+            else if (S.fmt == kFmtF56) f56_put((uint64_t*)(sval + S.val_base), voff, f56_encode(cp[fr + c], E56));
             else ((double*)(sval + S.val_base))[voff] = cp[fr + c];
         }
     }
@@ -302,7 +331,8 @@
 
 __host__ __device__ inline void sell_unfill_row(const Shape& S, uint32_t T, uint32_t p, const uint32_t* __restrict__ order,
                                                 const uint64_t* __restrict__ row_ptr, const int32_t* __restrict__ ssid,
-                                                const unsigned char* __restrict__ sval, int32_t* sid, double* cp) {
+                                                const unsigned char* __restrict__ sval, int32_t* sid, double* cp,
+                                                const int16_t* __restrict__ sexp = nullptr ) {
     const int G = shape_G(S);
     uint32_t slice_local, r;
     row_to_slot(S, T, p - S.row_base, slice_local, r);
@@ -312,18 +342,21 @@
     const uint64_t pl_local = (uint64_t)slice_local * S.K * 64;
     const uint64_t vl_local = (uint64_t)slice_local * shape_val_stride(S);
     const uint64_t pl0 = S.plane_base * 64 + pl_local;
+    const int E56 = (S.fmt == kFmtF56 && sexp) ? (int)sexp[S.slot_base + slice_local * shape_R(S) + r] : 1;
     for (int c = 0; c < L; c++) {
         const uint64_t off = (uint64_t)(c >> S.lg) * 64 + r * G + (c & (G - 1));
         sid[fr + c] = ssid[pl0 + off];
-        cp[fr + c] = ((const double*)(sval + S.val_base))[vl_local + shape_val_off(S, r, c)];
+        const uint64_t voff = vl_local + shape_val_off(S, r, c);
+        if (S.fmt == kFmtF56) cp[fr + c] = f56_double_of(f56_decode(f56_get((const uint64_t*)(sval + S.val_base), voff), E56));
+        else cp[fr + c] = ((const double*)(sval + S.val_base))[voff];
     }
 }
 __global__ void k_unfill_sell(const Shape* __restrict__ shapes, int n_shapes, uint32_t T, uint32_t n_sell_rows,
                               const uint32_t* __restrict__ order, const uint64_t* __restrict__ row_ptr, const int32_t* __restrict__ ssid,
-                              const unsigned char* __restrict__ sval, int32_t* sid, double* cp) {
+                              const unsigned char* __restrict__ sval, int32_t* sid, double* cp, const int16_t* __restrict__ sexp = nullptr) {
     const uint32_t p = blockIdx.x * blockDim.x + threadIdx.x;
     if (p >= n_sell_rows) return;
-    sell_unfill_row(shapes[find_shape_by_row(shapes, n_shapes, p)], T, p, order, row_ptr, ssid, sval, sid, cp);
+    sell_unfill_row(shapes[find_shape_by_row(shapes, n_shapes, p)], T, p, order, row_ptr, ssid, sval, sid, cp, sexp);
 }
 
 template <bool kIds>
@@ -508,6 +541,8 @@
     uint64_t val_bytes = 0;
     uint64_t n_val_entries = 0;
     uint64_t short_classes = 0;
+    uint32_t short_classes_f56 = 0;
+    uint32_t n_f56_rows = 0;
     uint32_t n_q32_rows = 0;
     uint64_t n_q32_planes = 0;
     uint64_t n_sid_planes_loaded = 0;
@@ -639,7 +674,8 @@
 inline int sell_build(SellLayout& L, hipStream_t st, uint64_t N1, int32_t M, const uint64_t* d_row_ptr,
                       const int32_t* d_sid, uint32_t target_waves, uint32_t forced_T = 0,
                       const double* d_cp_for_q32 = nullptr, int range_bits = 0, const unsigned char* d_also_apart = nullptr, int split = 0,
-                      int short_min_units = 0 ) {
+                      int short_min_units = 0 ,
+                      int pack = 0 ) {
     L.N1 = N1;
     int apart = kLayoutWindow;
     if (const char* e = getenv("RSEM_HIP_APART")) apart = atoi(e) ? kLayoutWindow : 0;
@@ -660,23 +696,26 @@
     RSEM_HIP_TRY(hipMemsetAsync(d_err, 0, sizeof(int), st));
     RSEM_HIP_TRY(hipMemsetAsync(d_first, 0xff, kShapeIds * sizeof(uint32_t), st));
     uint64_t short_classes = 0;
+    uint32_t short_f56 = 0;
+    uint64_t short_classes_unpacked = 0;
     if (N1 && short_min_units > 0) {
         unsigned long long* d_hist = nullptr;
-        unsigned long long h_hist[2 * kLenHist];
-        RSEM_HIP_TRY(dmalloc(&d_hist, 2 * kLenHist));
+        unsigned long long h_hist[3 * kLenHist];
+        RSEM_HIP_TRY(dmalloc(&d_hist, 3 * kLenHist));
         hipError_t e = hipMemsetAsync(d_hist, 0, sizeof(h_hist), st);
         if (e == hipSuccess) {
             hipLaunchKernelGGL(k_row_length_hist, dim3((unsigned)std::min<uint64_t>(4096, rsem::ceil_div(N1, kBlock))), dim3(kBlock), 0, st, N1, d_row_ptr,
-                               d_cp_for_q32, range_bits, d_hist);
+                               d_cp_for_q32, range_bits, d_hist, pack);
             e = hipGetLastError();
         }
         if (e == hipSuccess) e = hipMemcpyAsync(h_hist, d_hist, sizeof(h_hist), hipMemcpyDeviceToHost, st);
         if (e == hipSuccess) e = hipStreamSynchronize(st);
         (void)hipFree(d_hist);
         if (e != hipSuccess) { cleanup(); RSEM_HIP_TRY(e); }
-        short_classes = short_classes_worth_it(h_hist, target_waves, forced_T, short_min_units);
-    }
-    L.short_classes = short_classes;
+        short_classes = short_classes_worth_it(h_hist, target_waves, forced_T, short_min_units, &short_f56);
+        for (int i = 0; i < kLenHist; i++) { h_hist[i] += h_hist[2 * kLenHist + i]; h_hist[2 * kLenHist + i] = 0; }
+        short_classes_unpacked = short_classes_worth_it(h_hist, target_waves, forced_T, short_min_units);
+    }
     if (N1) {
         int do_split = apart ? split : 0;
         if (do_split) {
@@ -684,15 +723,17 @@
             RSEM_HIP_TRY(dmalloc(&d_ns, 2));
             RSEM_HIP_TRY(hipMemsetAsync(d_ns, 0, 2 * sizeof(unsigned long long), st));
             hipLaunchKernelGGL(k_row_keys, dim3(rsem::ceil_div(N1, kBlock)), dim3(kBlock), 0, st, N1, M, d_row_ptr, d_sid,
-                               d_cp_for_q32, range_bits, apart, do_split, d_also_apart, d_keys, d_vals, d_err, d_ns, short_classes);
+                               pack ? (const double*)nullptr : d_cp_for_q32, range_bits, apart, do_split, d_also_apart, d_keys, d_vals, d_err, d_ns,
+                               pack ? short_classes_unpacked : short_classes);
             RSEM_HIP_TRY(hipGetLastError());
             RSEM_HIP_TRY(hipMemcpyAsync(h_ns, d_ns, sizeof(h_ns), hipMemcpyDeviceToHost, st));
             RSEM_HIP_TRY(hipStreamSynchronize(st));
             if (h_ns[0] * 20ull < N1 && !getenv("RSEM_HIP_SPLIT_ALWAYS")) do_split = 0;
+            if (do_split && pack) { short_classes = short_classes_unpacked; short_f56 = 0; }
         }
         if (!do_split) {
             hipLaunchKernelGGL(k_row_keys, dim3(rsem::ceil_div(N1, kBlock)), dim3(kBlock), 0, st, N1, M, d_row_ptr, d_sid,
-                               d_cp_for_q32, range_bits, apart, 0, d_also_apart, d_keys, d_vals, d_err, (unsigned long long*)nullptr, short_classes);
+                               d_cp_for_q32, range_bits, apart, 0, d_also_apart, d_keys, d_vals, d_err, (unsigned long long*)nullptr, short_classes, pack, short_f56);
             RSEM_HIP_TRY(hipGetLastError());
         }
         size_t tb = 0;
@@ -702,6 +743,8 @@
         hipLaunchKernelGGL(k_shape_bounds, dim3(rsem::ceil_div(N1, kBlock)), dim3(kBlock), 0, st, N1, d_keys2, d_first);
         RSEM_HIP_TRY(hipGetLastError());
     }
+    L.short_classes = short_classes;
+    L.short_classes_f56 = short_f56;
     uint32_t h_first[kShapeIds];
     int h_err = 0;
     RSEM_HIP_TRY(hipMemcpyAsync(h_first, d_first, sizeof(h_first), hipMemcpyDeviceToHost, st));
@@ -718,6 +761,7 @@
     L.n_slots = 0;
     L.val_bytes = 0;
     L.n_q32_rows = 0;
+    L.n_f56_rows = 0;
     L.n_q32_planes = 0;
     L.n_x_rows = 0;
     L.x_row_base = 0;
@@ -728,10 +772,11 @@
     uint32_t long_first = (h_first[kLongShape] == 0xffffffffu) ? (uint32_t)N1 : h_first[kLongShape];
     L.n_sell_rows = long_first;
     L.n_long_rows = (uint32_t)N1 - long_first;
-    for (int id = 0; id < kMaxShapes; id++) {
+    for (int id = 0; id < kShapeIdEnd; id++) {
         if (h_first[id] == 0xffffffffu) continue;
+        if (L.n_shapes >= kMaxShapes) { cleanup(); rsem::set_last_error("more shapes than a layout holds"); return RSEM_ERR_STATE; }
         uint32_t next = long_first;
-        for (int j = id + 1; j < kMaxShapes; j++)
+        for (int j = id + 1; j < kShapeIdEnd; j++)
             if (h_first[j] != 0xffffffffu) { next = h_first[j]; break; }
         Shape& S = L.h_shapes[L.n_shapes++];
         {
@@ -752,6 +797,7 @@
         L.n_slots += S.n_slices * rps;
         L.val_bytes += shape_val_bytes(S);
         L.n_val_entries += (uint64_t)S.n_slices * shape_val_stride(S);
+        if (S.fmt == kFmtF56) L.n_f56_rows += S.n_rows;
         if (S.fmt == kFmtQ32) { L.n_q32_rows += S.n_rows; L.n_q32_planes += (uint64_t)S.n_slices * S.K; }
         if (S.fmt == kFmtF64X) {
             if (!L.n_x_rows) { L.x_row_base = S.row_base; L.x_slot_base = S.slot_base; }
@@ -993,14 +1039,14 @@
 inline int sell_build_refined(SellLayout& L, hipStream_t st, uint64_t N1, int32_t M, const uint64_t* d_row_ptr, const int32_t* d_sid,
                               uint32_t target_waves, uint32_t forced_T, const double* d_cp_for_q32, int range_bits, int window_cap,
                               std::vector<Unit>& units, Unit** d_units, unsigned long long* n_strays = nullptr, int split = 0,
-                              int short_min_units = 0) {
+                              int short_min_units = 0, int pack = 0) {
     unsigned char* d_also = nullptr;
     unsigned long long* d_n = nullptr;
     if (n_strays) *n_strays = 0;
     const char* knob = getenv("RSEM_HIP_APART");
     const bool refine = !(knob && atoi(knob) == 0);
     for (int pass = 0; pass < 2; pass++) {
-        int rc = sell_build(L, st, N1, M, d_row_ptr, d_sid, target_waves, forced_T, d_cp_for_q32, range_bits, d_also, split, short_min_units);
+        int rc = sell_build(L, st, N1, M, d_row_ptr, d_sid, target_waves, forced_T, d_cp_for_q32, range_bits, d_also, split, short_min_units, pack);
         if (rc == RSEM_OK) rc = sell_build_units(L, units, window_cap);
         if (rc != RSEM_OK) { (void)hipFree(d_also); return rc; }
         (void)hipFree(*d_units);
diff --git a/rsem_amd/csrc/sell_shape.hpp b/rsem_amd/csrc/sell_shape.hpp
--- a/rsem_amd/csrc/sell_shape.hpp
+++ b/rsem_amd/csrc/sell_shape.hpp
@@ -1,6 +1,6 @@
 #pragma once
 
-constexpr int kFmtF64 = 0, kFmtQ32 = 1, kFmtF64X = 2;
+constexpr int kFmtF64 = 0, kFmtQ32 = 1, kFmtF64X = 2, kFmtF56 = 3;
 constexpr int kShapeTableMax = 148;
 
 struct Shape {
@@ -18,7 +18,7 @@
     int32_t reserved;
 };
 
-__host__ __device__ inline uint32_t plane_bytes(int fmt) { return fmt == kFmtQ32 ? 256u : 512u; }
+__host__ __device__ inline uint32_t plane_bytes(int fmt) { return fmt == kFmtQ32 ? 256u : (fmt == kFmtF56 ? 448u : 512u); }
 
 __host__ __device__ inline int shape_G(const Shape& S) {
     return 1 << S.lg;
@@ -49,7 +49,69 @@
     return shape_val_off(S.lg, S.K, S.cut, r, c, ok);
 }
 __host__ __device__ inline uint64_t shape_val_bytes(const Shape& S) {
-    return (uint64_t)S.n_slices * shape_val_stride(S) * (plane_bytes(S.fmt) / 64u);
+    return ((uint64_t)S.n_slices * shape_val_stride(S) * (plane_bytes(S.fmt) / 64u) + 127u) & ~(uint64_t)127u;
+}
+
+constexpr int kF56MaxSpread = 14;
+__host__ __device__ inline uint64_t f56_bits_of(double v) { uint64_t b; __builtin_memcpy(&b, &v, 8); return b; }
+__host__ __device__ inline double f56_double_of(uint64_t b) { double v; __builtin_memcpy(&v, &b, 8); return v; }
+struct F56Range {
+    uint32_t emin = 2047u, emax = 0u;
+    bool bad = false;
+    __host__ __device__ void add(double v) {
+        const uint64_t b = f56_bits_of(v);
+        if (b == 0ull) return;
+        const uint32_t e = (uint32_t)(b >> 52);
+        if (e == 0u || e >= 2047u) { bad = true; return; }
+        emin = e < emin ? e : emin;
+        emax = e > emax ? e : emax;
+    }
+    __host__ __device__ bool takes_f56(int& E) const {
+        if (bad) return false;
+        if (emax == 0u) { E = 1; return true; }
+        E = (int)emin;
+        return emax - emin <= (uint32_t)kF56MaxSpread;
+    }
+};
+__host__ __device__ inline bool row_takes_f56(const double* __restrict__ cp, uint64_t fr, uint64_t to, int& E) {
+    F56Range r;
+    for (uint64_t j = fr; j < to; j++) r.add(cp[j]);
+    return r.takes_f56(E);
+}
+__host__ __device__ inline uint64_t f56_encode(double v, int E) {
+    const uint64_t b = f56_bits_of(v);
+    return b ? b - ((uint64_t)(E - 1) << 52) : 0ull;
+}
+__host__ __device__ inline uint64_t f56_decode(uint64_t entry, int E) {
+    return (entry >> 52) ? entry + ((uint64_t)(E - 1) << 52) : 0ull;
+}
+__host__ __device__ inline uint64_t f56_word_of(uint64_t entry_index) {
+    const uint64_t j = entry_index & 7u;
+    return (entry_index >> 3) * 7u + (j < 6u ? j : 6u);
+}
+__host__ __device__ inline void f56_or_word(uint64_t* p, uint64_t v) {
+#if defined(__HIP_DEVICE_COMPILE__)
+    atomicOr((unsigned long long*)p, (unsigned long long)v);
+#else
+    *p |= v;
+#endif
+}
+__host__ __device__ inline void f56_put(uint64_t* words, uint64_t entry_index, uint64_t entry) {
+    uint64_t* w = words + (entry_index >> 3) * 7u;
+    const unsigned j = (unsigned)(entry_index & 7u);
+    if (j < 7u) { f56_or_word(w + j, entry); return; }
+    for (unsigned k = 0; k < 7u; k++) {
+        const uint64_t byte = (entry >> (8u * k)) & 0xffull;
+        if (byte) f56_or_word(w + k, byte << 56);
+    }
+}
+__host__ __device__ inline uint64_t f56_get(const uint64_t* words, uint64_t entry_index) {
+    const uint64_t* w = words + (entry_index >> 3) * 7u;
+    const unsigned j = (unsigned)(entry_index & 7u);
+    if (j < 7u) return w[j] & 0x00ffffffffffffffull;
+    uint64_t e = 0;
+    for (unsigned k = 0; k < 7u; k++) e |= (w[k] >> 56) << (8u * k);
+    return e;
 }
 
 __host__ __device__ inline void row_to_slot(const Shape& S, uint32_t T, uint32_t q, uint32_t& slice_local, uint32_t& r) {
```
